# bipul-mohanto/fovPathTracing_optixCodeLatest

Measured on AMD Instinct MI355X. Metric: Mray/s, higher is better.
Workload: dtype f32; 1 GPU; C3: Sponza-class procedural atrium, 265640 tris, 1920x1080, foveated spp fovea/mid/periphery 8/2/1, radii 148/482, gaze centre, Disney BSDF + probe NEE, depth 4, ambient probe 2.5 @ frame res; triangles=265640, width=1920, height=1080, subframe=reset to 0 every frame (as the shipped app), parallelism=single GPU, frames_in_flight=2, gather=none

## Files before the change

fovpathtracing_optixcodelatest_amd/csrc/bvh_build.hip:

```cpp
#include <cstdio>
#include <cstring>
#include <vector>

#include <rocprim/rocprim.hpp>

#include "fovpt_device.h"

namespace {

__device__ inline uint32_t f2ord(float f)
{
    uint32_t u = __float_as_uint(f);
    return (u & 0x80000000u) ? ~u : (u | 0x80000000u);
}
__host__ __device__ inline float ord2f(uint32_t u)
{
    u = (u & 0x80000000u) ? (u & 0x7fffffffu) : ~u;
    float f;
    __builtin_memcpy(&f, &u, 4);
    return f;
}

struct Box { float lo[3], hi[3]; };

// ... 575 lines not shown
        C.code = code;
    }
    nodes[me.out] = nd;
    atomicMax(&stats[0], me.depth + 1u);
    atomicAdd(&stats[1], 1u);
}

#ifndef FOVPT_COST_LEAF_STEP
#define FOVPT_COST_LEAF_STEP 1.4f
#endif
__global__ void k_order_children(uint32_t first, uint32_t count, BvhNode4* __restrict__ nodes, const TriRec* __restrict__ tris, float2* __restrict__ pc)
{
    const uint32_t t = blockIdx.x * blockDim.x + threadIdx.x;
    if (t >= count) return;
    const uint32_t i = first + t;
    const BvhNode4 nd = nodes[i];
    float lo[3] = {INFINITY, INFINITY, INFINITY}, hi[3] = {-INFINITY, -INFINITY, -INFINITY};
    float P[4], C[4], sa[4], key[4];
    for (int k = 0; k < 4; k++) {
        const BvhChild& c = nd.c[k];
        P[k] = 0.f; C[k] = 1.f; sa[k] = 0.f; key[k] = -1.f;
        if (!(c.lox < INFINITY)) continue;
        lo[0] = fminf(lo[0], c.lox); lo[1] = fminf(lo[1], c.loy); lo[2] = fminf(lo[2], c.loz);
        hi[0] = fmaxf(hi[0], c.hix); hi[1] = fmaxf(hi[1], c.hiy); hi[2] = fmaxf(hi[2], c.hiz);
        const float dx = c.hix - c.lox, dy = c.hiy - c.loy, dz = c.hiz - c.loz;
        sa[k] = 2.0f * (dx * dy + dy * dz + dz * dx);
        if (c.code < 0) {
            const uint32_t lcode = (uint32_t)~c.code, n = (lcode & 7u) + 1u, t0 = (lcode >> 3) / 3u;
            float area = 0.f;
            for (uint32_t j = 0; j < n; j++) {
                const TriRec& T = tris[t0 + j];
                const float cx = T.e1y * T.e2z - T.e1z * T.e2y, cy = T.e1z * T.e2x - T.e1x * T.e2z, cz = T.e1x * T.e2y - T.e1y * T.e2x;
                area += 0.5f * sqrtf(cx * cx + cy * cy + cz * cz);
            }
            P[k] = sa[k] > 0.f ? fminf(1.0f, area / sa[k]) : 1.0f;
            C[k] = FOVPT_COST_LEAF_STEP;
        } else {
            const float2 v = pc[c.code];
            P[k] = v.x; C[k] = v.y;
        }
        key[k] = P[k] / C[k];
    }
    const float dx = hi[0] - lo[0], dy = hi[1] - lo[1], dz = hi[2] - lo[2];
    const float sa_node = 2.0f * (dx * dy + dy * dz + dz * dx);
    int ord[4] = {0, 1, 2, 3};
    for (int a = 1; a < 4; a++)
        for (int b = a; b > 0 && key[ord[b]] > key[ord[b - 1]]; b--) { const int tmp = ord[b]; ord[b] = ord[b - 1]; ord[b - 1] = tmp; }
    float pass = 1.0f, cost = 1.0f;
    BvhNode4 out;
    for (int k = 0; k < 4; k++) {
        const int j = ord[k];
        out.c[k] = nd.c[j];
        out.c[k].pad = (uint32_t)j;
        if (key[j] < 0.f) continue;
        const float h = sa_node > 0.f ? fminf(1.0f, sa[j] / sa_node) : 1.0f;
        cost += pass * h * C[j];
        pass *= 1.0f - h * P[j];
    }
    nodes[i] = out;
    pc[i] = make_float2(1.0f - pass, cost);
}

__global__ void k_emit_tiny(int n, const Box* __restrict__ boxes, BvhNode4* __restrict__ nodes, uint32_t* __restrict__ stats, uint32_t* __restrict__ leaf_pos)
{
    Box u = boxes[0];
    for (int i = 1; i < n; i++)
        for (int k = 0; k < 3; k++) { u.lo[k] = fminf(u.lo[k], boxes[i].lo[k]); u.hi[k] = fmaxf(u.hi[k], boxes[i].hi[k]); }
    BvhNode4 nd;
    for (int k = 0; k < 4; k++) {
        BvhChild& C = nd.c[k];
        C.lox = C.loy = C.loz = C.hix = C.hiy = C.hiz = INFINITY;
        C.code = leaf_code(0, 1);
        C.pad = (uint32_t)k;
    }
    nd.c[0].lox = u.lo[0]; nd.c[0].loy = u.lo[1]; nd.c[0].loz = u.lo[2];
    nd.c[0].hix = u.hi[0]; nd.c[0].hiy = u.hi[1]; nd.c[0].hiz = u.hi[2];
    nd.c[0].code = leaf_code(0, n);
    nodes[0] = nd;
    stats[0] = 1; stats[1] = 1;
    for (int i = 0; i < n; i++) leaf_pos[i] = (uint32_t)i;
}

__global__ void k_emit_tris_generic(const float* __restrict__ flat, const uint32_t* __restrict__ mesh_of_prim, const uint32_t* __restrict__ vals,
                                    const uint32_t* __restrict__ ref_prim, const uint32_t* __restrict__ leaf_pos, uint32_t n, TriRec* __restrict__ tris)
{
    uint32_t i = blockIdx.x * blockDim.x + threadIdx.x;
    if (i >= n) return;
    const uint32_t prim = ref_prim ? ref_prim[vals[i]] : vals[i];
    const float* p = flat + (size_t)prim * 9;
    TriRec t;
    t.v0x = p[0]; t.v0y = p[1]; t.v0z = p[2];
    t.e1x = p[3] - p[0]; t.e1y = p[4] - p[1]; t.e1z = p[5] - p[2];
    t.e2x = p[6] - p[0]; t.e2y = p[7] - p[1]; t.e2z = p[8] - p[2];
    t.prim = prim; t.mesh = mesh_of_prim[prim]; t.pad = 0;
    tris[leaf_pos[i]] = t;
}

#define FOVPT_SPLIT_MAX 8
__device__ inline uint32_t split_count(const float* __restrict__ p, float s)
{
    float ext = 0.f;
    for (int a = 0; a < 3; a++) ext = fmaxf(ext, fmaxf(p[a], fmaxf(p[3 + a], p[6 + a])) - fminf(p[a], fminf(p[3 + a], p[6 + a])));
    const float k = floorf(ext / s);
    return k >= (float)FOVPT_SPLIT_MAX ? (uint32_t)FOVPT_SPLIT_MAX : k >= 1.f ? (uint32_t)k : 1u;
}
__global__ void k_split_count(const float* __restrict__ flat, uint32_t n, float s, uint32_t* __restrict__ count, unsigned long long* __restrict__ total)
{
    const uint32_t i = blockIdx.x * blockDim.x + threadIdx.x;
    uint32_t k = i < n ? split_count(flat + (size_t)i * 9, s) : 0u;
    if (count && i < n) count[i] = k;
    for (int off = 32; off > 0; off >>= 1) k += __shfl_xor(k, off);
    if ((threadIdx.x & 63) == 0 && k) atomicAdd(total, (unsigned long long)k);
}
__global__ void k_scene_extent(const float* __restrict__ flat, uint32_t n, uint32_t* __restrict__ bounds)
{
    const uint32_t i = blockIdx.x * blockDim.x + threadIdx.x;
    for (int a = 0; a < 3; a++) {
        float mn = INFINITY, mx = -INFINITY;
        if (i < n) { const float* p = flat + (size_t)i * 9; mn = fminf(p[a], fminf(p[3 + a], p[6 + a])); mx = fmaxf(p[a], fmaxf(p[3 + a], p[6 + a])); }
        for (int off = 32; off > 0; off >>= 1) { mn = fminf(mn, __shfl_xor(mn, off)); mx = fmaxf(mx, __shfl_xor(mx, off)); }
        if ((threadIdx.x & 63) == 0) { atomicMin(&bounds[a], f2ord(mn)); atomicMax(&bounds[3 + a], f2ord(mx)); }
    }
}
__global__ void k_split_emit(const float* __restrict__ flat, uint32_t n, const uint32_t* __restrict__ count, const uint32_t* __restrict__ first,
                             Box* __restrict__ boxes, uint32_t* __restrict__ ref_prim, uint32_t* __restrict__ bounds)
{
    const uint32_t i = blockIdx.x * blockDim.x + threadIdx.x;
    float cmn[3] = {INFINITY, INFINITY, INFINITY}, cmx[3] = {-INFINITY, -INFINITY, -INFINITY};
    if (i < n) {
        const float* p = flat + (size_t)i * 9;
        float lo[3], hi[3], ext = 0.f, mag = 0.f;
        int ax = 0;
        for (int a = 0; a < 3; a++) {
            lo[a] = fminf(p[a], fminf(p[3 + a], p[6 + a])); hi[a] = fmaxf(p[a], fmaxf(p[3 + a], p[6 + a]));
            if (hi[a] - lo[a] > ext) { ext = hi[a] - lo[a]; ax = a; }
            mag = fmaxf(mag, fmaxf(fabsf(lo[a]), fabsf(hi[a])));
        }
        const float pad = fovpt_tri_pad(ext, mag);
        const uint32_t k = count[i], f = first[i];
        for (uint32_t j = 0; j < k; j++) {
            Box b;
            if (k == 1u) { for (int a = 0; a < 3; a++) { b.lo[a] = lo[a]; b.hi[a] = hi[a]; } }
            else {
                const float c0 = j == 0u ? lo[ax] : lo[ax] + (hi[ax] - lo[ax]) * ((float)j / (float)k);
                const float c1 = j + 1u == k ? hi[ax] : lo[ax] + (hi[ax] - lo[ax]) * ((float)(j + 1u) / (float)k);
                for (int a = 0; a < 3; a++) { b.lo[a] = INFINITY; b.hi[a] = -INFINITY; }
                for (int e = 0; e < 3; e++) {
                    const float* u = p + 3 * e;
                    const float* v = p + 3 * ((e + 1) % 3);
                    if (u[ax] >= c0 && u[ax] <= c1) for (int a = 0; a < 3; a++) { b.lo[a] = fminf(b.lo[a], u[a]); b.hi[a] = fmaxf(b.hi[a], u[a]); }
                    for (int side = 0; side < 2; side++) {
                        const float c = side ? c1 : c0;
                        if ((u[ax] < c && v[ax] > c) || (u[ax] > c && v[ax] < c)) {
                            const float t = (c - u[ax]) / (v[ax] - u[ax]);
                            for (int a = 0; a < 3; a++) {
                                const float x = a == ax ? c : u[a] + (v[a] - u[a]) * t;
                                b.lo[a] = fminf(b.lo[a], x); b.hi[a] = fmaxf(b.hi[a], x);
                            }
                        }
                    }
                }
                if (!(b.lo[0] <= b.hi[0])) { for (int a = 0; a < 3; a++) { b.lo[a] = lo[a]; b.hi[a] = hi[a]; } }
                for (int a = 0; a < 3; a++) { b.lo[a] = fmaxf(b.lo[a], lo[a]); b.hi[a] = fminf(b.hi[a], hi[a]); }
            }
            for (int a = 0; a < 3; a++) {
                b.lo[a] -= pad; b.hi[a] += pad;
                const float c = 0.5f * (b.lo[a] + b.hi[a]);
                cmn[a] = fminf(cmn[a], c); cmx[a] = fmaxf(cmx[a], c);
            }
            boxes[f + j] = b;
            ref_prim[f + j] = i;
        }
    }
    for (int a = 0; a < 3; a++) {
        float mn = cmn[a], mx = cmx[a];
        for (int off = 32; off > 0; off >>= 1) { mn = fminf(mn, __shfl_xor(mn, off)); mx = fmaxf(mx, __shfl_xor(mx, off)); }
        if ((threadIdx.x & 63) == 0 && mn <= mx) { atomicMin(&bounds[a], f2ord(mn)); atomicMax(&bounds[3 + a], f2ord(mx)); }
    }
}

#define HC(x) do { hipError_t e_ = (x); if (e_ != hipSuccess) { snprintf(err, errlen, "%s failed: %s", #x, hipGetErrorString(e_)); goto fail; } } while (0)

}

hipError_t fovpt_build_lbvh(hipStream_t st, const float* flat, const uint32_t* mesh_of_prim, uint32_t n_prims, int use_ploc, float split_budget,
                            int reinsert, BvhBuildResult* out, char* err, size_t errlen)
{
    uint32_t n = n_prims;
    uint32_t *ref_prim = nullptr, *split_cnt = nullptr, *split_first = nullptr;
    unsigned long long* split_total = nullptr;
    void* split_temp = nullptr;
    Box *boxes = nullptr, *ibox = nullptr;
    uint32_t *bounds = nullptr, *vals = nullptr, *vals_s = nullptr, *arrive = nullptr, *stats = nullptr;
    uint64_t *keys = nullptr, *keys_s = nullptr;
    int *left = nullptr, *right = nullptr, *parent_int = nullptr, *parent_leaf = nullptr, *rfirst = nullptr, *rlast = nullptr;
    void* temp = nullptr;
    size_t temp_bytes = 0;
    int *c_node = nullptr, *t_node = nullptr, *nn = nullptr;
    Box *c_box = nullptr, *t_box = nullptr;
    uint32_t *valid = nullptr, *pos = nullptr, *node_counter = nullptr, *size_int = nullptr, *leaf_pos = nullptr, *node_first = nullptr, *node_depth = nullptr;
    unsigned char *side_int = nullptr, *side_leaf = nullptr;
    void* scan_temp = nullptr;
    size_t scan_bytes = 0;
    Work4 *work_a = nullptr, *work_b = nullptr;
    DpCost* dp = nullptr;
    std::vector<uint32_t> round_end;
    std::vector<uint32_t> level_first;
    const char* order_env = getenv("FOVPT_BVH_ORDER");
    const bool order_children = !order_env || atoi(order_env) != 0;
    float2* order_pc = nullptr;
    const char* re_env = getenv("FOVPT_REINSERT");
    const int reinsert_rounds = reinsert >= 0 ? reinsert : re_env ? atoi(re_env) : FOVPT_REINSERT_DEFAULT;
    const bool verbose = getenv("FOVPT_BVH_VERBOSE") != nullptr;
    bool tree_changed = false;
    Move* re_moves = nullptr;
    unsigned long long* re_lock = nullptr;
    uint32_t *re_arrive = nullptr, *re_scalars = nullptr;
    unsigned char* re_flags = nullptr;
    uint32_t* dp_arrive = nullptr;
    uint32_t* counters = nullptr;
    BvhNode4* nodes = nullptr;
    TriRec* tris = nullptr;
    const int B = 256;
    uint32_t ni = 1, gn = 1, gi = 1;
    bool have_boxes = false;
    uint32_t h_bounds[6];
    uint32_t h_stats[2] = {0, 0};
    uint32_t h_counters[2] = {1, 0};
    hipError_t rc = hipSuccess;
    err[0] = 0;
    auto sweep_up = [&](int mode, const TreeView& T, float* cost) -> bool {
        const uint32_t nint = (uint32_t)T.n - 1u, g = (nint + 255u) / 256u;
        if (!re_arrive && hipMalloc(&re_arrive, 2ull * nint) != hipSuccess) { snprintf(err, errlen, "hipMalloc failed (sweep flags)"); return false; }
        if (hipMemsetAsync(re_arrive, 0, 2ull * nint, st) != hipSuccess) { snprintf(err, errlen, "hipMemsetAsync failed (sweep flags)"); return false; }
        unsigned short* done = (unsigned short*)re_arrive;
        for (uint32_t sweep = 0; sweep < 65000u;) {
            for (int k = 0; k < 16; k++, sweep++) {
                if (mode == 0) hipLaunchKernelGGL(k_sweep_up<0>, dim3(g), dim3(256), 0, st, T, sweep, done, size_int, side_int, side_leaf, cost, (DpCost*)nullptr);
                else hipLaunchKernelGGL(k_sweep_up<1>, dim3(g), dim3(256), 0, st, T, sweep, done, size_int, side_int, side_leaf, (float*)nullptr, dp);
            }
            unsigned short root_done = 0;
            if (hipMemcpyAsync(&root_done, done + (nint - 1u), 2, hipMemcpyDeviceToHost, st) != hipSuccess || hipStreamSynchronize(st) != hipSuccess) {
                snprintf(err, errlen, "bottom-up sweep failed: %s", hipGetErrorString(hipGetLastError()));
                return false;
            }
            if (root_done) return true;
        }
        snprintf(err, errlen, "bottom-up sweeps did not reach the root");
        return false;
    };
    for (int a = 0; a < 3; a++) { h_bounds[a] = 0xffffffffu; h_bounds[3 + a] = 0u; }
    HC(hipMalloc(&bounds, 6 * 4));
    if (split_budget > 0.f && n_prims > FOVPT_LEAF_MAX) {
        const uint32_t gp = (n_prims + B - 1) / B;
        unsigned long long h_total = 0, want = (unsigned long long)((double)n_prims * (1.0 + (double)split_budget));
        HC(hipMalloc(&split_total, 8));
        HC(hipMemcpyAsync(bounds, h_bounds, sizeof(h_bounds), hipMemcpyHostToDevice, st));
        hipLaunchKernelGGL(k_scene_extent, dim3(gp), dim3(B), 0, st, flat, n_prims, bounds);
        uint32_t hb[6];
        HC(hipMemcpyAsync(hb, bounds, sizeof(hb), hipMemcpyDeviceToHost, st));
        HC(hipStreamSynchronize(st));
        float hi_s = 0.f;
        for (int a = 0; a < 3; a++) hi_s = fmaxf(hi_s, ord2f(hb[3 + a]) - ord2f(hb[a]));
        float lo_s = hi_s * 1e-7f, s_cut = hi_s;
        for (int it = 0; it < 24 && hi_s > 0.f; it++) {
            const float mid = sqrtf(lo_s * hi_s);
            HC(hipMemsetAsync(split_total, 0, 8, st));
            hipLaunchKernelGGL(k_split_count, dim3(gp), dim3(B), 0, st, flat, n_prims, mid, (uint32_t*)nullptr, split_total);
            HC(hipMemcpyAsync(&h_total, split_total, 8, hipMemcpyDeviceToHost, st));
            HC(hipStreamSynchronize(st));
            if (h_total > want) lo_s = mid; else { hi_s = mid; s_cut = mid; }
        }
        HC(hipMalloc(&split_cnt, 4ull * n_prims)); HC(hipMalloc(&split_first, 4ull * n_prims));
        HC(hipMemsetAsync(split_total, 0, 8, st));
        hipLaunchKernelGGL(k_split_count, dim3(gp), dim3(B), 0, st, flat, n_prims, s_cut, split_cnt, split_total);
        HC(hipMemcpyAsync(&h_total, split_total, 8, hipMemcpyDeviceToHost, st));
        HC(hipStreamSynchronize(st));
        if (h_total > n_prims && h_total < (1ull << 27)) {
            size_t tb = 0;
            HC(rocprim::exclusive_scan(nullptr, tb, split_cnt, split_first, 0u, (size_t)n_prims, rocprim::plus<uint32_t>(), st));
            HC(hipMalloc(&split_temp, tb));
            HC(rocprim::exclusive_scan(split_temp, tb, split_cnt, split_first, 0u, (size_t)n_prims, rocprim::plus<uint32_t>(), st));
            n = (uint32_t)h_total;
            HC(hipMalloc(&boxes, sizeof(Box) * n));
            HC(hipMalloc(&ref_prim, 4ull * n));
            HC(hipMemcpyAsync(bounds, h_bounds, sizeof(h_bounds), hipMemcpyHostToDevice, st));
            hipLaunchKernelGGL(k_split_emit, dim3(gp), dim3(B), 0, st, flat, n_prims, split_cnt, split_first, boxes, ref_prim, bounds);
            HC(hipGetLastError());
            have_boxes = true;
        }
    }
    ni = n > 1 ? n - 1 : 1;
    gn = (n + B - 1) / B; gi = (ni + B - 1) / B;

    if (!have_boxes) HC(hipMalloc(&boxes, sizeof(Box) * n));
    HC(hipMalloc(&ibox, sizeof(Box) * ni));
    HC(hipMalloc(&stats, 2 * 4));
    HC(hipMalloc(&counters, 2 * 4));
    HC(hipMalloc(&keys, 8ull * n)); HC(hipMalloc(&keys_s, 8ull * n));
    HC(hipMalloc(&vals, 4ull * n)); HC(hipMalloc(&vals_s, 4ull * n));
    HC(hipMalloc(&left, 4ull * ni)); HC(hipMalloc(&right, 4ull * ni));
    HC(hipMalloc(&parent_int, 4ull * ni)); HC(hipMalloc(&parent_leaf, 4ull * n));
    HC(hipMalloc(&size_int, 4ull * ni)); HC(hipMalloc(&leaf_pos, 4ull * n)); HC(hipMalloc(&node_first, 4ull * ni));
    HC(hipMalloc(&nodes, sizeof(BvhNode4) * ni));
    HC(hipMalloc(&tris, sizeof(TriRec) * n));
    HC(hipMemsetAsync(stats, 0, 8, st));
    if (!have_boxes) {
        HC(hipMemcpyAsync(bounds, h_bounds, sizeof(h_bounds), hipMemcpyHostToDevice, st));
        hipLaunchKernelGGL(k_tri_bounds, dim3(gn), dim3(B), 0, st, flat, n, boxes, bounds);
    }
    if (n <= FOVPT_LEAF_MAX) {
        hipLaunchKernelGGL(k_iota, dim3(1), dim3(64), 0, st, vals_s, n);
        hipLaunchKernelGGL(k_emit_tiny, dim3(1), dim3(1), 0, st, (int)n, boxes, nodes, stats, leaf_pos);
    } else {
        int root = 0;
        hipLaunchKernelGGL(k_morton, dim3(gn), dim3(B), 0, st, boxes, n, bounds, keys, vals);
        HC(rocprim::radix_sort_pairs(nullptr, temp_bytes, keys, keys_s, vals, vals_s, (size_t)n, 0, 63, st));
        HC(hipMalloc(&temp, temp_bytes));
        HC(rocprim::radix_sort_pairs(temp, temp_bytes, keys, keys_s, vals, vals_s, (size_t)n, 0, 63, st));
        if (!use_ploc) {
            HC(hipMalloc(&arrive, 4ull * ni));
            HC(hipMalloc(&rfirst, 4ull * ni)); HC(hipMalloc(&rlast, 4ull * ni));
            HC(hipMemsetAsync(arrive, 0, 4ull * ni, st));
            hipLaunchKernelGGL(k_hierarchy, dim3(gi), dim3(B), 0, st, keys_s, (int)n, left, right, parent_int, parent_leaf, rfirst, rlast);
            hipLaunchKernelGGL(k_refit, dim3(gn), dim3(B), 0, st, boxes, vals_s, (int)n, left, right, parent_int, parent_leaf, ibox, arrive);
            hipLaunchKernelGGL(k_lbvh_generic, dim3(gn), dim3(B), 0, st, (int)n, rfirst, rlast, size_int, node_first, leaf_pos);
            root = 0;
        } else {
            HC(hipMalloc(&c_node, 4ull * n)); HC(hipMalloc(&t_node, 4ull * n)); HC(hipMalloc(&nn, 4ull * n));
            HC(hipMalloc(&c_box, sizeof(Box) * n)); HC(hipMalloc(&t_box, sizeof(Box) * n));
            HC(hipMalloc(&valid, 4ull * n)); HC(hipMalloc(&pos, 4ull * n));
            HC(hipMalloc(&node_counter, 4)); HC(hipMalloc(&node_depth, 4ull * ni));
            HC(hipMalloc(&side_int, ni)); HC(hipMalloc(&side_leaf, n));
            HC(hipMemsetAsync(node_counter, 0, 4, st));
            HC(hipMemsetAsync(side_int, 0, ni, st));
            HC(rocprim::exclusive_scan(nullptr, scan_bytes, valid, pos, 0u, (size_t)n, rocprim::plus<uint32_t>(), st));
            HC(hipMalloc(&scan_temp, scan_bytes));
            hipLaunchKernelGGL(k_ploc_init, dim3(gn), dim3(B), 0, st, (int)n, boxes, vals_s, c_node, c_box);
            uint32_t m = n;
            int force = 0, rounds = 0;
            round_end.clear();
            while (m > 1) {
                const uint32_t gm = (m + B - 1) / B;
                hipLaunchKernelGGL(k_ploc_nn, dim3(gm), dim3(B), 0, st, (int)m, force, c_box, nn);
                hipLaunchKernelGGL(k_ploc_merge, dim3(gm), dim3(B), 0, st, (int)m, c_node, c_box, nn, node_counter, left, right, parent_int,
                                   parent_leaf, side_int, side_leaf, ibox, size_int, valid, t_node, t_box);
                HC(rocprim::exclusive_scan(scan_temp, scan_bytes, valid, pos, 0u, (size_t)m, rocprim::plus<uint32_t>(), st));
                hipLaunchKernelGGL(k_ploc_compact, dim3(gm), dim3(B), 0, st, (int)m, valid, pos, t_node, t_box, c_node, c_box);
                uint32_t last_pos = 0, last_valid = 0, made = 0;
                HC(hipMemcpyAsync(&made, node_counter, 4, hipMemcpyDeviceToHost, st));
                HC(hipMemcpyAsync(&last_pos, pos + (m - 1), 4, hipMemcpyDeviceToHost, st));
                HC(hipMemcpyAsync(&last_valid, valid + (m - 1), 4, hipMemcpyDeviceToHost, st));
                HC(hipStreamSynchronize(st));
                round_end.push_back(made);
                const uint32_t m2 = last_pos + last_valid;
                force = ((uint64_t)(m - m2) * 64u < m) ? 1 : 0;
                m = m2;
                if (++rounds > 4096) { snprintf(err, errlen, "PLOC did not converge"); goto fail; }
            }
            if (reinsert_rounds > 0 && n > 16) {
                TreeView T;
                T.n = (int)n; T.left = left; T.right = right; T.parent_int = parent_int; T.parent_leaf = parent_leaf;
                T.ibox = ibox; T.boxes = boxes; T.vals = vals_s;
                const uint32_t nall = 2 * n - 1, gall2 = (nall + B - 1) / B;
                HC(hipMalloc(&re_moves, sizeof(Move) * (size_t)nall));
                HC(hipMalloc(&re_lock, 8ull * nall));
                HC(hipMalloc(&re_arrive, 2ull * ni));
                HC(hipMalloc(&re_scalars, 16));
                HC(hipMalloc(&re_flags, 2ull * nall));
                float cost_prev = 0.f;
                HC(hipMemsetAsync(re_scalars, 0, 16, st));
                if (!sweep_up(0, T, (float*)(re_scalars + 1))) goto fail;
                HC(hipMemcpyAsync(&cost_prev, re_scalars + 1, 4, hipMemcpyDeviceToHost, st));
                HC(hipStreamSynchronize(st));
                if (verbose) fprintf(stderr, "[fovpt bvh] PLOC tree: sum of internal areas %.6g\n", (double)cost_prev);
                for (int round = 0; round < reinsert_rounds; round++) {
                    uint32_t applied = 0;
                    float cost = 0.f;
                    hipLaunchKernelGGL(k_reinsert_find, dim3(gall2), dim3(B), 0, st, T, (int)n - 2, re_moves, 0u, 1u);
                    HC(hipMemsetAsync(re_lock, 0, 8ull * nall, st));
                    HC(hipMemsetAsync(re_flags, 0, 2ull * nall, st));
                    HC(hipMemsetAsync(re_scalars, 0, 16, st));
                    hipLaunchKernelGGL(k_reinsert_lock, dim3(gall2), dim3(B), 0, st, T, re_moves, re_lock, re_scalars);
                    hipLaunchKernelGGL(k_reinsert_check, dim3(gall2), dim3(B), 0, st, T, re_moves, re_lock, re_flags);
                    hipLaunchKernelGGL(k_reinsert_check2, dim3(gall2), dim3(B), 0, st, T, re_moves, re_lock, re_flags, re_flags + nall, re_scalars);
                    hipLaunchKernelGGL(k_reinsert_apply, dim3(gall2), dim3(B), 0, st, T, re_moves, re_flags + nall);
                    if (!sweep_up(0, T, (float*)(re_scalars + 1))) goto fail;
                    uint32_t candidates = 0;
                    HC(hipMemcpyAsync(&applied, re_scalars, 4, hipMemcpyDeviceToHost, st));
                    HC(hipMemcpyAsync(&cost, re_scalars + 1, 4, hipMemcpyDeviceToHost, st));
                    HC(hipMemcpyAsync(&candidates, re_scalars + 2, 4, hipMemcpyDeviceToHost, st));
                    HC(hipStreamSynchronize(st));
                    HC(hipGetLastError());
                    tree_changed = tree_changed || applied > 0;
                    if (verbose) fprintf(stderr, "[fovpt bvh] reinsertion round %d: %u of %u candidate moves, sum of internal areas %.6g\n", round, applied, candidates, (double)cost);
                    if (applied == 0 || !(cost_prev - cost > FOVPT_REINSERT_STOP * cost_prev)) break;
                    cost_prev = cost;
                }
            }
            const uint32_t gall = (2 * n - 1 + B - 1) / B;
            hipLaunchKernelGGL(k_dfs_offsets, dim3(gall), dim3(B), 0, st, (int)n, left, parent_int, parent_leaf, side_int, side_leaf, size_int,
                               leaf_pos, node_first, node_depth);
            root = (int)n - 2;
        }
        HC(hipMalloc(&dp, sizeof(DpCost) * ni));
        if (use_ploc && !tree_changed) {
            uint32_t first = 0;
            for (uint32_t end : round_end) {
                if (end > first)
                    hipLaunchKernelGGL(k_dp_range, dim3((end - first + B - 1) / B), dim3(B), 0, st, (int)first, (int)(end - first), boxes, vals_s,
                                       left, right, size_int, ibox, dp);
                first = end;
            }
        } else if (use_ploc) {
            TreeView T;
            T.n = (int)n; T.left = left; T.right = right; T.parent_int = parent_int; T.parent_leaf = parent_leaf;
            T.ibox = ibox; T.boxes = boxes; T.vals = vals_s;
            if (!sweep_up(1, T, nullptr)) goto fail;
        } else {
            HC(hipMalloc(&dp_arrive, 4ull * ni));
            HC(hipMemsetAsync(dp_arrive, 0, 4ull * ni, st));
            hipLaunchKernelGGL(k_dp_collapse, dim3(gn), dim3(B), 0, st, (int)n, boxes, vals_s, left, right, parent_int, parent_leaf, size_int, ibox,
                               dp, dp_arrive);
        }
        HC(hipMalloc(&work_a, sizeof(Work4) * ni)); HC(hipMalloc(&work_b, sizeof(Work4) * ni));
        Work4 w0; w0.node = root; w0.out = 0; w0.depth = 0;
        HC(hipMemcpyAsync(work_a, &w0, sizeof(w0), hipMemcpyHostToDevice, st));
        HC(hipMemcpyAsync(counters, h_counters, 8, hipMemcpyHostToDevice, st));
        uint32_t nwork = 1;
        int levels = 0;
        level_first.push_back(0u);
        level_first.push_back(1u);
        while (nwork > 0) {
            hipLaunchKernelGGL(k_collapse4, dim3((nwork + B - 1) / B), dim3(B), 0, st, (int)nwork, work_a, work_b, counters, left, right,
                               size_int, node_first, leaf_pos, boxes, vals_s, ibox, dp, nodes, stats);
            HC(hipMemcpyAsync(h_counters, counters, 8, hipMemcpyDeviceToHost, st));
            HC(hipStreamSynchronize(st));
            nwork = h_counters[1];
            if (nwork > 0) level_first.push_back(h_counters[0]);
            h_counters[1] = 0;
            HC(hipMemcpyAsync(counters + 1, &h_counters[1], 4, hipMemcpyHostToDevice, st));
            Work4* t = work_a; work_a = work_b; work_b = t;
            if (++levels > 4096) { snprintf(err, errlen, "BVH collapse did not terminate"); goto fail; }
        }
    }
    hipLaunchKernelGGL(k_emit_tris_generic, dim3(gn), dim3(B), 0, st, flat, mesh_of_prim, vals_s, ref_prim, leaf_pos, n, tris);
    HC(hipGetLastError());
    if (order_children && level_first.size() >= 2) {
        const uint32_t total = level_first.back();
        HC(hipMalloc(&order_pc, sizeof(float2) * (size_t)total));
        for (size_t L = level_first.size() - 1; L-- > 0;) {
            const uint32_t first = level_first[L], count = level_first[L + 1] - first;
            if (count) hipLaunchKernelGGL(k_order_children, dim3((count + B - 1) / B), dim3(B), 0, st, first, count, nodes, tris, order_pc);
        }
        HC(hipGetLastError());
    }
    HC(hipMemcpyAsync(h_stats, stats, 8, hipMemcpyDeviceToHost, st));
    HC(hipStreamSynchronize(st));

    {
        const size_t node_bytes = sizeof(BvhNode4) * (size_t)h_stats[1], tri_bytes = sizeof(TriRec) * (size_t)n;
        const size_t tri_off = (node_bytes + 255) & ~(size_t)255;
        char* scene = nullptr;
        HC(hipMalloc(&scene, tri_off + tri_bytes + 64));
        if (hipMemcpyAsync(scene, nodes, node_bytes, hipMemcpyDeviceToDevice, st) != hipSuccess
            || hipMemcpyAsync(scene + tri_off, tris, tri_bytes, hipMemcpyDeviceToDevice, st) != hipSuccess
            || hipMemsetAsync(scene + tri_off + tri_bytes, 0, 64, st) != hipSuccess
            || hipStreamSynchronize(st) != hipSuccess) {
            (void)hipFree(scene);
            snprintf(err, errlen, "copying the hierarchy failed");
            goto fail;
        }
        out->nodes = (BvhNode4*)scene; out->tris = (TriRec*)(scene + tri_off);
        out->num_nodes = h_stats[1];
        out->num_refs = n;
        out->max_depth = h_stats[0];
        out->reinserted = tree_changed ? 1u : 0u;
        out->node_bytes = node_bytes;
        out->tri_bytes = tri_bytes;
        if (level_first.size() < 2) level_first.assign({0u, 1u});
        out->num_levels = level_first.size() - 1 <= FOVPT_BVH_MAX_LEVELS ? (uint32_t)(level_first.size() - 1) : 0u;
        for (uint32_t L = 0; out->num_levels && L <= out->num_levels; L++) out->level_first[L] = level_first[L];
    }
fail:
    if (err[0]) rc = hipErrorUnknown;
    (void)hipFree(ref_prim); (void)hipFree(split_cnt); (void)hipFree(split_first); (void)hipFree(split_total); (void)hipFree(split_temp);
    (void)hipFree(boxes); (void)hipFree(ibox); (void)hipFree(bounds); (void)hipFree(stats); (void)hipFree(keys); (void)hipFree(keys_s);
    (void)hipFree(vals); (void)hipFree(vals_s); (void)hipFree(arrive); (void)hipFree(left); (void)hipFree(right); (void)hipFree(parent_int);
    (void)hipFree(parent_leaf); (void)hipFree(rfirst); (void)hipFree(rlast); (void)hipFree(temp); (void)hipFree(nodes); (void)hipFree(tris);
    (void)hipFree(c_node); (void)hipFree(t_node); (void)hipFree(nn); (void)hipFree(c_box); (void)hipFree(t_box); (void)hipFree(valid); (void)hipFree(pos);
    (void)hipFree(node_counter); (void)hipFree(size_int); (void)hipFree(leaf_pos); (void)hipFree(node_first); (void)hipFree(node_depth);
    (void)hipFree(dp); (void)hipFree(dp_arrive); (void)hipFree(order_pc);
    (void)hipFree(re_moves); (void)hipFree(re_lock); (void)hipFree(re_arrive); (void)hipFree(re_scalars); (void)hipFree(re_flags);
    (void)hipFree(side_int); (void)hipFree(side_leaf); (void)hipFree(scan_temp); (void)hipFree(work_a); (void)hipFree(work_b); (void)hipFree(counters);
    return rc;
}
```

fovpathtracing_optixcodelatest_amd/csrc/fovpt_api.hip:

```cpp
#include <cmath>
#include <cstdarg>
#include <cstdio>
#include <cstdlib>
#include <cstring>
#include <string>
#include <vector>

#include "fovpt_device.h"
#ifndef FOVPT_ASYNC_LAST_SHADE_DEFAULT
#define FOVPT_ASYNC_LAST_SHADE_DEFAULT 0
#endif
#ifndef FOVPT_SPLIT_BUDGET_DEFAULT
#define FOVPT_SPLIT_BUDGET_DEFAULT 0.0f
#endif
#include <dlfcn.h>
#include <rccl/rccl.h>

namespace {

std::string g_create_error;

struct DevBuf {
    void* p = nullptr;
    size_t bytes = 0;
    hipError_t reserve(size_t n)
    {
        if (n <= bytes) return hipSuccess;
        if (p) (void)hipFree(p);
        p = nullptr; bytes = 0;
        hipError_t e = hipMalloc(&p, n);
        if (e == hipSuccess) bytes = n;
        return e;
    }
    void release() { if (p) (void)hipFree(p); p = nullptr; bytes = 0; }
};

struct EventPair { hipEvent_t a, b; int kind; };

}

void fovpt_internal_set_error(const char* text) { g_create_error = text ? text : ""; }

#define FOVPT_NSQ 4

struct StateSet {
    DevBuf s_thr, s_rng, s_hit, s_rad, s_alpha, s_backplate, s_guide_n, s_guide_a, s_trace;
    DevBuf q_o[2], q_d[2], counters;
    DevBuf sq_o[FOVPT_NSQ], sq_d[FOVPT_NSQ], sq_vis[FOVPT_NSQ], sq_occ[FOVPT_NSQ];
    hipEvent_t ev_shade[FOVPT_MAX_ITERS + 1] = {};
    hipEvent_t ev_shadow[FOVPT_MAX_ITERS + 1] = {};
    hipEvent_t ev_shade2[FOVPT_MAX_ITERS + 1] = {};
    hipEvent_t ev_shadow2[FOVPT_MAX_ITERS + 1] = {};
    hipEvent_t ev_last_closest2 = nullptr;
    hipEvent_t ev_done = nullptr;
    hipEvent_t ev_last_closest = nullptr;
    bool used = false;
    std::vector<DevBuf*> all()
    {
        std::vector<DevBuf*> v = {&q_o[0], &q_d[0], &q_o[1], &q_d[1], &s_thr, &s_rng, &s_hit, &s_rad, &s_alpha, &s_backplate, &s_guide_n, &s_guide_a, &s_trace, &counters};
        for (int k = 0; k < FOVPT_NSQ; k++) { v.push_back(&sq_o[k]); v.push_back(&sq_d[k]); v.push_back(&sq_vis[k]); v.push_back(&sq_occ[k]); }
        return v;
    }
};

#ifndef FOVPT_LANES_DEFAULT
#define FOVPT_LANES_DEFAULT 2
#endif
#define FOVPT_MAX_LANES 4
#ifndef FOVPT_SETS_SLOT_LIMIT
#define FOVPT_SETS_SLOT_LIMIT (16ull << 20)
#endif

struct fovpt_ctx {
    int device = 0;
    int num_cus = 256;
    hipStream_t stream = nullptr;
    hipStream_t shadow_stream = nullptr;
    hipStream_t lane_main[FOVPT_MAX_LANES] = {}, lane_shadow[FOVPT_MAX_LANES] = {};
    int lanes = FOVPT_LANES_DEFAULT;
    int chains_default = 1;
    int partition = 1;
    std::string err;
    fovpt_config cfg;
    bool has_scene = false;
    uint64_t scene_id = 0;
    BvhNode4* nodes = nullptr;
    TriRec* tris = nullptr;
    DevBuf tri_tc, meshes, textures;
    std::vector<void*> tex_pixels;
    uint32_t num_tris = 0, any_catcher = 0;
    uint32_t bvh_levels[FOVPT_BVH_MAX_LEVELS + 1] = {};
    uint32_t bvh_num_levels = 0;
    std::vector<uint32_t> mesh_prim0, mesh_vbase, mesh_nv, h_tri_vidx;
    std::vector<float> h_vtx;
    DevBuf up_vtx, up_vidx;
    struct Staging { void* p = nullptr; size_t bytes = 0; hipEvent_t ev = nullptr; bool pending = false; } up_stage[2];
    int up_next = 0;
    hipEvent_t ev_scene = nullptr;
    bool refit_pending = false;
    DevBuf pr_data, pr_pdfx, pr_cdfx, pr_pdfy, pr_cdfy, pr_guidex, pr_guidey, pr_rec;
    bool guide_ok = false;
    int guide_w = 0, guide_h = 0;
    bool rows_identical = false;
    DevBuf fb_frame, fb_accum, fb_color, fb_normal, fb_albedo;
    DevBuf accum_before;
    DevBuf plan_owner, plan_blocks, plan_total, plan_base, plan_idx;
    std::vector<uint32_t> plan_off;
    std::string plan_key;
    bool use_accum_before = false;
    int dn_w = 0, dn_h = 0;
    FrameDev dn_frame{};
    int32_t dn_uniform = 0, dn_guides = 0, dn_world = 1;
    DevBuf dn_level, dn_i0, dn_i1, dn_color, dn_rgba;
    DevBuf gb_o, gb_d, gb_hit, gb_cnt, gb_prim, gb_pos, gb_nrm, gb_alb, rc_color, rc_rgba;
    DevBuf tp_prim[2], tp_pos[2], tp_nrm[2], tp_alb[2], tp_hist[2], tp_color, tp_rgba;
    int tp_last = 0;
    bool tp_valid = false;
    int tp_w = 0, tp_h = 0;
    float tp_eye[3] = {}, tp_U[3] = {}, tp_V[3] = {}, tp_W[3] = {};
    ncclComm_t comm = nullptr;
    int comm_rank = 0, comm_world = 0;
    DevBuf comm_packed, comm_gathered;
    StateSet set[2 * FOVPT_MAX_LANES];
    unsigned nsets = 4;
    unsigned last_set = 0;
    unsigned jobs = 0;
    int grid = 2048, grid_trace = 2048, grid_shadow = 1024, grid_shade = 1024;
    int spread_occlusion = 1;
    int async_last_shade = FOVPT_ASYNC_LAST_SHADE_DEFAULT;
    uint64_t slot_budget = 64ull << 20;
    fovpt_stats stats;
    std::vector<EventPair> pending;
    std::vector<hipEvent_t> free_events;
};

namespace {

int fail(fovpt_ctx* c, int code, const char* fmt, ...);
int sync_all(fovpt_ctx* c);

int fail(fovpt_ctx* c, int code, const char* fmt, ...)
{
    char buf[512];
    va_list ap;
    va_start(ap, fmt);
    vsnprintf(buf, sizeof(buf), fmt, ap);
    va_end(ap);
    if (c) c->err = buf; else g_create_error = buf;
    return code;
}

#define HIPCHK(c, x) do { hipError_t e_ = (x); if (e_ != hipSuccess) return fail((c), FOVPT_E_DEVICE, "%s: %s", #x, hipGetErrorString(e_)); } while (0)

int sync_all(fovpt_ctx* c)
{
    for (int l = 0; l < FOVPT_MAX_LANES; l++) {
        if (c->lane_main[l]) HIPCHK(c, hipStreamSynchronize(c->lane_main[l]));
        if (c->lane_shadow[l]) HIPCHK(c, hipStreamSynchronize(c->lane_shadow[l]));
    }
    if (c->shadow_stream) HIPCHK(c, hipStreamSynchronize(c->shadow_stream));
    return FOVPT_OK;
}

fovpt_config default_config()
{
    fovpt_config c;
    memset(&c, 0, sizeof(c));
    c.uniform = 0;
    c.r_inner = 74; c.r_outer = 241;
    c.spp_periphery = 8; c.spp_middle = 16; c.spp_fovea = 32;
    c.spp_uniform = 4;
    c.max_depth = 4;
    c.accumulate = 0;
    c.rank = 0; c.world = 1; c.tile_w = 8; c.tile_h = 4;
    return c;
}

hipEvent_t get_event(fovpt_ctx* c)
{
    if (!c->free_events.empty()) { hipEvent_t e = c->free_events.back(); c->free_events.pop_back(); return e; }
    hipEvent_t e = nullptr;
    if (hipEventCreate(&e) != hipSuccess) return nullptr;
    return e;
}

struct Timed {
    fovpt_ctx* c; int kind; hipStream_t st; hipEvent_t a = nullptr, b = nullptr;
    Timed(fovpt_ctx* c_, int k, hipStream_t s = nullptr) : c(c_), kind(k), st(s ? s : c_->stream)
    {
        if (c->cfg.profile == 2) (void)sync_all(c);
        if (c->cfg.profile) {
            a = get_event(c); b = get_event(c);
            if (a && b) (void)hipEventRecord(a, st);
            else { if (a) c->free_events.push_back(a); if (b) c->free_events.push_back(b); a = b = nullptr; }
        }
    }
    ~Timed()
    {
        if (a && b) { (void)hipEventRecord(b, st); EventPair p = {a, b, kind}; c->pending.push_back(p); }
        if (c->cfg.profile == 2) (void)hipStreamSynchronize(st);
    }
};

void drain_events(fovpt_ctx* c)
{
    for (auto& p : c->pending) {
        float ms = 0.f;
        if (hipEventElapsedTime(&ms, p.a, p.b) == hipSuccess) {
            switch (p.kind) {
            case 0: c->stats.ms_generate += ms; break;
            case 1: c->stats.ms_trace += ms; c->stats.n_trace_launches++; break;
            case 2: c->stats.ms_shade += ms; break;
            case 3: c->stats.ms_shadow += ms; c->stats.n_shadow_launches++; break;
            case 4: c->stats.ms_resolve += ms; break;
            }
        }
        c->free_events.push_back(p.a); c->free_events.push_back(p.b);
    }
    c->pending.clear();
}

void free_scene(fovpt_ctx* c)
{
    if (c->nodes) (void)hipFree(c->nodes);
    c->nodes = nullptr; c->tris = nullptr;
    for (void* p : c->tex_pixels) (void)hipFree(p);
    c->tex_pixels.clear();
    c->has_scene = false;
}

uint32_t shard_capacity(size_t slots) { return (uint32_t)(slots / FOVPT_SHARDS + 512); }

int ensure_state(fovpt_ctx* c, StateSet& S, size_t slots, size_t launches, hipStream_t st)
{
    const size_t v = 16;
    HIPCHK(c, S.s_thr.reserve(slots * v)); HIPCHK(c, S.s_rng.reserve(slots * v));
    HIPCHK(c, S.s_hit.reserve((size_t)shard_capacity(slots) * FOVPT_SHARDS * v));
#if FOVPT_V_STEPSTAT
    HIPCHK(c, S.s_trace.reserve((size_t)shard_capacity(slots) * FOVPT_SHARDS * v));
#endif
    HIPCHK(c, S.s_alpha.reserve(slots * v));
    HIPCHK(c, S.s_rad.reserve(slots * v * (size_t)c->cfg.max_depth));
    HIPCHK(c, S.s_backplate.reserve(launches * v));
    if (c->cfg.write_guides) { HIPCHK(c, S.s_guide_n.reserve(slots * v)); HIPCHK(c, S.s_guide_a.reserve(slots * v)); }
    const size_t qn = (size_t)shard_capacity(slots) * FOVPT_SHARDS;
    for (int k = 0; k < 2; k++) { HIPCHK(c, S.q_o[k].reserve(qn * v)); HIPCHK(c, S.q_d[k].reserve(qn * v)); }
    const int iters_max = c->cfg.max_depth + (c->any_catcher ? 25 : 0);
    for (int k = 0; k < FOVPT_NSQ && k < iters_max; k++) {
        HIPCHK(c, S.sq_o[k].reserve(qn * v)); HIPCHK(c, S.sq_d[k].reserve(qn * v));
        HIPCHK(c, S.sq_vis[k].reserve(qn * v)); HIPCHK(c, S.sq_occ[k].reserve(qn * v));
    }
    if (!S.counters.p) {
        HIPCHK(c, S.counters.reserve(sizeof(Counters)));
        HIPCHK(c, hipMemsetAsync(S.counters.p, 0, sizeof(Counters), st));
        HIPCHK(c, hipStreamSynchronize(st));
    }
    return FOVPT_OK;
}

SceneView scene_view(const fovpt_ctx* c)
{
    SceneView sc;
    sc.nodes = c->nodes; sc.tris = c->tris; sc.tri_tc = (const float2*)c->tri_tc.p;
    sc.meshes = (const MeshDev*)c->meshes.p; sc.textures = (const TexDev*)c->textures.p;
    sc.num_tris = c->num_tris; sc.any_catcher = c->any_catcher;
    sc.tri_off = (uint32_t)((const char*)c->tris - (const char*)c->nodes);
    sc.num_nodes = c->stats.num_bvh_nodes;
    return sc;
}


int run_job(fovpt_ctx* c, const fovpt_launch_params* lp, const PassDev* passes_in, int npass, int chunked, int whole_frame);

int run_passes(fovpt_ctx* c, const fovpt_launch_params* lp, const PassDev* passes_in, int npass, int whole_frame)
{
    if (!c->has_scene || lp->traversable != c->scene_id) return fail(c, FOVPT_E_NO_SCENE, "launch without a scene (traversable %llu, current %llu)",
                                                                     (unsigned long long)lp->traversable, (unsigned long long)c->scene_id);
    if (!lp->probe.data || !lp->probe.cdfValuesX || !lp->probe.cdfValuesY || !lp->probe.pdfValuesX || !lp->probe.pdfValuesY
        || lp->probe.width <= 0 || lp->probe.height <= 0)
        return fail(c, FOVPT_E_NO_PROBE, "launch with an incomplete probe");
    if (!lp->frame.accum_buffer || !lp->frame.frame_buffer) return fail(c, FOVPT_E_NO_FRAME, "launch with null frame buffers");
    if (lp->frame.size.x <= 0 || lp->frame.size.y <= 0) return fail(c, FOVPT_E_INVALID, "bad frame size");
    if (c->cfg.max_depth < 1 || c->cfg.max_depth > 32) return fail(c, FOVPT_E_INVALID, "max_depth out of range");

    uint64_t all_slots = 0;
    for (int p = 0; p < npass; p++) {
        if (passes_in[p].spp == 0) return fail(c, FOVPT_E_INVALID, "samples_per_launch must be >= 1 (do{}while(--i), deviceProgram.cu:448,539)");
        all_slots += (uint64_t)passes_in[p].gw * passes_in[p].gh * passes_in[p].spp;
    }
    const uint64_t budget = c->slot_budget;
    if (all_slots > budget) {
        c->stats.frames++;
        const size_t npix = (size_t)lp->frame.size.x * lp->frame.size.y;
        auto blends = [&](const PassDev& P) { return c->cfg.accumulate && P.subframe > 0 && !P.redraw; };
        auto snapshot = [&]() -> int {
            HIPCHK(c, c->accum_before.reserve(npix * 16));
            HIPCHK(c, hipMemcpyAsync(c->accum_before.p, lp->frame.accum_buffer, npix * 16, hipMemcpyDeviceToDevice, c->shadow_stream));
            return FOVPT_OK;
        };
        if (npass > 0 && blends(passes_in[0])) { int rc = snapshot(); if (rc) return rc; }
        if (whole_frame && c->cfg.world > 1 && c->cfg.rank != 0) {
            HIPCHK(c, hipMemsetAsync(lp->frame.frame_buffer, 0, npix * 4, c->shadow_stream));
            HIPCHK(c, hipMemsetAsync(lp->frame.accum_buffer, 0, npix * 16, c->shadow_stream));
        }
        for (int p = 0; p < npass; p++) {
            const PassDev& P = passes_in[p];
            c->use_accum_before = blends(P);
            if (p > 0 && c->use_accum_before) { int rc = snapshot(); if (rc) return rc; }
            const uint64_t per_row = (uint64_t)P.gw * P.spp;
            if (per_row == 0 || P.gh == 0) continue;
            if (per_row > budget) return fail(c, FOVPT_E_INVALID, "one launch row needs %llu sample slots (budget %llu)", (unsigned long long)per_row, (unsigned long long)budget);
            const uint32_t rows_per = (uint32_t)(budget / per_row);
            for (uint32_t y0 = 0; y0 < P.gh; y0 += rows_per) {
                PassDev Q = P;
                Q.frame_pass = (uint32_t)p;
                Q.row0 = y0; Q.row1 = y0 + rows_per < P.gh ? y0 + rows_per : P.gh;
                int rc = run_job(c, lp, &Q, 1, 1, 0);
                if (rc) return rc;
            }
        }
        return FOVPT_OK;
    }
    PassDev full[FOVPT_MAX_PASSES];
    for (int p = 0; p < npass; p++) { full[p] = passes_in[p]; full[p].row0 = 0; full[p].row1 = passes_in[p].gh; full[p].frame_pass = (uint32_t)p; }
    c->stats.frames++;
    return run_job(c, lp, full, npass, 0, whole_frame);
}

int run_job(fovpt_ctx* c, const fovpt_launch_params* lp, const PassDev* passes_in, int npass, int chunked, int whole_frame)
{
    FrameDev fd;
    memset(&fd, 0, sizeof(fd));
    fd.chunked = chunked;
    fd.zero_holes = (whole_frame && !chunked && c->cfg.world > 1 && c->cfg.rank != 0) ? 1 : 0;
    uint64_t slots = 0, launches = 0;
    for (int p = 0; p < npass; p++) {
        PassDev P = passes_in[p];
        const uint64_t rows = P.row1 - P.row0;
        P.slot_base = (uint32_t)slots; P.launch_base = (uint32_t)launches;
        slots += (uint64_t)P.gw * rows * P.spp;
        launches += (uint64_t)P.gw * rows;
        fd.pass[p] = P;
    }
    if (slots >= (1ull << 31)) return fail(c, FOVPT_E_INVALID, "launch too large: %llu sample slots", (unsigned long long)slots);
    fd.npass = npass;
    fd.w = lp->frame.size.x; fd.h = lp->frame.size.y;
    fd.cx = lp->frame.c.x; fd.cy = lp->frame.c.y;
    const fovpt_float3* cam[4] = {&lp->camera.eye, &lp->camera.U, &lp->camera.V, &lp->camera.W};
    float* dst[4] = {fd.eye, fd.U, fd.V, fd.W};
    for (int k = 0; k < 4; k++) { dst[k][0] = cam[k]->x; dst[k][1] = cam[k]->y; dst[k][2] = cam[k]->z; }
    fd.probe = lp->probe;
    const bool own_probe = c->guide_ok && lp->probe.cdfValuesX == (float*)c->pr_cdfx.p && lp->probe.cdfValuesY == (float*)c->pr_cdfy.p
                           && lp->probe.width == c->guide_w && lp->probe.height == c->guide_h;
    fd.guide_x = own_probe ? (const uint32_t*)c->pr_guidex.p : nullptr;
    fd.guide_y = own_probe ? (const uint32_t*)c->pr_guidey.p : nullptr;
    fd.probe_rec = (own_probe && !c->rows_identical && lp->probe.data == (fovpt_float4*)c->pr_data.p && lp->probe.pdfValuesX == (float*)c->pr_pdfx.p)
                   ? (const float4*)c->pr_rec.p : nullptr;
    fd.probe_row_mul = (c->rows_identical && lp->probe.data == (fovpt_float4*)c->pr_data.p && lp->probe.pdfValuesX == (float*)c->pr_pdfx.p
                        && lp->probe.cdfValuesX == (float*)c->pr_cdfx.p && lp->probe.width == c->guide_w && lp->probe.height == c->guide_h) ? 0 : 1;
    fd.accum = lp->frame.accum_buffer;
    fd.accum_prev = (chunked && c->use_accum_before) ? (const fovpt_float4*)c->accum_before.p : lp->frame.accum_buffer;
    fd.frame = lp->frame.frame_buffer;
    if (c->cfg.write_guides) {
        if (c->any_catcher) return fail(c, FOVPT_E_INVALID, "write_guides is not available with shadow-catcher materials");
        fd.g_normal = lp->frame.normal_buffer; fd.g_color = lp->frame.color_buffer; fd.g_albedo = lp->frame.albedo_buffer;
    }
    fd.total_slots = (uint32_t)slots;
    fd.max_depth = c->cfg.max_depth;
    fd.accumulate = c->cfg.accumulate;
    fd.options = c->cfg.options;
    fd.partition = (c->partition == 2 || (c->partition == 1 && !c->cfg.uniform)) ? 1 : 0;
    fd.rank = c->cfg.rank; fd.world = c->cfg.world < 1 ? 1 : c->cfg.world;
    fd.tile_w = c->cfg.tile_w > 0 ? c->cfg.tile_w : 8; fd.tile_h = c->cfg.tile_h > 0 ? c->cfg.tile_h : 4;

    if (slots == 0) return FOVPT_OK;
    if (c->refit_pending) {
        for (int l = 0; l < FOVPT_MAX_LANES; l++) {
            if (c->lane_main[l]) HIPCHK(c, hipStreamWaitEvent(c->lane_main[l], c->ev_scene, 0));
            if (c->lane_shadow[l] && c->lane_shadow[l] != c->shadow_stream) HIPCHK(c, hipStreamWaitEvent(c->lane_shadow[l], c->ev_scene, 0));
        }
        c->refit_pending = false;
    }
    const unsigned few = c->lanes < 2 ? 2u : (unsigned)c->lanes;
    const unsigned nrot = (chunked || (unsigned long long)slots > FOVPT_SETS_SLOT_LIMIT || c->nsets < few) ? few : c->nsets;
    const unsigned set_index = c->jobs == 0 ? 0u : (c->last_set + 1u) % nrot;
    StateSet& S = c->set[set_index];
    const int fif = c->cfg.frames_in_flight > 0 ? c->cfg.frames_in_flight : c->lanes;
    const unsigned lanes = (unsigned)(fif < c->lanes ? fif : c->lanes);
    const int chains = c->cfg.chains_per_frame > 0 ? c->cfg.chains_per_frame : c->chains_default;
    const bool two_chains = chains == 2 && c->lanes >= 2 && !chunked && slots >= 16384;
    const unsigned lane = two_chains ? 0u : (lanes > 1u && !chunked) ? c->jobs % lanes : 0u;
    hipStream_t st = c->lane_main[lane], ss = c->lane_shadow[lane];
    if (S.used) HIPCHK(c, hipStreamWaitEvent(st, S.ev_done, 0));
    if (S.used && two_chains) HIPCHK(c, hipStreamWaitEvent(c->lane_main[1], S.ev_done, 0));
    int rc = ensure_state(c, S, (size_t)slots, (size_t)launches, st);
    if (rc) return rc;
    for (unsigned k = 0; k < nrot && !chunked; k++)
        if (k != set_index && (c->set[k].s_thr.bytes < (size_t)slots * 16 || c->set[k].s_rad.bytes < (size_t)slots * 16 * (size_t)c->cfg.max_depth)) {
            rc = ensure_state(c, c->set[k], (size_t)slots, (size_t)launches, st);
            if (rc) return rc;
        }
    c->jobs++;
    c->last_set = set_index;
    S.used = true;

    PathState ps;
    ps.thr = (float4*)S.s_thr.p;
    ps.rng = (uint4*)S.s_rng.p; ps.hit = (float4*)S.s_hit.p; ps.rad = (float4*)S.s_rad.p; ps.stride = (size_t)c->cfg.max_depth;
    ps.alpha = (float4*)S.s_alpha.p; ps.backplate = (float4*)S.s_backplate.p;
    ps.guide_n = c->cfg.write_guides ? (float4*)S.s_guide_n.p : nullptr;
    ps.guide_a = c->cfg.write_guides ? (float4*)S.s_guide_a.p : nullptr;
#if FOVPT_V_STEPSTAT
    ps.trace = (uint4*)S.s_trace.p;
#endif
    ShadowQueue sq[FOVPT_NSQ];
    for (int k = 0; k < FOVPT_NSQ; k++) {
        sq[k].o = (float4*)S.sq_o[k].p; sq[k].d = (float4*)S.sq_d[k].p;
        sq[k].val_vis = (float4*)S.sq_vis[k].p; sq[k].val_occ = (float4*)S.sq_occ[k].p;
    }
    const SceneView sc = scene_view(c);
    Counters* cnt = (Counters*)S.counters.p;
#if FOVPT_V_STEPSTAT
    HIPCHK(c, hipMemsetAsync(cnt, 0, offsetof(Counters, stat_radiance), st));
#endif
    const uint32_t cap = shard_capacity((size_t)slots);
    int iters = c->cfg.max_depth + (c->any_catcher ? 1 + 24 : 0);
    if (iters > FOVPT_MAX_ITERS) iters = FOVPT_MAX_ITERS;
    const int nsq = iters < FOVPT_NSQ ? iters : FOVPT_NSQ;
    const bool tail_async = c->async_last_shade != 0;
    int spread_it = (c->spread_occlusion && fd.world > 1 && lanes > 1u && lane == 0u && !two_chains && !chunked && !tail_async
                           && c->cfg.max_depth >= 2) ? (c->spread_occlusion == 2 ? 1 : -2) : -1;
    if (spread_it == -2) spread_it = iters <= nsq ? iters - 1 : 1;
    auto issue_chain = [&](hipStream_t st, hipStream_t ss, uint32_t sel, uint32_t slot_begin, uint32_t slot_end, int div,
                           hipEvent_t* ev_shade, hipEvent_t* ev_shadow, hipEvent_t ev_last_closest) -> int {
        RayQueue qa, qb;
        qa.o = (float4*)S.q_o[0].p; qa.d = (float4*)S.q_d[0].p;
        qb.o = (float4*)S.q_o[1].p; qb.d = (float4*)S.q_d[1].p;
        const int g_gen = c->grid / div, g_trace = c->grid_trace / div, g_shadow = c->grid_shadow / div, g_shade = c->grid_shade / div;
        { Timed t(c, 0, st); fovpt_launch_generate(st, fd, ps, qa, cap, cnt, slot_begin, slot_end, g_gen, sel); }
        { Timed t(c, 1, st); fovpt_launch_traverse(st, sc, ps, qa, sq[0], cap, cnt, 0, -1, g_trace, (tail_async && iters == 1) ? ev_last_closest : nullptr, sel); }
// ... 154 lines not shown
    double r[3][3];
    cross(v, w, r[0]); cross(w, u, r[1]); cross(u, v, r[2]);
    const double det = (u[0] * r[0][0] + u[1] * r[0][1]) + u[2] * r[0][2];
    if (det == 0.0 || !std::isfinite(det)) return false;
    for (int i = 0; i < 3; i++)
        for (int j = 0; j < 3; j++) inv[3 * i + j] = (float)(r[i][j] / det);
    return true;
}

int enqueue_gbuffer(fovpt_ctx* c, const fovpt_launch_params* lp, const FrameDev& view, GBufferDev& g, const char* who,
                    const GBufferDev* target = nullptr)
{
    if (!c->has_scene || lp->traversable != c->scene_id) return fail(c, FOVPT_E_NO_SCENE, "%s without a scene (traversable %llu, current %llu)", who,
                                                                     (unsigned long long)lp->traversable, (unsigned long long)c->scene_id);
#if FOVPT_V_STEPSTAT
    return fail(c, FOVPT_E_INVALID, "%s: not available in a diagnostic (FOVPT_V_STEPSTAT) build", who);
#endif
    const int w = lp->frame.size.x, h = lp->frame.size.y;
    if (w <= 0 || h <= 0) return fail(c, FOVPT_E_INVALID, "%s: frame size %d x %d", who, w, h);
    const size_t n = (size_t)w * (size_t)h;
    if (n >= (1ull << 31)) return fail(c, FOVPT_E_INVALID, "%s: frame too large (%d x %d)", who, w, h);
    HIPCHK(c, hipSetDevice(c->device));
    { const int rc_ = reserve_gbuffer(c, n); if (rc_) return rc_; }
    FrameDev fd;
    memset(&fd, 0, sizeof(fd));
    fd.w = w; fd.h = h;
    memcpy(fd.eye, view.eye, sizeof(fd.eye)); memcpy(fd.U, view.U, sizeof(fd.U));
    memcpy(fd.V, view.V, sizeof(fd.V)); memcpy(fd.W, view.W, sizeof(fd.W));
    RayQueue q; q.o = (float4*)c->gb_o.p; q.d = (float4*)c->gb_d.p;
    PathState ps;
    memset(&ps, 0, sizeof(ps));
    ps.hit = (float4*)c->gb_hit.p;
    ShadowQueue sq;
    memset(&sq, 0, sizeof(sq));
    Counters* cnt = (Counters*)c->gb_cnt.p;
    if (target) g = *target;
    else { g.prim = (uint32_t*)c->gb_prim.p; g.pos = (float4*)c->gb_pos.p; g.nrm = (float4*)c->gb_nrm.p; g.alb = (float4*)c->gb_alb.p; }
    hipStream_t st = c->shadow_stream;
    fovpt_launch_gbuffer_rays(st, fd, q, cnt);
    fovpt_launch_traverse(st, scene_view(c), ps, q, sq, (uint32_t)n, cnt, 0, -1, c->grid_trace);
    fovpt_launch_gbuffer_fill(st, fd, scene_view(c), q, ps.hit, g);
    HIPCHK(c, hipGetLastError());
    return FOVPT_OK;
}

int build_hierarchy(fovpt_ctx* c, hipStream_t st, const float* d_flat, const uint32_t* d_mesh_of, uint32_t ntri, BvhBuildResult& br, float& ms)
{
    struct Ev { hipEvent_t e = nullptr; ~Ev() { if (e) (void)hipEventDestroy(e); } } ev0, ev1;
    HIPCHK(c, hipEventCreate(&ev0.e)); HIPCHK(c, hipEventCreate(&ev1.e));
    const hipEvent_t e0 = ev0.e, e1 = ev1.e;
    HIPCHK(c, hipEventRecord(e0, st));
    memset(&br, 0, sizeof(br));
    char errbuf[256];
    const char* bvh_env = getenv("FOVPT_BVH");
    const int use_ploc = !(bvh_env && strcmp(bvh_env, "lbvh") == 0);
    float split_budget = FOVPT_SPLIT_BUDGET_DEFAULT;
    if (const char* sb = getenv("FOVPT_SPLIT")) split_budget = (float)atof(sb);
    if (!(split_budget >= 0.f) || split_budget > 2.f) split_budget = 0.f;
    hipError_t be = fovpt_build_lbvh(st, d_flat, d_mesh_of, ntri, use_ploc, split_budget, -1, &br, errbuf, sizeof(errbuf));
    if (be == hipSuccess && br.reinserted && 3 * br.max_depth + 1 > FOVPT_STACK) {
        (void)hipFree(br.nodes);
        memset(&br, 0, sizeof(br));
        be = fovpt_build_lbvh(st, d_flat, d_mesh_of, ntri, use_ploc, split_budget, 0, &br, errbuf, sizeof(errbuf));
    }
    (void)hipEventRecord(e1, st);
    (void)hipEventSynchronize(e1);
    ms = 0.f;
    (void)hipEventElapsedTime(&ms, e0, e1);
    if (be != hipSuccess) return fail(c, FOVPT_E_DEVICE, "LBVH build: %s", errbuf);
    if (3 * br.max_depth + 1 > FOVPT_STACK) {
        (void)hipFree(br.nodes);
        return fail(c, FOVPT_E_BVH_DEPTH, "hierarchy depth %u needs more than the %d traversal stack entries", br.max_depth, FOVPT_STACK);
    }
    if ((size_t)((const char*)br.tris - (const char*)br.nodes) + br.tri_bytes + 64 >= (1ull << 32)) {
        (void)hipFree(br.nodes);
        return fail(c, FOVPT_E_INVALID, "hierarchy of %llu bytes exceeds the 32-bit offsets of the traversal",
                    (unsigned long long)(br.node_bytes + br.tri_bytes));
    }
    return FOVPT_OK;
}

void adopt_hierarchy(fovpt_ctx* c, const BvhBuildResult& br, float ms)
{
    c->nodes = br.nodes; c->tris = br.tris;
    c->num_tris = br.num_refs;
    c->bvh_num_levels = br.num_levels;
    memcpy(c->bvh_levels, br.level_first, sizeof(c->bvh_levels));
    c->stats.num_bvh_nodes = br.num_nodes; c->stats.bvh_max_depth = br.max_depth;
    c->stats.bvh_bytes = br.node_bytes; c->stats.tri_bytes = br.tri_bytes; c->stats.ms_bvh_build = ms;
}

}

extern "C" {

int fovpt_create(fovpt_ctx** out, int device)
{
    if (!out) return fail(nullptr, FOVPT_E_INVALID, "null out pointer");
    *out = nullptr;
    int n = 0;
    hipError_t e = hipGetDeviceCount(&n);
    if (e != hipSuccess || n == 0) return fail(nullptr, FOVPT_E_DEVICE, "no HIP device found (%s)", hipGetErrorString(e));
    if (device < 0 || device >= n) return fail(nullptr, FOVPT_E_INVALID, "device %d out of range (%d devices)", device, n);
    e = hipSetDevice(device);
    if (e != hipSuccess) return fail(nullptr, FOVPT_E_DEVICE, "hipSetDevice: %s", hipGetErrorString(e));
    fovpt_ctx* c = new fovpt_ctx;
    c->device = device;
    c->cfg = default_config();
    memset(&c->stats, 0, sizeof(c->stats));
    hipDeviceProp_t prop;
    if (hipGetDeviceProperties(&prop, device) == hipSuccess && prop.multiProcessorCount > 0) c->num_cus = prop.multiProcessorCount;
    c->grid = c->num_cus * 8;
    c->grid_trace = c->num_cus * FOVPT_GRID_PER_CU;
    c->grid_shadow = c->num_cus * FOVPT_GRID_SHADOW_PER_CU;
    if (const char* g = getenv("FOVPT_GRID_GEN")) { const int v = atoi(g); if (v > 0 && v <= 64) c->grid = c->num_cus * v; }
    if (const char* g = getenv("FOVPT_GRID")) { const int v = atoi(g); if (v > 0 && v <= 64) c->grid_trace = c->num_cus * v; }
    if (const char* g = getenv("FOVPT_GRID_SHADOW")) { const int v = atoi(g); if (v > 0 && v <= 16) c->grid_shadow = c->num_cus * v; }
    c->grid = (c->grid + FOVPT_SHARDS - 1) / FOVPT_SHARDS * FOVPT_SHARDS;
    c->grid_trace = (c->grid_trace + FOVPT_SHARDS - 1) / FOVPT_SHARDS * FOVPT_SHARDS;
    c->grid_shadow = (c->grid_shadow + FOVPT_SHARDS - 1) / FOVPT_SHARDS * FOVPT_SHARDS;
    c->grid_shade = c->num_cus * 8;
    if (const char* g = getenv("FOVPT_GRID_SHADE")) { const int v = atoi(g); if (v > 0 && v <= 16) c->grid_shade = c->num_cus * v; }
    c->grid_shade = (c->grid_shade + FOVPT_SHARDS - 1) / FOVPT_SHARDS * FOVPT_SHARDS;
    if (const char* a = getenv("FOVPT_ASYNC_LAST_SHADE")) c->async_last_shade = atoi(a) != 0;
    if (const char* sb = getenv("FOVPT_SLOT_BUDGET")) { const long long v = atoll(sb); if (v > 0) c->slot_budget = (uint64_t)v; }
    int prio_lo = 0, prio_hi = 0;
    (void)hipDeviceGetStreamPriorityRange(&prio_lo, &prio_hi);
    e = hipStreamCreateWithPriority(&c->stream, hipStreamDefault, prio_hi);
    if (e == hipSuccess) e = hipStreamCreateWithPriority(&c->shadow_stream, hipStreamDefault, prio_lo);
    if (const char* l = getenv("FOVPT_LANES")) { const int v = atoi(l); if (v >= 1 && v <= FOVPT_MAX_LANES) c->lanes = v; }
    if (const char* l = getenv("FOVPT_PARTITION")) { const int v = atoi(l); if (v >= 0 && v <= 2) c->partition = v; }
    if (const char* l = getenv("FOVPT_SPREAD_OCCLUSION")) c->spread_occlusion = atoi(l);
    if (const char* l = getenv("FOVPT_CHAINS")) { const int v = atoi(l); if (v == 1 || v == 2) c->chains_default = v; }
    c->nsets = 2u * (unsigned)c->lanes;
    if (const char* l = getenv("FOVPT_SETS")) { const int v = atoi(l); if (v >= 2 && v <= 2 * FOVPT_MAX_LANES) c->nsets = (unsigned)v; }
    c->lane_main[0] = c->stream; c->lane_shadow[0] = c->shadow_stream;
    for (int l = 1; l < c->lanes; l++) {
        if (e == hipSuccess) e = hipStreamCreateWithPriority(&c->lane_main[l], hipStreamDefault, prio_hi);
        if (e == hipSuccess) e = hipStreamCreateWithPriority(&c->lane_shadow[l], hipStreamDefault, prio_lo);
    }
    for (StateSet& S : c->set) {
        for (int k = 0; k <= FOVPT_MAX_ITERS && e == hipSuccess; k++) {
            e = hipEventCreateWithFlags(&S.ev_shade[k], hipEventDefault);
            if (e == hipSuccess) e = hipEventCreateWithFlags(&S.ev_shadow[k], hipEventDefault);
            if (e == hipSuccess) e = hipEventCreateWithFlags(&S.ev_shade2[k], hipEventDefault);
            if (e == hipSuccess) e = hipEventCreateWithFlags(&S.ev_shadow2[k], hipEventDefault);
        }
        if (e == hipSuccess) e = hipEventCreateWithFlags(&S.ev_done, hipEventDefault);
        if (e == hipSuccess) e = hipEventCreateWithFlags(&S.ev_last_closest, hipEventDefault);
        if (e == hipSuccess) e = hipEventCreateWithFlags(&S.ev_last_closest2, hipEventDefault);
    }
    if (e != hipSuccess) { fovpt_destroy(c); return fail(nullptr, FOVPT_E_DEVICE, "stream/event creation: %s", hipGetErrorString(e)); }
    *out = c;
    return FOVPT_OK;
}

void fovpt_destroy(fovpt_ctx* c)
{
    if (!c) return;
    (void)hipSetDevice(c->device);
    (void)sync_all(c);
    drain_events(c);
    for (hipEvent_t e : c->free_events) (void)hipEventDestroy(e);
    for (StateSet& S : c->set) {
        for (int k = 0; k <= FOVPT_MAX_ITERS; k++) {
            if (S.ev_shade[k]) (void)hipEventDestroy(S.ev_shade[k]);
            if (S.ev_shadow[k]) (void)hipEventDestroy(S.ev_shadow[k]);
            if (S.ev_shade2[k]) (void)hipEventDestroy(S.ev_shade2[k]);
            if (S.ev_shadow2[k]) (void)hipEventDestroy(S.ev_shadow2[k]);
        }
        if (S.ev_done) (void)hipEventDestroy(S.ev_done);
        if (S.ev_last_closest) (void)hipEventDestroy(S.ev_last_closest);
        if (S.ev_last_closest2) (void)hipEventDestroy(S.ev_last_closest2);
        for (DevBuf* b : S.all()) b->release();
    }
    (void)fovpt_comm_destroy(c);
    free_scene(c);
    DevBuf* bufs[] = {&c->tri_tc, &c->meshes, &c->textures, &c->pr_data, &c->pr_pdfx, &c->pr_cdfx, &c->pr_pdfy, &c->pr_cdfy, &c->pr_guidex, &c->pr_guidey, &c->pr_rec,
                      &c->fb_frame, &c->fb_accum, &c->fb_color, &c->fb_normal, &c->fb_albedo, &c->accum_before,
                      &c->plan_owner, &c->plan_blocks, &c->plan_total, &c->plan_base, &c->plan_idx,
                      &c->comm_packed, &c->comm_gathered, &c->dn_level, &c->dn_i0, &c->dn_i1, &c->dn_color, &c->dn_rgba,
                      &c->gb_o, &c->gb_d, &c->gb_hit, &c->gb_cnt, &c->gb_prim, &c->gb_pos, &c->gb_nrm, &c->gb_alb, &c->rc_color, &c->rc_rgba,
                      &c->tp_color, &c->tp_rgba, &c->up_vtx, &c->up_vidx};
    for (DevBuf* b : bufs) b->release();
    for (int k = 0; k < 2; k++) { c->tp_prim[k].release(); c->tp_pos[k].release(); c->tp_nrm[k].release(); c->tp_alb[k].release(); c->tp_hist[k].release(); }
    for (auto& S : c->up_stage) {
        if (S.p) (void)hipHostFree(S.p);
        if (S.ev) (void)hipEventDestroy(S.ev);
    }
    if (c->ev_scene) (void)hipEventDestroy(c->ev_scene);
    for (int l = 0; l < FOVPT_MAX_LANES; l++) {
        if (c->lane_main[l] && c->lane_main[l] != c->stream) (void)hipStreamDestroy(c->lane_main[l]);
        if (c->lane_shadow[l] && c->lane_shadow[l] != c->shadow_stream) (void)hipStreamDestroy(c->lane_shadow[l]);
    }
    if (c->stream) (void)hipStreamDestroy(c->stream);
    if (c->shadow_stream) (void)hipStreamDestroy(c->shadow_stream);
    delete c;
}

const char* fovpt_last_error(const fovpt_ctx* c) { return c ? c->err.c_str() : g_create_error.c_str(); }

int fovpt_set_scene(fovpt_ctx* c, const fovpt_mesh_desc* meshes, int num_meshes,
                    const fovpt_texture_desc* textures, int num_textures, uint64_t* traversable_out)
{
    if (!c) return FOVPT_E_INVALID;
    if (!meshes || num_meshes <= 0) return fail(c, FOVPT_E_INVALID, "scene needs at least one mesh");
    HIPCHK(c, hipSetDevice(c->device));
    { const int rc_ = sync_all(c); if (rc_) return rc_; }
    free_scene(c);
    c->tp_valid = false;
    c->up_vtx.release(); c->up_vidx.release();
    c->refit_pending = false;
    uint64_t ntri = 0;
    bool any_tc = false;
    for (int m = 0; m < num_meshes; m++) {
        const fovpt_mesh_desc& D = meshes[m];
        if (!D.vertex || !D.index) return fail(c, FOVPT_E_INVALID, "mesh %d has null vertex/index", m);
        ntri += D.num_triangles;
        if (D.texcoord && D.texture_id >= 0) any_tc = true;
        if (D.texture_id >= num_textures) return fail(c, FOVPT_E_INVALID, "mesh %d references texture %d of %d (SimplePathtracer.cpp:581-583 would index out of range)", m, D.texture_id, num_textures);
    }
    if (ntri == 0) return fail(c, FOVPT_E_INVALID, "scene has no triangles");
    if (ntri > (1ull << 26)) return fail(c, FOVPT_E_INVALID, "too many triangles (%llu > 2^26)", (unsigned long long)ntri);
    std::vector<float> flat((size_t)ntri * 9);
    std::vector<uint32_t> mesh_of((size_t)ntri);
    std::vector<float> tc(any_tc ? (size_t)ntri * 6 : 0, 0.0f);
    std::vector<MeshDev> md((size_t)num_meshes);
    c->any_catcher = 0;
    c->mesh_prim0.assign((size_t)num_meshes, 0u); c->mesh_vbase.assign((size_t)num_meshes, 0u); c->mesh_nv.assign((size_t)num_meshes, 0u);
    c->h_tri_vidx.assign((size_t)ntri * 3, 0u);
    c->h_vtx.clear();
    size_t t = 0;
    for (int m = 0; m < num_meshes; m++) {
        const fovpt_mesh_desc& D = meshes[m];
        c->mesh_prim0[m] = (uint32_t)t; c->mesh_vbase[m] = (uint32_t)(c->h_vtx.size() / 3); c->mesh_nv[m] = D.num_vertices;
        c->h_vtx.insert(c->h_vtx.end(), D.vertex, D.vertex + 3 * (size_t)D.num_vertices);
        md[m].material = D.material;
        md[m].texture_id = D.texture_id >= 0 ? D.texture_id : -1;
        md[m].has_texcoord = D.texcoord ? 1 : 0;
        if (D.material.flags & FOVPT_MATERIAL_FLAG_SHADOW_CATCHER) c->any_catcher = 1;
        for (uint32_t k = 0; k < D.num_triangles; k++, t++) {
            for (int v = 0; v < 3; v++) {
                const uint32_t idx = D.index[3 * (size_t)k + v];
                if (idx >= D.num_vertices) return fail(c, FOVPT_E_INVALID, "mesh %d triangle %u indexes vertex %u of %u", m, k, idx, D.num_vertices);
                c->h_tri_vidx[t * 3 + v] = c->mesh_vbase[m] + idx;
                flat[t * 9 + v * 3 + 0] = D.vertex[3 * (size_t)idx + 0];
                flat[t * 9 + v * 3 + 1] = D.vertex[3 * (size_t)idx + 1];
                flat[t * 9 + v * 3 + 2] = D.vertex[3 * (size_t)idx + 2];
                if (any_tc && D.texcoord) { tc[t * 6 + v * 2] = D.texcoord[2 * (size_t)idx]; tc[t * 6 + v * 2 + 1] = D.texcoord[2 * (size_t)idx + 1]; }
            }
            mesh_of[t] = (uint32_t)m;
        }
    }
    struct Tmp { void* p = nullptr; ~Tmp() { if (p) (void)hipFree(p); } } t_flat, t_mesh_of;
    HIPCHK(c, hipMalloc(&t_flat.p, flat.size() * 4));
    HIPCHK(c, hipMalloc(&t_mesh_of.p, mesh_of.size() * 4));
    float* d_flat = (float*)t_flat.p; uint32_t* d_mesh_of = (uint32_t*)t_mesh_of.p;
    HIPCHK(c, hipMemcpy(d_flat, flat.data(), flat.size() * 4, hipMemcpyHostToDevice));
    HIPCHK(c, hipMemcpy(d_mesh_of, mesh_of.data(), mesh_of.size() * 4, hipMemcpyHostToDevice));
    if (any_tc) {
        HIPCHK(c, c->tri_tc.reserve(tc.size() * 4));
        HIPCHK(c, hipMemcpy(c->tri_tc.p, tc.data(), tc.size() * 4, hipMemcpyHostToDevice));
    }
    std::vector<TexDev> td((size_t)(num_textures > 0 ? num_textures : 1));
    for (int k = 0; k < num_textures; k++) {
        const fovpt_texture_desc& X = textures[k];
        if (!X.pixel || X.width <= 0 || X.height <= 0) return fail(c, FOVPT_E_INVALID, "texture %d is empty", k);
        void* px = nullptr;
        const size_t nb = (size_t)X.width * X.height * 4;
        HIPCHK(c, hipMalloc(&px, nb));
        c->tex_pixels.push_back(px);
        HIPCHK(c, hipMemcpy(px, X.pixel, nb, hipMemcpyHostToDevice));
        td[k].px = (const uint32_t*)px; td[k].w = X.width; td[k].h = X.height;
    }
    HIPCHK(c, c->textures.reserve(td.size() * sizeof(TexDev)));
    HIPCHK(c, hipMemcpy(c->textures.p, td.data(), td.size() * sizeof(TexDev), hipMemcpyHostToDevice));
    for (int m = 0; m < num_meshes; m++) {
        md[m].tex.px = nullptr; md[m].tex.w = md[m].tex.h = 0;
        if (md[m].texture_id >= 0) md[m].tex = td[md[m].texture_id];
    }
    HIPCHK(c, c->meshes.reserve(md.size() * sizeof(MeshDev)));
    HIPCHK(c, hipMemcpy(c->meshes.p, md.data(), md.size() * sizeof(MeshDev), hipMemcpyHostToDevice));

    BvhBuildResult br;
    float ms = 0.f;
    { const int rc_ = build_hierarchy(c, c->stream, d_flat, d_mesh_of, (uint32_t)ntri, br, ms); if (rc_) return rc_; }
    adopt_hierarchy(c, br, ms);
    c->stats.num_triangles = ntri;
    c->has_scene = true;
    c->scene_id = (c->scene_id & 0xffffffffull) + 1;
    c->scene_id |= 0x464f565000000000ull;
    if (traversable_out) *traversable_out = c->scene_id;
    return FOVPT_OK;
}

int fovpt_update_vertices(fovpt_ctx* c, const fovpt_vertex_update* up, int num_updates, int flags)
{
    if (!c) return FOVPT_E_INVALID;
    if (!c->has_scene) return fail(c, FOVPT_E_NO_SCENE, "fovpt_update_vertices without a scene");
    if (num_updates < 0 || (num_updates > 0 && !up)) return fail(c, FOVPT_E_INVALID, "fovpt_update_vertices: %d updates at %p", num_updates, (const void*)up);
    if (flags & ~(FOVPT_UPDATE_DEVICE | FOVPT_UPDATE_REBUILD)) return fail(c, FOVPT_E_INVALID, "fovpt_update_vertices: unknown flag bits %d", flags);
    const bool device = (flags & FOVPT_UPDATE_DEVICE) != 0, rebuild = (flags & FOVPT_UPDATE_REBUILD) != 0;
    const int nmesh = (int)c->mesh_nv.size();
    std::vector<char> seen((size_t)nmesh, 0);
    size_t floats = 0;
    for (int k = 0; k < num_updates; k++) {
        const fovpt_vertex_update& U = up[k];
        if (U.mesh < 0 || U.mesh >= nmesh) return fail(c, FOVPT_E_INVALID, "fovpt_update_vertices: mesh %d of %d", U.mesh, nmesh);
        if (seen[U.mesh]) return fail(c, FOVPT_E_INVALID, "fovpt_update_vertices: mesh %d is listed twice", U.mesh);
        seen[U.mesh] = 1;
        if (U.num_vertices != c->mesh_nv[U.mesh])
            return fail(c, FOVPT_E_INVALID, "fovpt_update_vertices: mesh %d has %u vertices, the update %u", U.mesh, c->mesh_nv[U.mesh], U.num_vertices);
        if (!U.vertex) return fail(c, FOVPT_E_INVALID, "fovpt_update_vertices: mesh %d has a null vertex pointer", U.mesh);
        if (!device)
            for (size_t i = 0; i < 3 * (size_t)U.num_vertices; i++)
                if (!std::isfinite(U.vertex[i])) return fail(c, FOVPT_E_INVALID, "fovpt_update_vertices: mesh %d vertex %zu is not finite", U.mesh, i / 3);
        floats += 3 * (size_t)U.num_vertices;
    }
    if (c->h_vtx.size() / 3 >= (1ull << 32)) return fail(c, FOVPT_E_INVALID, "fovpt_update_vertices: more than 2^32 - 1 vertices");
    if (c->bvh_num_levels == 0) return fail(c, FOVPT_E_INVALID, "fovpt_update_vertices: the hierarchy has more than %d levels", FOVPT_BVH_MAX_LEVELS);
    if (num_updates == 0 && !rebuild) return FOVPT_OK;
    HIPCHK(c, hipSetDevice(c->device));
    if (rebuild) { const int rc_ = sync_all(c); if (rc_) return rc_; }
    const hipStream_t st = c->shadow_stream;
    if (!c->up_vtx.p) {
        if (!c->ev_scene) HIPCHK(c, hipEventCreateWithFlags(&c->ev_scene, hipEventDisableTiming));
        for (auto& S : c->up_stage)
            if (!S.ev) HIPCHK(c, hipEventCreateWithFlags(&S.ev, hipEventDisableTiming));
        HIPCHK(c, c->up_vidx.reserve(c->h_tri_vidx.size() * 4));
        HIPCHK(c, c->up_vtx.reserve(c->h_vtx.size() * 4));
        HIPCHK(c, hipMemcpyAsync(c->up_vidx.p, c->h_tri_vidx.data(), c->h_tri_vidx.size() * 4, hipMemcpyHostToDevice, st));
        HIPCHK(c, hipMemcpyAsync(c->up_vtx.p, c->h_vtx.data(), c->h_vtx.size() * 4, hipMemcpyHostToDevice, st));
    }
    float* vtx = (float*)c->up_vtx.p;
    if (device) {
        VertexGather g;
        memset(&g, 0, sizeof(g));
        for (int k = 0; k < num_updates; k++) {
            g.src[g.count] = up[k].vertex; g.dst[g.count] = c->mesh_vbase[up[k].mesh]; g.n[g.count] = up[k].num_vertices;
            g.max_n = up[k].num_vertices > g.max_n ? up[k].num_vertices : g.max_n;
            if (++g.count == FOVPT_GATHER_BATCH || k + 1 == num_updates) { fovpt_launch_gather_vertices(st, g, vtx); memset(&g, 0, sizeof(g)); }
        }
        HIPCHK(c, hipGetLastError());
    } else if (floats) {
        auto& S = c->up_stage[c->up_next];
        c->up_next ^= 1;
        if (S.pending) { HIPCHK(c, hipEventSynchronize(S.ev)); S.pending = false; }
        if (S.bytes < floats * 4) {
            if (S.p) (void)hipHostFree(S.p);
            S.p = nullptr; S.bytes = 0;
            HIPCHK(c, hipHostMalloc(&S.p, floats * 4, hipHostMallocDefault));
            S.bytes = floats * 4;
        }
        float* h = (float*)S.p;
        for (int k = 0; k < num_updates; k++) {
            const size_t n = 3 * (size_t)up[k].num_vertices;
            memcpy(h, up[k].vertex, n * 4);
            HIPCHK(c, hipMemcpyAsync(vtx + 3 * (size_t)c->mesh_vbase[up[k].mesh], h, n * 4, hipMemcpyHostToDevice, st));
            h += n;
        }
        HIPCHK(c, hipEventRecord(S.ev, st));
        S.pending = true;
    }
    if (!rebuild) {
        fovpt_launch_refit(st, c->nodes, c->tris, c->bvh_levels, c->bvh_num_levels, (const uint3*)c->up_vidx.p, vtx);
        HIPCHK(c, hipGetLastError());
        HIPCHK(c, hipEventRecord(c->ev_scene, st));
        c->refit_pending = true;
        return FOVPT_OK;
    }
    const uint32_t ntri = (uint32_t)c->stats.num_triangles;
    struct Tmp { void* p = nullptr; ~Tmp() { if (p) (void)hipFree(p); } } t_flat, t_mesh_of;
    HIPCHK(c, hipMalloc(&t_flat.p, (size_t)ntri * 36));
    HIPCHK(c, hipMalloc(&t_mesh_of.p, (size_t)ntri * 4));
    std::vector<uint32_t> mesh_of((size_t)ntri);
    for (int m = 0; m < nmesh; m++) {
        const uint32_t end = m + 1 < nmesh ? c->mesh_prim0[m + 1] : ntri;
        for (uint32_t t = c->mesh_prim0[m]; t < end; t++) mesh_of[t] = (uint32_t)m;
    }
    HIPCHK(c, hipMemcpyAsync(t_mesh_of.p, mesh_of.data(), mesh_of.size() * 4, hipMemcpyHostToDevice, st));
    fovpt_launch_flatten(st, ntri, (const uint3*)c->up_vidx.p, vtx, (float*)t_flat.p);
    HIPCHK(c, hipGetLastError());
    HIPCHK(c, hipStreamSynchronize(st));
    BvhBuildResult br;
    float ms = 0.f;
    { const int rc_ = build_hierarchy(c, st, (const float*)t_flat.p, (const uint32_t*)t_mesh_of.p, ntri, br, ms); if (rc_) return rc_; }
    (void)hipFree(c->nodes);
    adopt_hierarchy(c, br, ms);
    return FOVPT_OK;
}

int fovpt_set_probe(fovpt_ctx* c, int width, int height, const fovpt_float4* data,
                    const float* pdfX, const float* cdfX, const float* pdfY, const float* cdfY,
                    const fovpt_float3* offset, fovpt_probe* out)
{
    if (!c) return FOVPT_E_INVALID;
    if (!data || !pdfX || !cdfX || !pdfY || !cdfY || width <= 0 || height <= 0 || !out)
        return fail(c, FOVPT_E_INVALID, "Probe Data is not valid");
    HIPCHK(c, hipSetDevice(c->device));
    { const int rc_ = sync_all(c); if (rc_) return rc_; }
    const size_t n = (size_t)width * height;
    HIPCHK(c, c->pr_pdfx.reserve(n * 4)); HIPCHK(c, c->pr_cdfx.reserve(n * 4));
    HIPCHK(c, c->pr_pdfy.reserve((size_t)height * 4)); HIPCHK(c, c->pr_cdfy.reserve((size_t)height * 4));
    HIPCHK(c, c->pr_data.reserve(n * 16));
    HIPCHK(c, hipMemcpy(c->pr_pdfx.p, pdfX, n * 4, hipMemcpyHostToDevice));
    HIPCHK(c, hipMemcpy(c->pr_cdfx.p, cdfX, n * 4, hipMemcpyHostToDevice));
    HIPCHK(c, hipMemcpy(c->pr_pdfy.p, pdfY, (size_t)height * 4, hipMemcpyHostToDevice));
    HIPCHK(c, hipMemcpy(c->pr_cdfy.p, cdfY, (size_t)height * 4, hipMemcpyHostToDevice));
    HIPCHK(c, hipMemcpy(c->pr_data.p, data, n * 16, hipMemcpyHostToDevice));
    bool sorted = true;
    for (int row = 0; row < height && sorted; row++) {
        const float* cr = cdfX + (size_t)row * width;
        for (int k = 1; k < width; k++) if (!(cr[k] >= cr[k - 1])) { sorted = false; break; }
    }
    for (int k = 1; k < height && sorted; k++) if (!(cdfY[k] >= cdfY[k - 1])) sorted = false;
    c->guide_ok = false;
    if (sorted) {
        HIPCHK(c, c->pr_guidex.reserve((size_t)height * (width + 2) * 4));
        HIPCHK(c, c->pr_guidey.reserve((size_t)(height + 2) * 4));
        fovpt_launch_build_guide(c->stream, (const float*)c->pr_cdfx.p, width, height, (uint32_t*)c->pr_guidex.p);
        fovpt_launch_build_guide(c->stream, (const float*)c->pr_cdfy.p, height, 1, (uint32_t*)c->pr_guidey.p);
        HIPCHK(c, c->pr_rec.reserve(n * 32));
        fovpt_launch_probe_records(c->stream, n, (const float*)c->pr_cdfx.p, (const float*)c->pr_pdfx.p, (const float4*)c->pr_data.p, (float4*)c->pr_rec.p);
        HIPCHK(c, hipStreamSynchronize(c->stream));
        c->guide_ok = true;
    }
    c->guide_w = width; c->guide_h = height;
    c->rows_identical = true;
    for (int row = 1; row < height && c->rows_identical; row++)
        if (memcmp(data + (size_t)row * width, data, (size_t)width * 16) || memcmp(pdfX + (size_t)row * width, pdfX, (size_t)width * 4)
            || memcmp(cdfX + (size_t)row * width, cdfX, (size_t)width * 4)) c->rows_identical = false;
    memset(out, 0, sizeof(*out));
    out->width = width; out->height = height;
    out->data = (fovpt_float4*)c->pr_data.p;
    out->pdfValuesX = (float*)c->pr_pdfx.p; out->cdfValuesX = (float*)c->pr_cdfx.p;
    out->pdfValuesY = (float*)c->pr_pdfy.p; out->cdfValuesY = (float*)c->pr_cdfy.p;
    if (offset) out->offset = *offset;
    return FOVPT_OK;
}

int fovpt_set_probe_data(fovpt_ctx* c, int width, int height, const fovpt_float4* data, const fovpt_float3* offset, fovpt_probe* out)
{
    if (!c) return FOVPT_E_INVALID;
    if (!data || width <= 0 || height <= 0 || !out) return fail(c, FOVPT_E_INVALID, "Probe Data is not valid");
    HIPCHK(c, hipSetDevice(c->device));
    { const int rc_ = sync_all(c); if (rc_) return rc_; }
    const size_t n = (size_t)width * height;
    HIPCHK(c, c->pr_pdfx.reserve(n * 4)); HIPCHK(c, c->pr_cdfx.reserve(n * 4));
// ... 592 lines not shown
    if (!c || !out) return FOVPT_E_INVALID;
    HIPCHK(c, hipSetDevice(c->device));
    { const int rc_ = sync_all(c); if (rc_) return rc_; }
    drain_events(c);
    c->stats.radiance_rays = c->stats.shadow_rays = c->stats.paths = 0;
    for (StateSet& S : c->set) {
        if (!S.counters.p) continue;
        unsigned long long h[3];
        HIPCHK(c, hipMemcpy(h, (const char*)S.counters.p + offsetof(Counters, stat_radiance), sizeof(h), hipMemcpyDeviceToHost));
        c->stats.radiance_rays += h[0]; c->stats.shadow_rays += h[1]; c->stats.paths += h[2];
    }
    *out = c->stats;
    return FOVPT_OK;
}

int fovpt_reset_stats(fovpt_ctx* c)
{
    if (!c) return FOVPT_E_INVALID;
    HIPCHK(c, hipSetDevice(c->device));
    { const int rc_ = sync_all(c); if (rc_) return rc_; }
    drain_events(c);
    for (StateSet& S : c->set)
        if (S.counters.p) HIPCHK(c, hipMemset((char*)S.counters.p + offsetof(Counters, stat_radiance), 0, sizeof(Counters) - offsetof(Counters, stat_radiance)));
    c->stats.radiance_rays = c->stats.shadow_rays = c->stats.paths = c->stats.frames = 0;
    c->stats.ms_generate = c->stats.ms_trace = c->stats.ms_shade = c->stats.ms_shadow = c->stats.ms_resolve = 0.0;
    c->stats.n_trace_launches = c->stats.n_shadow_launches = 0;
    return FOVPT_OK;
}

void* fovpt_stream(fovpt_ctx* c) { return c ? (void*)c->shadow_stream : nullptr; }

int fovpt_probe_build_cdf(int width, int height, const fovpt_float4* data,
                          float* pdfValuesX, float* cdfValuesX, float* pdfValuesY, float* cdfValuesY)
{
    if (width <= 0 || height <= 0 || !data || !pdfValuesX || !cdfValuesX || !pdfValuesY || !cdfValuesY) return FOVPT_E_INVALID;
    volatile float col_total = 0.0f;
    for (int row = 0; row < height; ++row) {
        volatile float row_total = 0.0f;
        float* pdf_row = pdfValuesX + (size_t)row * width;
        float* cdf_row = cdfValuesX + (size_t)row * width;
        const fovpt_float4* px = data + (size_t)row * width;
        for (int k = 0; k < width; ++k) {
            const float lum = px[k].x * 0.3f + px[k].y * 0.6f + px[k].z * 0.1f;
            row_total = row_total + lum;
            pdf_row[k] = lum;
            cdf_row[k] = row_total;
        }
        const float inv = 1.0f / row_total;
        for (int k = 0; k < width; ++k) { pdf_row[k] *= inv; cdf_row[k] *= inv; }
        col_total = col_total + row_total;
        pdfValuesY[row] = row_total;
        cdfValuesY[row] = col_total;
    }
    const float total = col_total;
    for (int row = 0; row < height; ++row) { cdfValuesY[row] /= total; pdfValuesY[row] /= total; }
    return FOVPT_OK;
}

int fovpt_camera_uvw(const fovpt_float3* eye, const fovpt_float3* lookat, const fovpt_float3* up,
                     float fovY, float aspect, fovpt_float3* U, fovpt_float3* V, fovpt_float3* W)
{
    if (!eye || !lookat || !up || !U || !V || !W) return FOVPT_E_INVALID;
    const float wx = lookat->x - eye->x, wy = lookat->y - eye->y, wz = lookat->z - eye->z;
    const float wlen = sqrtf(wx * wx + wy * wy + wz * wz);
    float ux = wy * up->z - wz * up->y, uy = wz * up->x - wx * up->z, uz = wx * up->y - wy * up->x;
    float inv = 1.0f / sqrtf(ux * ux + uy * uy + uz * uz);
    ux *= inv; uy *= inv; uz *= inv;
    float vx = uy * wz - uz * wy, vy = uz * wx - ux * wz, vz = ux * wy - uy * wx;
    inv = 1.0f / sqrtf(vx * vx + vy * vy + vz * vz);
    vx *= inv; vy *= inv; vz *= inv;
    const float vlen = wlen * tanf(0.5f * fovY * 3.14159265358979323846f / 180.0f);
    vx *= vlen; vy *= vlen; vz *= vlen;
    const float ulen = vlen * aspect;
    ux *= ulen; uy *= ulen; uz *= ulen;
    U->x = ux; U->y = uy; U->z = uz; V->x = vx; V->y = vy; V->z = vz; W->x = wx; W->y = wy; W->z = wz;
    return FOVPT_OK;
}

int fovpt_debug_buffer(fovpt_ctx* c, const char* name, void** ptr, size_t* bytes)
{
    if (!c || !name || !ptr || !bytes) return FOVPT_E_INVALID;
    if (strcmp(name, "bvh_nodes") == 0 && c->has_scene) { *ptr = c->nodes; *bytes = (size_t)c->stats.bvh_bytes; return FOVPT_OK; }
    if (strcmp(name, "bvh_tris") == 0 && c->has_scene) { *ptr = c->tris; *bytes = (size_t)c->stats.tri_bytes; return FOVPT_OK; }
    if (strcmp(name, "scene_vertices") == 0 && c->up_vtx.p) { *ptr = c->up_vtx.p; *bytes = c->h_vtx.size() * 4; return FOVPT_OK; }
    StateSet& S = c->set[c->last_set];
    struct { const char* n; DevBuf* b; } tab[] = {
        {"sq_o", &S.sq_o[0]}, {"sq_d", &S.sq_d[0]}, {"sq_vis", &S.sq_vis[0]}, {"sq_occ", &S.sq_occ[0]}, {"counters", &S.counters},
        {"hit", &S.s_hit}, {"trace", &S.s_trace}, {"queue_a_o", &S.q_o[0]}, {"queue_a_d", &S.q_d[0]}, {"queue_b_o", &S.q_o[1]}, {"queue_b_d", &S.q_d[1]},
    };
    for (auto& t : tab)
        if (strcmp(t.n, name) == 0) { *ptr = t.b->p; *bytes = t.b->bytes; return FOVPT_OK; }
    return fail(c, FOVPT_E_INVALID, "unknown debug buffer %s", name);
}

int fovpt_debug_trace(fovpt_ctx* c, int n, const float* origins3, const float* dirs3, uint32_t* prim_out, float* tuv_out3, uint8_t* occluded_out)
{
    if (!c || n < 0 || (n && (!origins3 || !dirs3))) return FOVPT_E_INVALID;
    if (!c->has_scene) return fail(c, FOVPT_E_NO_SCENE, "fovpt_debug_trace without a scene");
    if (n == 0) return FOVPT_OK;
    HIPCHK(c, hipSetDevice(c->device));
    { const int rc_ = sync_all(c); if (rc_) return rc_; }
    StateSet& S = c->set[(c->last_set + 1u) % 2u];
    const size_t slots = (size_t)n * FOVPT_SHARDS;
    int rc = ensure_state(c, S, slots, 1, c->stream);
    if (rc) return rc;
    const uint32_t cap = shard_capacity(slots);
    hipStream_t st = c->stream;
    std::vector<float> o4((size_t)n * 4), d4((size_t)n * 4), d4s((size_t)n * 4), vis((size_t)n * 4, 0.f), occ((size_t)n * 4, 0.f);
    for (int i = 0; i < n; i++) {
        const uint32_t slot = (uint32_t)i, cell = 0u;
        for (int k = 0; k < 3; k++) { o4[4 * (size_t)i + k] = origins3[3 * (size_t)i + k]; d4[4 * (size_t)i + k] = d4s[4 * (size_t)i + k] = dirs3[3 * (size_t)i + k]; }
        memcpy(&o4[4 * (size_t)i + 3], &slot, 4);
        d4[4 * (size_t)i + 3] = 0.f;
        memcpy(&d4s[4 * (size_t)i + 3], &cell, 4);
        vis[4 * (size_t)i] = 1.f; occ[4 * (size_t)i] = 2.f;
    }
    const size_t bytes = (size_t)n * 16;
    HIPCHK(c, hipMemcpyAsync(S.q_o[0].p, o4.data(), bytes, hipMemcpyHostToDevice, st));
    HIPCHK(c, hipMemcpyAsync(S.q_d[0].p, d4.data(), bytes, hipMemcpyHostToDevice, st));
    HIPCHK(c, hipMemcpyAsync(S.sq_o[0].p, o4.data(), bytes, hipMemcpyHostToDevice, st));
    HIPCHK(c, hipMemcpyAsync(S.sq_d[0].p, d4s.data(), bytes, hipMemcpyHostToDevice, st));
    HIPCHK(c, hipMemcpyAsync(S.sq_vis[0].p, vis.data(), bytes, hipMemcpyHostToDevice, st));
    HIPCHK(c, hipMemcpyAsync(S.sq_occ[0].p, occ.data(), bytes, hipMemcpyHostToDevice, st));
    HIPCHK(c, hipMemsetAsync(S.counters.p, 0, offsetof(Counters, stat_radiance), st));
    const uint32_t un = (uint32_t)n;
    Counters* cnt = (Counters*)S.counters.p;
    HIPCHK(c, hipMemcpyAsync(&cnt->shard[0][FOVPT_CNT_Q(0)], &un, 4, hipMemcpyHostToDevice, st));
    HIPCHK(c, hipMemcpyAsync(&cnt->shard[0][FOVPT_CNT_SQ(0)], &un, 4, hipMemcpyHostToDevice, st));
    PathState ps;
    memset(&ps, 0, sizeof(ps));
    ps.thr = (float4*)S.s_thr.p; ps.rng = (uint4*)S.s_rng.p; ps.hit = (float4*)S.s_hit.p; ps.rad = (float4*)S.s_rad.p;
    ps.stride = (size_t)c->cfg.max_depth; ps.alpha = (float4*)S.s_alpha.p; ps.backplate = (float4*)S.s_backplate.p;
#if FOVPT_V_STEPSTAT
    ps.trace = (uint4*)S.s_trace.p;
#endif
    RayQueue q; q.o = (float4*)S.q_o[0].p; q.d = (float4*)S.q_d[0].p;
    ShadowQueue sq; sq.o = (float4*)S.sq_o[0].p; sq.d = (float4*)S.sq_d[0].p; sq.val_vis = (float4*)S.sq_vis[0].p; sq.val_occ = (float4*)S.sq_occ[0].p;
    const SceneView sc = scene_view(c);
    fovpt_launch_traverse(st, sc, ps, q, sq, cap, cnt, 0, -1, c->grid_trace);
    fovpt_launch_traverse(st, sc, ps, q, sq, cap, cnt, -1, 0, c->grid_shadow);
    HIPCHK(c, hipGetLastError());
    std::vector<float> hit((size_t)n * 4), cell((size_t)n * 4 * (size_t)c->cfg.max_depth);
    HIPCHK(c, hipMemcpyAsync(hit.data(), S.s_hit.p, bytes, hipMemcpyDeviceToHost, st));
    HIPCHK(c, hipMemcpyAsync(cell.data(), S.s_rad.p, bytes * (size_t)c->cfg.max_depth, hipMemcpyDeviceToHost, st));
    HIPCHK(c, hipStreamSynchronize(st));
    std::vector<TriRec> tris(c->num_tris);
    HIPCHK(c, hipMemcpy(tris.data(), c->tris, sizeof(TriRec) * (size_t)c->num_tris, hipMemcpyDeviceToHost));
    HIPCHK(c, hipMemset(S.counters.p, 0, offsetof(Counters, stat_radiance)));
    for (int i = 0; i < n; i++) {
        uint32_t pos;
        memcpy(&pos, &hit[4 * (size_t)i + 3], 4);
        const bool miss = pos == 0xffffffffu;
        const size_t tri = miss ? 0 : (size_t)pos / 3;
        if (!miss && (pos % 3u != 0u || tri >= tris.size())) return fail(c, FOVPT_E_DEVICE, "hit record %d points at 16-byte unit %u", i, pos);
        if (prim_out) prim_out[i] = miss ? 0xffffffffu : tris[tri].prim;
        if (tuv_out3) for (int k = 0; k < 3; k++) tuv_out3[3 * (size_t)i + k] = hit[4 * (size_t)i + k];
        if (occluded_out) {
            const float v = cell[4 * (size_t)i * (size_t)c->cfg.max_depth];
            if (v != 1.f && v != 2.f) return fail(c, FOVPT_E_DEVICE, "shadow ray %d left %g in its cell", i, (double)v);
            occluded_out[i] = v == 2.f ? 1 : 0;
        }
    }
    return FOVPT_OK;
}

int fovpt_debug_math(fovpt_ctx* c, int op, const float* a, const float* b, float* out, size_t n)
// ... 19 lines not shown
```

fovpathtracing_optixcodelatest_amd/csrc/fovpt_device.h:

```cpp
#pragma once

#include <hip/hip_runtime.h>
#include <stdint.h>

#include "../../include/fovpt.h"

#define FOVPT_WAVE 64
#define FOVPT_BLOCK 256
#ifndef FOVPT_V_STEPSTAT
#define FOVPT_V_STEPSTAT 0
#endif
#ifndef FOVPT_V_CYCLES
#define FOVPT_V_CYCLES 0
#endif
#ifndef FOVPT_V_VOTE_ANYHIT
#define FOVPT_V_VOTE_ANYHIT 1
#endif
#ifndef FOVPT_V_MIXED
#define FOVPT_V_MIXED 1
#endif
#ifndef FOVPT_V_MIXED_ANYHIT
#define FOVPT_V_MIXED_ANYHIT 1
#endif
#ifndef FOVPT_V_GEN_OWNED
#define FOVPT_V_GEN_OWNED 1
#endif
#ifndef FOVPT_V_ANYHIT_SORT
#define FOVPT_V_ANYHIT_SORT 0
#endif
#ifndef FOVPT_LEAF_MAX
#define FOVPT_LEAF_MAX 4
#endif
#define FOVPT_STACK 64
#define FOVPT_QUADS_PER_BLOCK (FOVPT_BLOCK / 4)
#ifndef FOVPT_TBLOCK
#define FOVPT_TBLOCK 64
#endif
#define FOVPT_TQUADS (FOVPT_TBLOCK / 4)
#ifndef FOVPT_GRID_PER_CU
#define FOVPT_GRID_PER_CU 24
#endif
#ifndef FOVPT_GRID_SHADOW_PER_CU
#define FOVPT_GRID_SHADOW_PER_CU 6
#endif
#define FOVPT_MAX_PASSES 3
#define FOVPT_MAX_ITERS 63
#define FOVPT_SHARDS 8

struct alignas(16) TriRec {
    float v0x, v0y, v0z, e1x;
    float e1y, e1z, e2x, e2y;
    float e2z;
    uint32_t prim;
    uint32_t mesh;
    uint32_t pad;
};
static_assert(sizeof(TriRec) == 48, "TriRec");

struct alignas(16) BvhChild {
    float lox, loy, loz, hix;
    float hiy, hiz;
    int32_t code;
    uint32_t pad;
};
struct alignas(16) BvhNode4 {
    BvhChild c[4];
};
static_assert(sizeof(BvhNode4) == 128, "BvhNode4");

struct TexDev {
    const uint32_t* px;
    int32_t w, h;
};

struct MeshDev {
    fovpt_material material;
    int32_t texture_id;
    int32_t has_texcoord;
    TexDev tex;
};

struct SceneView {
    const BvhNode4* nodes;
    const TriRec* tris;
    const float2* tri_tc;
    const MeshDev* meshes;
    const TexDev* textures;
    uint32_t num_tris;
    uint32_t any_catcher;
    uint32_t tri_off;
    uint32_t num_nodes;
};


struct PassDev {
    uint32_t gw, gh;
    uint32_t fx, fy, fz;
    int32_t fill;
    uint32_t offx, offy;
    float r_inner, r_outer;
    uint32_t spp;
    uint32_t subframe;
    uint32_t redraw;
    uint32_t slot_base;
    uint32_t launch_base;
    uint32_t row0, row1;
    uint32_t frame_pass;
};

struct FrameDev {
    PassDev pass[FOVPT_MAX_PASSES];
    int32_t npass;
    int32_t w, h;
    uint32_t cx, cy;
    float eye[3], U[3], V[3], W[3];
    fovpt_probe probe;
    const uint32_t* guide_x;
    const uint32_t* guide_y;
    const float4* probe_rec;
    int32_t probe_row_mul;
    fovpt_float4* accum;
    const fovpt_float4* accum_prev;
    uint32_t* frame;
    fovpt_float4 *g_normal, *g_color, *g_albedo;
    uint32_t total_slots;
    int32_t max_depth;
    int32_t accumulate;
    int32_t rank, world, tile_w, tile_h;
    int32_t chunked;
    int32_t zero_holes;
    int32_t options;
    int32_t partition;
};

struct RayQueue {
    float4* o;
    float4* d;
};

struct PathState {
    float4* thr;
    uint4* rng;
    float4* hit;
    float4* rad;
    size_t stride;
    float4* alpha;
    float4* guide_n;
    float4* guide_a;
    float4* backplate;
#if FOVPT_V_STEPSTAT
    uint4* trace;
#endif
};

struct ShadowQueue {
    float4* o;
    float4* d;
    float4* val_vis;
    float4* val_occ;
};

#ifndef FOVPT_SHARD_STRIDE
#define FOVPT_SHARD_STRIDE 128
#endif
struct Counters {
    uint32_t shard[FOVPT_SHARDS][FOVPT_SHARD_STRIDE];
    unsigned long long stat_radiance, stat_shadow, stat_paths;
    unsigned long long diag[2][4];
#if FOVPT_V_CYCLES
    unsigned long long cyc[2][8][16];
    uint32_t hist[2][8][3][64];
    unsigned long long wtime[8][32768][2];
#endif
};
static_assert(2 * (FOVPT_MAX_ITERS + 1) <= FOVPT_SHARD_STRIDE, "shard block holds both queues' sizes");
#define FOVPT_CNT_Q(it) (it)
#define FOVPT_CNT_SQ(it) (FOVPT_MAX_ITERS + 1 + (it))

__device__ inline float fovpt_tri_pad(float ext, float mag) { return 1e-4f * ext + 1e-5f * mag + 1e-20f; }

#define FOVPT_BVH_MAX_LEVELS 64
struct BvhBuildResult {
    BvhNode4* nodes;
    TriRec* tris;
    uint32_t num_nodes;
    uint32_t num_refs;
    uint32_t max_depth;
    uint32_t reinserted;
    size_t node_bytes, tri_bytes;
    uint32_t num_levels;
    uint32_t level_first[FOVPT_BVH_MAX_LEVELS + 1];
};

hipError_t fovpt_build_lbvh(hipStream_t st, const float* flat, const uint32_t* mesh_of_prim, uint32_t n, int use_ploc, float split_budget,
                            int reinsert, BvhBuildResult* out, char* err, size_t errlen);

void fovpt_launch_generate(hipStream_t st, const FrameDev& fd, PathState ps, RayQueue queue0, uint32_t cap, Counters* cnt, uint32_t slot_begin,
                           uint32_t slot_end, int grid, uint32_t sel = 0);
void fovpt_launch_traverse(hipStream_t st, SceneView sc, PathState ps, RayQueue queue, ShadowQueue sq, uint32_t cap,
                           Counters* cnt, int it_closest, int it_shadow, int grid, hipEvent_t done = nullptr, uint32_t sel = 0);
void fovpt_launch_shade(hipStream_t st, const FrameDev& fd, SceneView sc, PathState ps, RayQueue queue_in, RayQueue queue_out,
                        ShadowQueue sq, uint32_t cap, Counters* cnt, int depth, int grid, hipEvent_t done = nullptr, uint32_t sel = 0);
void fovpt_launch_resolve(hipStream_t st, const FrameDev& fd, PathState ps, Counters* cnt, hipEvent_t done = nullptr);
void fovpt_launch_plan_owner(hipStream_t st, const FrameDev& fd, uint8_t* owner, uint32_t* block_count, uint32_t nblocks);
void fovpt_launch_plan_scan_fill(hipStream_t st, uint32_t npix, uint32_t nblocks, int world, const uint8_t* owner, uint32_t* block_count,
                                 uint32_t* total, const uint32_t* rank_base, uint32_t* idx, int phase);
void fovpt_launch_gather_pack(hipStream_t st, uint32_t n, const uint32_t* idx, const uint32_t* frame, uint32_t* packed);
void fovpt_launch_gather_unpack(hipStream_t st, int world, uint32_t stride, uint32_t total, const uint32_t* base, const uint32_t* idx,
                                const uint32_t* gathered, uint32_t* frame);
struct DenoiseArgs {
    int32_t n_pass[FOVPT_MAX_PASSES];
    int32_t iterations;
    float inv_c, inv_n, inv_a;
};
void fovpt_launch_denoise(hipStream_t st, const FrameDev& fd, const DenoiseArgs& a, const fovpt_float4* color, const fovpt_float4* normal,
                          const fovpt_float4* albedo, float4* I0, float4* I1, uint8_t* level, fovpt_float4* out_color, uint32_t* out_rgba);
struct GBufferDev {
    uint32_t* prim;
    float4* pos;
    float4* nrm;
    float4* alb;
};
void fovpt_launch_gbuffer_rays(hipStream_t st, const FrameDev& fd, RayQueue q, Counters* cnt);
void fovpt_launch_gbuffer_fill(hipStream_t st, const FrameDev& fd, SceneView sc, RayQueue q, const float4* hit, GBufferDev g);
struct ReconstructArgs {
    float inv_support[2];
    float inv_n, inv_z;
    int32_t levels;
    int32_t remodulate;
};
void fovpt_launch_reconstruct(hipStream_t st, const FrameDev& fd, const ReconstructArgs& a, const fovpt_float4* in, const fovpt_float4* albedo,
                              GBufferDev g, fovpt_float4* out_color, uint32_t* out_rgba);
struct TemporalArgs {
    float inv[9];
    float eye_prev[3];
    int32_t cap[4];
    float normal_tol, depth_tol;
    int32_t reproject;
    int32_t uniform;
};
void fovpt_launch_temporal(hipStream_t st, const FrameDev& fd, const TemporalArgs& a, const fovpt_float4* in, GBufferDev g, GBufferDev gp,
                           const float4* hist_prev, float4* hist_out, fovpt_float4* out_color, uint32_t* out_rgba);
#define FOVPT_GATHER_BATCH 32
struct VertexGather {
    const float* src[FOVPT_GATHER_BATCH];
    uint32_t dst[FOVPT_GATHER_BATCH];
    uint32_t n[FOVPT_GATHER_BATCH];
    int32_t count;
    uint32_t max_n;
};
void fovpt_launch_gather_vertices(hipStream_t st, const VertexGather& g, float* vtx);
void fovpt_launch_refit(hipStream_t st, BvhNode4* nodes, TriRec* tris, const uint32_t* levels, uint32_t num_levels, const uint3* tri_vidx,
                        const float* vtx);
void fovpt_launch_flatten(hipStream_t st, uint32_t n, const uint3* tri_vidx, const float* vtx, float* flat);
void fovpt_launch_build_guide(hipStream_t st, const float* cdf, int n, int segments, uint32_t* guide);
void fovpt_launch_probe_records(hipStream_t st, size_t n, const float* cdfX, const float* pdfX, const float4* data, float4* rec);
void fovpt_launch_build_cdf(hipStream_t st, int w, int h, const float4* data, float* pdfX, float* cdfX, float* pdfY, float* cdfY, float* row_total);
void fovpt_launch_math(hipStream_t st, int op, const float* a, const float* b, float* out, size_t n);
```

fovpathtracing_optixcodelatest_amd/csrc/refit.hip:

```cpp
#include "fovpt_device.h"

namespace {

__device__ inline void tri_box(const float* p, float* lo, float* hi)
{
    float ext = 0.f, mag = 0.f;
    for (int a = 0; a < 3; a++) {
        const float x0 = p[a], x1 = p[3 + a], x2 = p[6 + a];
        lo[a] = fminf(x0, fminf(x1, x2)); hi[a] = fmaxf(x0, fmaxf(x1, x2));
        ext = fmaxf(ext, hi[a] - lo[a]);
        mag = fmaxf(mag, fmaxf(fabsf(lo[a]), fabsf(hi[a])));
    }
    const float pad = fovpt_tri_pad(ext, mag);
    for (int a = 0; a < 3; a++) { lo[a] -= pad; hi[a] += pad; }
}

__global__ void k_gather_vertices(VertexGather g, float* __restrict__ vtx)
{
    for (int u = blockIdx.y; u < g.count; u += gridDim.y) {
        const float* __restrict__ src = g.src[u];
        float* __restrict__ dst = vtx + 3 * (size_t)g.dst[u];
        const size_t n = 3 * (size_t)g.n[u];
        for (size_t i = (size_t)blockIdx.x * blockDim.x + threadIdx.x; i < n; i += (size_t)gridDim.x * blockDim.x) dst[i] = src[i];
    }
}

__global__ void k_refit_level(uint32_t first, uint32_t count, BvhNode4* __restrict__ nodes, TriRec* __restrict__ tris,
                              const uint3* __restrict__ tri_vidx, const float* __restrict__ vtx)
{
    const uint32_t t = blockIdx.x * blockDim.x + threadIdx.x;
    if (t >= 4u * count) return;
    float4* rec = reinterpret_cast<float4*>(&nodes[first + (t >> 2)].c[t & 3u]);
    const float4 r0 = rec[0], r1 = rec[1];
    if (!(r0.x < INFINITY)) return;
    const int32_t code = __float_as_int(r1.z);
    float lo[3] = {INFINITY, INFINITY, INFINITY}, hi[3] = {-INFINITY, -INFINITY, -INFINITY};
    if (code < 0) {
        const uint32_t lcode = (uint32_t)~code, n = (lcode & 7u) + 1u, t0 = (lcode >> 3) / 3u;
        for (uint32_t j = 0; j < n; j++) {
            float4* tr = reinterpret_cast<float4*>(&tris[t0 + j]);
            const float4 w2 = tr[2];
            const uint3 iv = tri_vidx[__float_as_uint(w2.y)];
            const uint32_t vi[3] = {iv.x, iv.y, iv.z};
            float p[9];
            for (int v = 0; v < 3; v++)
                for (int a = 0; a < 3; a++) p[3 * v + a] = vtx[3 * (size_t)vi[v] + a];
            tr[0] = make_float4(p[0], p[1], p[2], p[3] - p[0]);
            tr[1] = make_float4(p[4] - p[1], p[5] - p[2], p[6] - p[0], p[7] - p[1]);
            tr[2] = make_float4(p[8] - p[2], w2.y, w2.z, w2.w);
            float blo[3], bhi[3];
            tri_box(p, blo, bhi);
            for (int a = 0; a < 3; a++) { lo[a] = fminf(lo[a], blo[a]); hi[a] = fmaxf(hi[a], bhi[a]); }
        }
    } else {
        const float4* ch = reinterpret_cast<const float4*>(&nodes[code]);
        for (int k = 0; k < 4; k++) {
            const float4 c0 = ch[2 * k], c1 = ch[2 * k + 1];
            if (!(c0.x < INFINITY)) continue;
            lo[0] = fminf(lo[0], c0.x); lo[1] = fminf(lo[1], c0.y); lo[2] = fminf(lo[2], c0.z);
            hi[0] = fmaxf(hi[0], c0.w); hi[1] = fmaxf(hi[1], c1.x); hi[2] = fmaxf(hi[2], c1.y);
        }
    }
    rec[0] = make_float4(lo[0], lo[1], lo[2], hi[0]);
    rec[1] = make_float4(hi[1], hi[2], r1.z, r1.w);
}

__global__ void k_flatten(uint32_t n, const uint3* __restrict__ tri_vidx, const float* __restrict__ vtx, float* __restrict__ flat)
{
    const uint32_t i = blockIdx.x * blockDim.x + threadIdx.x;
    if (i >= n) return;
    const uint3 iv = tri_vidx[i];
    const uint32_t vi[3] = {iv.x, iv.y, iv.z};
    for (int v = 0; v < 3; v++)
        for (int a = 0; a < 3; a++) flat[9 * (size_t)i + 3 * v + a] = vtx[3 * (size_t)vi[v] + a];
}

}

void fovpt_launch_gather_vertices(hipStream_t st, const VertexGather& g, float* vtx)
{
    if (g.count <= 0 || g.max_n == 0) return;
    const uint64_t floats = 3ull * g.max_n;
    const uint32_t gx = (uint32_t)(floats < 1024ull * FOVPT_BLOCK ? (floats + FOVPT_BLOCK - 1) / FOVPT_BLOCK : 1024ull);
    hipLaunchKernelGGL(k_gather_vertices, dim3(gx, (uint32_t)g.count), dim3(FOVPT_BLOCK), 0, st, g, vtx);
}

void fovpt_launch_refit(hipStream_t st, BvhNode4* nodes, TriRec* tris, const uint32_t* levels, uint32_t num_levels, const uint3* tri_vidx,
                        const float* vtx)
{
    for (uint32_t L = num_levels; L-- > 0;) {
        const uint32_t first = levels[L], count = levels[L + 1] - first;
        if (count) hipLaunchKernelGGL(k_refit_level, dim3((4u * count + FOVPT_BLOCK - 1) / FOVPT_BLOCK), dim3(FOVPT_BLOCK), 0, st, first, count,
                                      nodes, tris, tri_vidx, vtx);
    }
}

void fovpt_launch_flatten(hipStream_t st, uint32_t n, const uint3* tri_vidx, const float* vtx, float* flat)
{
    if (n) hipLaunchKernelGGL(k_flatten, dim3((n + FOVPT_BLOCK - 1) / FOVPT_BLOCK), dim3(FOVPT_BLOCK), 0, st, n, tri_vidx, vtx, flat);
}
```

fovpathtracing_optixcodelatest_amd/csrc/wavefront.hip:

```cpp
#include "fovpt_device.h"
#include <hip/hip_ext.h>
#include "../../include/fovpt_detmath.h"
#include "fovpt_pixel.h"
#include "fovpt_scene.h"

#ifndef FOVPT_V_WAVES
#define FOVPT_V_WAVES 8
#endif

namespace {

#define kPi (3.141592653589793f)
#define k2Pi (3.141592653589793f * 2.0f)
#define kInvPi (1.0f / kPi)
#define kInv2Pi (1.0f / k2Pi)

__device__ inline uint32_t tea4(uint32_t v0, uint32_t v1)
{
    uint32_t s0 = 0;
#pragma unroll
    for (int n = 0; n < 4; n++) {
        s0 += 0x9e3779b9u;
        v0 += ((v1 << 4) + 0xa341316cu) ^ (v1 + s0) ^ ((v1 >> 5) + 0xc8013ea4u);
        v1 += ((v0 << 4) + 0xad90777du) ^ (v0 + s0) ^ ((v0 >> 5) + 0x7e95761eu);
    }
    return v0;
}
__device__ inline float rnd(uint32_t& prev)
{
    prev = 1664525u * prev + 1013904223u;
    return (float)(prev & 0x00FFFFFFu) / (float)0x01000000;
}
struct Rng {
    uint32_t s1, s2;
    __device__ inline uint32_t next()
    {
        s1 = (s2 ^ ((s1 << 5) | (s1 >> 27))) ^ (s1 * s2);
        s2 = s1 ^ ((s2 << 12) | (s2 >> 20));
        return s1;
    }
    __device__ inline float randf()
    {
        return clampf((float)next() * (1.0f / 4294967296.0f), 0.f, 0.999999f);
    }
    __device__ inline float randf01()
    {
        float t = randf();
        return (1.0f - t) * 0.0f + t * 1.0f;
    }
};

__device__ inline void probe_dir_to_uv(const V3& dir, float& u, float& v)
{
    float theta = fovpt_dm_acosf(clampf(dir.y, -1.0f, 1.0f));
    float phi = (dir.x == 0.0f && dir.z == 0.0f) ? 0.0f : fovpt_dm_atan2f(dir.z, dir.x);
    u = (kPi + phi) * kInvPi * 0.5f;
    v = theta * kInvPi;
}
__device__ inline float4 probe_eval(const fovpt_probe& pr, int row_mul, float u, float v)
{
    int px = max(0, min((int)(u * pr.width), pr.width - 1));
    int py = max(0, min((int)(v * pr.height), pr.height - 1));
    return ((const float4*)pr.data)[py * row_mul * pr.width + px];
}
__device__ inline int lower_bound(const float* __restrict__ a, int lower, int upper, float value)
{
    while (lower < upper) {
        int mid = lower + (upper - lower) / 2;
        if (a[mid] < value) lower = mid + 1;
        else upper = mid;
    }
    return lower;
}
template <int STRIDE>
__device__ inline int lower_bound_guided(const float* __restrict__ a, const uint32_t* __restrict__ guide, int base, int n, float value)
{
    const float fn = (float)n, inv = 1.0f / fn;
    int k = (int)(value * fn);
    k = max(0, min(k, n - 1));
    if ((float)k * inv > value) k = max(k - 1, 0);
    else if ((float)(k + 1) * inv <= value) k = min(k + 1, n - 1);
    const bool bracket = (float)k * inv <= value && value < (float)(k + 1) * inv;
    int lower = base + (bracket ? (int)guide[k] : 0);
    int upper = base + (bracket ? (int)guide[k + 1] : n);
    const int m = upper - lower;
    if (m <= 4) {
        if (m <= 0) return lower;
        const int last = upper - 1;
        const float v0 = a[(size_t)lower * STRIDE], v1 = a[(size_t)min(lower + 1, last) * STRIDE], v2 = a[(size_t)min(lower + 2, last) * STRIDE],
                    v3 = a[(size_t)min(lower + 3, last) * STRIDE];
        return lower + (int)(v0 < value) + (int)(m > 1 && v1 < value) + (int)(m > 2 && v2 < value) + (int)(m > 3 && v3 < value);
    }
    while (lower < upper) {
        int mid = lower + (upper - lower) / 2;
        if (a[(size_t)mid * STRIDE] < value) lower = mid + 1;
        else upper = mid;
    }
    return lower;
}
__device__ inline void probe_sample(const fovpt_probe& pr, const uint32_t* __restrict__ guide_x, const uint32_t* __restrict__ guide_y, const float4* __restrict__ rec,
                                    int row_mul, V3& dir, V3& color, float& pdf, Rng& rng)
{
    float r1 = rng.randf01();
    float r2 = rng.randf01();
    int row, col;
    if (guide_x) {
        row = lower_bound_guided<1>(pr.cdfValuesY, guide_y, 0, pr.height, r1);
        const int rx = row * row_mul;
        if (rec) col = lower_bound_guided<8>((const float*)rec, guide_x + (size_t)rx * (pr.width + 2), rx * pr.width, pr.width, r2) - rx * pr.width;
        else col = lower_bound_guided<1>(pr.cdfValuesX, guide_x + (size_t)rx * (pr.width + 2), rx * pr.width, pr.width, r2) - rx * pr.width;
    } else {
        row = lower_bound(pr.cdfValuesY, 0, pr.height, r1);
        const int rx = row * row_mul;
        col = lower_bound(pr.cdfValuesX, rx * pr.width, (rx + 1) * pr.width, r2) - rx * pr.width;
    }
    const int rowx = row * row_mul;
    if (guide_x && rec) {
        const float4 ra = rec[2 * (size_t)(rowx * pr.width + col)], rb = rec[2 * (size_t)(rowx * pr.width + col) + 1];
        color = v3(ra.z, ra.w, rb.x);
        pdf = ra.y * pr.pdfValuesY[row];
    } else {
        color = v3(((const float4*)pr.data)[rowx * pr.width + col]);
        pdf = pr.pdfValuesX[rowx * pr.width + col] * pr.pdfValuesY[row];
    }
    float u = col / float(pr.width);
    float v = row / float(pr.height);
    float sinTheta, cosTheta;
    fovpt_dm_sincos(v * kPi, &sinTheta, &cosTheta);
    if (sinTheta == 0.0f) pdf = 0.0f;
    else pdf *= pr.width * pr.height / (2.0f * kPi * kPi * sinTheta);
    float sinPhi, cosPhi;
    fovpt_dm_sincos(u * 2.0f * kPi, &sinPhi, &cosPhi);
    dir = v3(-sinTheta * cosPhi, cosTheta, -sinTheta * sinPhi);
}

typedef fovpt_material Mat;

__device__ inline float rcp_of_sqrt_as_the_reference(float x) { return (float)(1.0 / (double)sqrtf(x)); }
__device__ inline void basis_from_vector(const V3& w, V3& u, V3& v)
{
    if (fabsf(w.x) > fabsf(w.y)) {
        float invLen = rcp_of_sqrt_as_the_reference(w.x * w.x + w.z * w.z);
        u = v3(-w.z * invLen, 0.0f, w.x * invLen);
    } else {
        float invLen = rcp_of_sqrt_as_the_reference(w.y * w.y + w.z * w.z);
        u = v3(0.0f, w.z * invLen, -w.y * invLen);
    }
    v = cross(w, u);
}
__device__ inline V3 safe_normalize(const V3& a)
{
    float m = dot(a, a);
    if ((double)m > 0.0) return a * rcp_of_sqrt_as_the_reference(m);
    return v3(0.0f);
}
__device__ inline float half_plus_as_the_reference(float y) { return (float)(0.5 + (double)y); }
__device__ inline float schlick(float u)
{
    float m = clampf(1 - u, 0.0f, 1.0f);
    float m2 = m * m;
    return m2 * m2 * m;
}
__device__ inline float gtr1_pre(float NDotH, float a2, float log_a2)
{
    if (a2 < 0.0f) return kInvPi;
    float t = 1 + (a2 - 1) * NDotH * NDotH;
    return (a2 - 1) / (kPi * log_a2 * t);
}
__device__ inline float gtr2(float NDotH, float a)
{
    float a2 = a * a;
    float t = 1.0f + (a2 - 1.0f) * NDotH * NDotH;
    return a2 / (kPi * t * t);
}
__device__ inline float smith_ggx(float NDotv, float alphaG)
{
    float a = alphaG * alphaG;
    float b = NDotv * NDotv;
    return 1 / (NDotv + sqrtf(a + b - a * b));
}
__device__ inline float fresnel(float VDotN, float etaI, float etaT)
{
    float SinThetaT2 = sqr(etaI / etaT) * (1.0f - VDotN * VDotN);
    if (SinThetaT2 > 1.0f) return 1.0f;
    float LDotN = sqrtf(1.0f - SinThetaT2);
    float eta = etaT / etaI;
    float r1 = (VDotN - eta * LDotN) / (VDotN + eta * LDotN);
    float r2 = (LDotN - eta * VDotN) / (LDotN + eta * VDotN);
    return 0.5f * (sqr(r1) + sqr(r2));
}
struct BsdfView {
    float etaI, etaO;
    float NDotV;
    float FrV;
    float a;
    float GV_a, GV_q;
    float FV;
    V3 Cspec0;
    float cc_a2, cc_log;
};
__device__ inline BsdfView bsdf_view(const Mat& mat, const V3& albedo, float etaI, float etaO, const V3& N, const V3& V)
{
    BsdfView w;
    w.etaI = etaI; w.etaO = etaO;
    w.NDotV = dot(N, V);
    w.FrV = fresnel(w.NDotV, etaI, etaO);
    w.a = fmaxf(0.001f, mat.roughness);
    w.GV_a = smith_ggx(w.NDotV, w.a);
    w.GV_q = smith_ggx(w.NDotV, .25f);
    w.FV = schlick(w.NDotV);
    const V3 Cdlin = albedo;
    const float Cdlum = (float)(.3 * (double)Cdlin.x + .6 * (double)Cdlin.y + .1 * (double)Cdlin.z);
    const V3 Ctint = Cdlum > 0.0f ? div_vs(Cdlin, Cdlum) : v3(1.0f);
    w.Cspec0 = lerp3((float)((double)mat.specular * .08) * lerp3(v3(1.0f), Ctint, mat.specularTint), Cdlin, mat.metallic);
    const float cc_a = lerpf(.1f, .001f, mat.clearcoatGloss);
    w.cc_a2 = cc_a >= 1 ? -1.0f : cc_a * cc_a;
    w.cc_log = cc_a >= 1 ? 0.0f : fovpt_dm_logf(w.cc_a2);
    return w;
}
__device__ float bsdf_pdf(const Mat& mat, const BsdfView& w, const V3& n, const V3& V, const V3& L)
{
    if (dot(L, n) <= 0.0f) {
        float bsdfPdf = 0.0f;
        float brdfPdf = kInv2Pi * mat.subsurface * 0.5f;
        return lerpf(brdfPdf, bsdfPdf, mat.transmission);
    }
    const float F = w.FrV;
    const float a = w.a;
    const V3 half = safe_normalize(L + V);
    const float cosThetaHalf = fabsf(dot(half, n));
    const float pdfHalf = gtr2(cosThetaHalf, a) * cosThetaHalf;
    float pdfSpec = 0.25f * pdfHalf / fmaxf(1.e-6f, dot(L, half));
    float pdfDiff = fabsf(dot(L, n)) * kInvPi * (1.0f - mat.subsurface);
    float bsdfPdf = pdfSpec * F;
    float brdfPdf = lerpf(pdfDiff, pdfSpec, 0.5f);
    return lerpf(brdfPdf, bsdfPdf, mat.transmission);
}
__device__ float bsdf_sample(const Mat& mat, const BsdfView& w, const V3& U, const V3& V, const V3& N,
                             const V3& view, V3& light, Rng& rng)
{
    enum { SPECULAR, UNIFORM, COSINE };
    int kind;
    float r1, r2, z = 0.0f, angle;
    if (rng.randf() < mat.transmission) {
        const float F = w.FrV;
        if (rng.randf() < F) {
            r1 = rng.randf01();
            r2 = rng.randf01();
            kind = SPECULAR;
        } else {
            float eta = w.etaI / w.etaO;
            float cosThetaI = w.NDotV;
            float sin2ThetaI = fmaxf(0.0f, 1.0f - cosThetaI * cosThetaI);
            float sin2ThetaT = eta * eta * sin2ThetaI;
            if (sin2ThetaT >= 1) return 0.0f;
            float cosThetaT = sqrtf(1.0f - sin2ThetaT);
            light = eta * neg(view) + (eta * cosThetaI - cosThetaT) * N;
            return (1.0f - F) * mat.transmission;
        }
    } else {
        r1 = rng.randf01();
        r2 = rng.randf01();
        if (rng.randf() < 0.5f) {
            if (rng.randf() < mat.subsurface) { kind = UNIFORM; z = rng.randf01(); }
            else kind = COSINE;
        } else {
            kind = SPECULAR;
        }
    }
    if (kind == SPECULAR) angle = r1 * k2Pi;
    else if (kind == COSINE) angle = k2Pi * r2;
    else angle = k2Pi * rng.randf01();
    float sn, cs;
    fovpt_dm_sincos(angle, &sn, &cs);
    if (kind == SPECULAR) {
        const float a = w.a;
        const float cosThetaHalf = sqrtf((1.0f - r2) / (1.0f + (sqr(a) - 1.0f) * r2));
        const float sinThetaHalf = sqrtf(fmaxf(0.0f, 1.0f - sqr(cosThetaHalf)));
        V3 half = U * (sinThetaHalf * cs) + V * (sinThetaHalf * sn) + N * cosThetaHalf;
        if (dot(half, view) <= 0.0f) half = half * -1.0f;
        light = 2.0f * dot(view, half) * half - view;
    } else if (kind == UNIFORM) {
        const float ww = sqrtf(1.0f - z * z);
        const float x = cs * ww, y = sn * ww;
        light = U * x + V * y - N * z;
    } else {
        const float r = sqrtf(r1);
        const float sx = r * cs, sy = r * sn;
        const float zz = sqrtf(fmaxf(0.0f, 1.0f - sx * sx - sy * sy));
        light = U * sx + V * sy + N * zz;
    }
    return bsdf_pdf(mat, w, N, view, light);
}
__device__ V3 bsdf_eval(const Mat& mat, const V3& albedo, const BsdfView& w, const V3& N, const V3& V, const V3& L)
{
    float NDotL = dot(N, L);
    const float NDotV = w.NDotV;
    V3 H = normalize(L + V);
    float NDotH = dot(N, H);
    float LDotH = dot(L, H);
    const V3 Cdlin = albedo;
    const V3 Cspec0 = w.Cspec0;
    V3 bsdf = v3(0.0f);
    V3 brdf = v3(0.0f);
    float Ds = 0.0f, Gs = 0.0f;
    if (NDotL > 0) {
        Ds = gtr2(NDotH, w.a);
        Gs = w.GV_a * smith_ggx(NDotL, w.a);
    }
    if (mat.transmission > 0.0f) {
        if (NDotL <= 0) {
            const float F = w.FrV;
            bsdf = v3(mat.transmission * (1.0f - F) / fabsf(NDotL) * (1.0f - mat.metallic));
        } else {
            float FH = fresnel(LDotH, w.etaI, w.etaO);
            V3 Fs = lerp3(Cspec0, v3(1.0f), FH);
            bsdf = Gs * Fs * Ds;
        }
    }
    if (mat.transmission < 1.0f) {
        if (NDotL <= 0) {
            if (mat.subsurface > 0.0f) {
                V3 s = v3(sqrtf(mat.color.x), sqrtf(mat.color.y), sqrtf(mat.color.z));
                float FL = schlick(fabsf(NDotL)), FV = w.FV;
                float Fd = (1.0f - 0.5f * FL) * (1.0f - 0.5f * FV);
                brdf = kInvPi * s * mat.subsurface * Fd * (1.0f - mat.metallic);
            }
        } else {
            float FH = schlick(LDotH);
            V3 Fs = lerp3(Cspec0, v3(1.f), FH);
            float FL = schlick(NDotL), FV = w.FV;
            float Fd90 = half_plus_as_the_reference(2.0f * LDotH * LDotH * mat.roughness);
            float Fd = lerpf(1.0f, Fd90, FL) * lerpf(1.0f, Fd90, FV);
            float Dr = gtr1_pre(NDotH, w.cc_a2, w.cc_log);
            float Fc = lerpf(.04f, 1.0f, FH);
            float Gr = smith_ggx(NDotL, .25f) * w.GV_q;
            brdf = add_vs(kInvPi * Fd * Cdlin * (1.0f - mat.metallic) * (1.0f - mat.subsurface) + Gs * Fs * Ds,
                          mat.clearcoat * Gr * Fc * Dr);
        }
    }
    (void)NDotV;
    return lerp3(brdf, bsdf, mat.transmission);
}

__device__ inline uint32_t sel_first(uint32_t sel) { return sel == 2u ? 4u : 0u; }
__device__ inline uint32_t sel_mask(uint32_t sel) { return sel == 0u ? (uint32_t)FOVPT_SHARDS - 1u : 3u; }

__device__ inline uint32_t block_append(Counters* cnt, int word, uint32_t cap, bool pred, uint32_t* s_scratch , uint32_t sel = 0u)
{
    const unsigned long long mask = __ballot(pred);
    const uint32_t lane = __lane_id();
    const uint32_t wave = threadIdx.x >> 6;
    const uint32_t prefix = __popcll(mask & ((1ull << lane) - 1ull));
    if (lane == 0) s_scratch[wave] = (uint32_t)__popcll(mask);
    __syncthreads();
    const uint32_t c0 = s_scratch[0], c1 = s_scratch[1], c2 = s_scratch[2], c3 = s_scratch[3];
    const uint32_t shard = sel_first(sel) + (blockIdx.x & sel_mask(sel));
    if (threadIdx.x == 0) {
        const uint32_t total = c0 + c1 + c2 + c3;
        s_scratch[4] = total ? atomicAdd(&cnt->shard[shard][word], total) : 0u;
    }
    __syncthreads();
    const uint32_t before = (wave > 0 ? c0 : 0u) + (wave > 1 ? c1 : 0u) + (wave > 2 ? c2 : 0u);
    const uint32_t pos = shard * cap + s_scratch[4] + before + prefix;
    __syncthreads();
    return pos;
}

__device__ inline void block_append2(Counters* cnt, int word_a, bool pred_a, int word_b, bool pred_b, uint32_t cap,
                                     uint32_t* s_scratch , uint32_t& pos_a, uint32_t& pos_b, uint32_t sel = 0u)
{
    const unsigned long long ma = __ballot(pred_a), mb = __ballot(pred_b);
    const uint32_t lane = __lane_id();
    const uint32_t wave = threadIdx.x >> 6;
    const unsigned long long below = (1ull << lane) - 1ull;
    const uint32_t pa = __popcll(ma & below), pb = __popcll(mb & below);
    if (lane == 0) { s_scratch[wave] = (uint32_t)__popcll(ma); s_scratch[4 + wave] = (uint32_t)__popcll(mb); }
    __syncthreads();
    const uint32_t a0 = s_scratch[0], a1 = s_scratch[1], a2 = s_scratch[2], a3 = s_scratch[3];
    const uint32_t b0 = s_scratch[4], b1 = s_scratch[5], b2 = s_scratch[6], b3 = s_scratch[7];
    const uint32_t shard = sel_first(sel) + (blockIdx.x & sel_mask(sel));
    if (threadIdx.x == 0) {
        const uint32_t ta = a0 + a1 + a2 + a3;
        s_scratch[8] = ta ? atomicAdd(&cnt->shard[shard][word_a], ta) : 0u;
    }
    if (threadIdx.x == 64) {
        const uint32_t tb = b0 + b1 + b2 + b3;
        s_scratch[9] = tb ? atomicAdd(&cnt->shard[shard][word_b], tb) : 0u;
    }
    __syncthreads();
    pos_a = shard * cap + s_scratch[8] + (wave > 0 ? a0 : 0u) + (wave > 1 ? a1 : 0u) + (wave > 2 ? a2 : 0u) + pa;
    pos_b = shard * cap + s_scratch[9] + (wave > 0 ? b0 : 0u) + (wave > 1 ? b1 : 0u) + (wave > 2 ? b2 : 0u) + pb;
    __syncthreads();
}

__device__ inline void block_append2d(Counters* cnt, int word_a, bool pred_a, int word_b, bool pred_b, bool cls_b, uint32_t cap,
                                      uint32_t* s_scratch , uint32_t& pos_a, uint32_t& pos_b, uint32_t sel = 0u)
{
    const unsigned long long ma = __ballot(pred_a), mb0 = __ballot(pred_b & !cls_b), mb1 = __ballot(pred_b & cls_b);
    const uint32_t lane = __lane_id();
    const uint32_t wave = threadIdx.x >> 6;
    const unsigned long long below = (1ull << lane) - 1ull;
    const uint32_t pa = __popcll(ma & below), pb = __popcll((cls_b ? mb1 : mb0) & below);
    if (lane == 0) { s_scratch[wave] = (uint32_t)__popcll(ma); s_scratch[4 + wave] = (uint32_t)__popcll(mb0); s_scratch[8 + wave] = (uint32_t)__popcll(mb1); }
    __syncthreads();
    const uint32_t a0 = s_scratch[0], a1 = s_scratch[1], a2 = s_scratch[2], a3 = s_scratch[3];
    uint32_t before_b = 0u, tb0 = 0u, tb1 = 0u;
#pragma unroll
    for (uint32_t w = 0; w < 4u; w++) {
        const uint32_t b0 = s_scratch[4 + w], b1 = s_scratch[8 + w];
        if (w < wave) before_b += cls_b ? b1 : b0;
        tb0 += b0; tb1 += b1;
    }
    const uint32_t shard = sel_first(sel) + (blockIdx.x & sel_mask(sel));
    if (threadIdx.x == 0) {
        const uint32_t ta = a0 + a1 + a2 + a3;
        s_scratch[12] = ta ? atomicAdd(&cnt->shard[shard][word_a], ta) : 0u;
    }
    if (threadIdx.x == 64) s_scratch[13] = (tb0 + tb1) ? atomicAdd(&cnt->shard[shard][word_b], tb0 + tb1) : 0u;
    __syncthreads();
// ... 628 lines not shown
    if (MODE == 0) it_shadow = -1;
    if (MODE == 1) it_closest = -1;
    ShardMap ms, mq;
    if (MODE != 0) ms.load(cnt, FOVPT_CNT_SQ(it_shadow >= 0 ? it_shadow : 0), sel, cap);
    if (MODE != 1) mq.load(cnt, FOVPT_CNT_Q(it_closest >= 0 ? it_closest : 0), sel, cap);
    const uint32_t n_sh = (MODE != 0 && it_shadow >= 0) ? ms.total() : 0u;
    const uint32_t n_cl = (MODE != 1 && it_closest >= 0) ? mq.total() : 0u;
    if (blockIdx.x == 0 && threadIdx.x == 0) {
        if (n_cl) atomicAdd(&cnt->stat_radiance, (unsigned long long)n_cl);
        if (n_sh) atomicAdd(&cnt->stat_shadow, (unsigned long long)n_sh);
        if (it_closest == 0) atomicAdd(&cnt->stat_paths, (unsigned long long)n_cl);
    }
    QuadLane q;
    q.init();
    int* stack = s_stack + (threadIdx.x >> 2);
#if FOVPT_V_TOPLDS
    if (MODE != 1 && sc.num_nodes >= FOVPT_TOPN) {
        for (uint32_t k = threadIdx.x; k < FOVPT_TOPN * 8u; k += FOVPT_TBLOCK) s_top[k] = ((const float4*)sc.nodes)[k];
        __syncthreads();
    }
#endif
#if FOVPT_V_CYCLES
    if (threadIdx.x < 192) s_cyc_hist[threadIdx.x] = 0u;
    if (threadIdx.x == 0) s_cyc_last = 0u;
    __syncthreads();
    Cyc C;
    const uint32_t cyc_every = gridDim.x >= 512u ? gridDim.x / 256u : 1u;
    C.init(FOVPT_V_CYCLES != 3 && __builtin_amdgcn_readfirstlane((blockIdx.x % cyc_every == 0u && threadIdx.x < 64u) ? 1 : 0) != 0);
    const unsigned long long real0 = __builtin_amdgcn_s_memrealtime();
    const uint32_t life0 = cyc_stamp();
#endif
    if (n_sh) {
        const uint32_t nwaves = gridDim.x * (FOVPT_TBLOCK / 64), wave = blockIdx.x * (FOVPT_TBLOCK / 64) + (threadIdx.x >> 6);
        const uint32_t per = (n_sh + nwaves - 1u) / nwaves, first = min(n_sh, wave * per);
        traverse_shadow_pool(sc, ps, sq, ms, cap, first, min(n_sh, first + per), stack, q, cnt->diag[1] CYC_A);
    }
    const uint32_t quads = gridDim.x * FOVPT_TQUADS;
    for (uint32_t i = blockIdx.x * FOVPT_TQUADS + (threadIdx.x >> 2); i < n_cl; i += quads) {
        const uint32_t i0 = __builtin_amdgcn_readfirstlane(i - ((threadIdx.x & 63u) >> 2));
        RayT r;
        QuadTrav T;
        const uint32_t ph = mq.phys16(i, i0, cap);
        const float4 o = queue.o[ph], d = queue.d[ph];
        ray_setup(r, o, d);
        traverse_quad(sc, r, stack, q, T, cnt->diag[0] CYC_A);
        store_hit(ps, ph, T);
#if FOVPT_V_STEPSTAT
        if (q.j == 0) {
            ((uint32_t*)&queue.d[ph])[3] = T.steps;
            ps.trace[ph] = make_uint4((uint32_t)T.tr_lo, (uint32_t)(T.tr_lo >> 32), (uint32_t)T.tr_hi, (uint32_t)(T.tr_hi >> 32));
        }
#endif
    }
#if FOVPT_V_CYCLES
    {
        const uint32_t life1 = cyc_stamp();
        const unsigned long long real1 = __builtin_amdgcn_s_memrealtime();
        const int kind = it_shadow >= 0 ? 1 : 0, itn = (it_shadow >= 0 ? it_shadow : it_closest) & 3;
        const uint32_t wave = blockIdx.x * (FOVPT_TBLOCK / 64) + (threadIdx.x >> 6);
        if ((threadIdx.x & 63u) == 0u && wave < 32768u) { cnt->wtime[kind * 4 + itn][wave][0] = real0; cnt->wtime[kind * 4 + itn][wave][1] = real1; }
        if (C.on) {
            unsigned long long* g = cnt->cyc[kind][itn];
            const uint32_t v[9] = {C.n_node, C.gap, C.load, C.alu, C.lds, C.n_leaf, C.lgap, C.lload, C.lrest};
#pragma unroll
            for (int k = 0; k < 9; k++) if (v[k]) atomicAdd(g + k, (unsigned long long)v[k]);
            if ((threadIdx.x & 63u) == 0u) {
                const uint32_t x = cyc_stamp(), y = cyc_stamp();
                atomicAdd(g + 9, (unsigned long long)(y - x)); atomicAdd(g + 10, 1ull);
                atomicAdd(g + 11, (unsigned long long)(life1 - life0)); atomicAdd(g + 12, (unsigned long long)(real1 - real0)); atomicAdd(g + 13, 1ull);
            }
        }
        if (FOVPT_V_CYCLES >= 2 && C.on && threadIdx.x < 64u)
            for (uint32_t k = threadIdx.x; k < 192u; k += 64u) if (s_cyc_hist[k]) atomicAdd(&cnt->hist[kind][itn][k >> 6][k & 63u], s_cyc_hist[k]);
    }
#endif
}

#define FLAG_DONE 1u
#define FLAG_SECONDARY 2u

#define FLAG_ALPHA_ONE 4u
#define FLAG_ALPHA_SET 8u

#ifndef FOVPT_V_SHADEWAVES
#define FOVPT_V_SHADEWAVES 1
#endif
template <bool EXTRA>
__global__ __launch_bounds__(FOVPT_BLOCK, FOVPT_V_SHADEWAVES) void k_shade(const FrameDev fd, SceneView sc, PathState ps,
                                                       RayQueue queue_in, RayQueue queue_out,
                                                       ShadowQueue sq, uint32_t cap, Counters* __restrict__ cnt, int depth_iter, uint32_t sel)
{
    __shared__ uint32_t s_scratch[14];
    ShardMap mq;
    mq.load(cnt, FOVPT_CNT_Q(depth_iter), sel, cap);
    const uint32_t n = mq.total();
    const uint32_t nround = (n + FOVPT_BLOCK - 1) / FOVPT_BLOCK * FOVPT_BLOCK;
    for (uint32_t i = blockIdx.x * FOVPT_BLOCK + threadIdx.x; i < nround; i += gridDim.x * FOVPT_BLOCK) {
        bool want_shadow = false, want_next = false;
        uint32_t slot = 0;
        V3 next_o = v3(0.f), next_d = v3(0.f);
        float next_pdf = 0.f;
        float4 sh_o, sh_d, sh_vis, sh_occ;
        sh_o = sh_d = sh_vis = sh_occ = make_float4(0.f, 0.f, 0.f, 0.f);
        if (i < n) {
            const uint32_t ph = mq.phys(i, cap);
            const float4 o4 = queue_in.o[ph], d4 = queue_in.d[ph];
            slot = __float_as_uint(o4.w);
            const float4 hit = ps.hit[ph];
            const uint32_t tpos = __float_as_uint(hit.w);
            uint4 rs = ps.rng[slot];
            uint32_t flags = rs.z & 0xffu;
            int depth = (int)(rs.z >> 8);
            if (tpos == 0xffffffffu) {
                flags |= FLAG_DONE;
                if (EXTRA && (fd.options & FOVPT_OPT_SKY_MISS) && (flags & FLAG_SECONDARY) && depth < fd.max_depth) {
                    const V3 dir = v3(d4);
                    const float bsdfPdf = d4.w;
                    const V3 thr = v3(ps.thr[slot]);
                    float u, v;
                    probe_dir_to_uv(dir, u, v);
                    const fovpt_probe& pr = fd.probe;
                    const int col = max(0, min((int)(u * pr.width), pr.width - 1));
                    const int row = max(0, min((int)(v * pr.height), pr.height - 1));
                    float skyPdf = pr.pdfValuesX[row * fd.probe_row_mul * pr.width + col] * pr.pdfValuesY[row];
                    const float sinTheta = fovpt_dm_sinf(v * kPi);
                    if (fabsf(sinTheta) < 0.0001f) skyPdf = 0.0f;
                    else skyPdf *= float(pr.width) * float(pr.height) / (2.0f * kPi * kPi * sinTheta);
                    const float weight = 0.5f * bsdfPdf / (0.5f * bsdfPdf + 0.5f * skyPdf);
                    const V3 rad = v3(0.f) + (weight * v3(probe_eval(pr, fd.probe_row_mul, u, v))) * thr;
                    ps.rad[(size_t)slot * ps.stride + depth] = f4(rad, 0.f);
                    depth += 1;
                }
            } else {
                const V3 ray_o = v3(o4), ray_dir = v3(d4);
                Rng rng_probe; rng_probe.s1 = rs.x; rng_probe.s2 = rs.y;
                V3 wi, skyColor; float skyPdf;
                probe_sample(fd.probe, fd.guide_x, fd.guide_y, fd.probe_rec, fd.probe_row_mul, wi, skyColor, skyPdf, rng_probe);
                const float4 thr_in = ps.thr[slot];
                const TriRec T = load_tri_off(sc.tris, tpos << 4);
                const MeshDev M = sc.meshes[T.mesh];
                const Mat& mat = M.material;
                const V3 e1 = v3(T.e1x, T.e1y, T.e1z), e2 = v3(T.e2x, T.e2y, T.e2z);
                const V3 N_0 = normalize(cross(e1, e2));
                const V3 wo = neg(ray_dir);
                const V3 N = N_0 * copysignf(1.0f, dot(wo, N_0));
                const V3 P = ray_o + hit.x * ray_dir;
                const bool catcher = (mat.flags & FOVPT_MATERIAL_FLAG_SHADOW_CATCHER) != 0;
                if (catcher && (flags & FLAG_SECONDARY)) {
                    next_o = P; next_d = ray_dir; next_pdf = d4.w;
                    want_next = true;
                } else if (depth >= fd.max_depth) {
                    flags |= FLAG_ALPHA_ONE | FLAG_DONE;
                } else {
                    const float4 t4 = (flags & FLAG_SECONDARY) ? thr_in : make_float4(1.f, 1.f, 1.f, 1.0f);
                    V3 thr = v3(t4);
                    float rayEta = t4.w;
                    Rng rng = rng_probe;
                    V3 albedo = v3(mat.color);
                    if (M.texture_id >= 0 && M.has_texcoord) {
                        const float2* tc = sc.tri_tc + (size_t)T.prim * 3;
                        const float2 t0 = tc[0], t1 = tc[1], t2 = tc[2];
                        const float w0 = 1.f - hit.y - hit.z;
                        const float tcx = (w0 * t0.x + hit.y * t1.x) + hit.z * t2.x;
                        const float tcy = (w0 * t0.y + hit.y * t1.y) + hit.z * t2.y;
                        albedo = v3(tex2d(M.tex, tcx, tcy));
                    }
                    if (ps.guide_n && depth == 0 && (flags & FLAG_SECONDARY) == 0) {
                        ps.guide_n[slot] = f4(N, 0.f);
                        ps.guide_a[slot] = f4(albedo, 0.f);
                    }
                    float outEta;
                    if (rayEta == 1.0f)
                        outEta = (mat.eta == 0.0f) ? 2.0f / (1.0f - sqrtf(0.08f * mat.specular)) - 1.0f : mat.eta;
                    else
                        outEta = 1.0f;
                    const BsdfView view = bsdf_view(mat, albedo, rayEta, outEta, N, wo);
                    V3 sum_hit = v3(0.0f);
                    {
                        const float bsdfPdf = bsdf_pdf(mat, view, N, wo, wi);
                        const V3 f = bsdf_eval(mat, albedo, view, N, wo, wi);
                        if (bsdfPdf > 0.0f) {
                            const float weight = 0.5f * skyPdf / (0.5f * bsdfPdf + 0.5f * skyPdf);
                            if (weight > 0.0f) {
                                const V3 val = div_vs(weight * skyColor * f * fabsf(dot(wi, N)), skyPdf) * (1.0f / 1.f);
                                sum_hit = sum_hit + val;
                            }
                        }
                    }
                    const V3 sum_zero = v3(0.0f);
                    V3 rad_vis, rad_occ;
                    V3 alpha_vis = v3(0.f), alpha_occ = v3(0.f);
                    bool alpha_set_one = false;
                    if (!catcher) {
                        rad_vis = v3(0.f) + thr * sum_hit;
                        rad_occ = v3(0.f) + thr * sum_zero;
                        alpha_set_one = true;
                    } else {
                        rad_vis = v3(0.f); rad_occ = v3(0.f);
                        alpha_vis = thr * sum_zero;
                        alpha_occ = thr * sum_hit;
                    }
                    if ((flags & FLAG_SECONDARY) == 0) {
                        rad_vis = rad_vis + v3(mat.emission);
                        rad_occ = rad_occ + v3(mat.emission);
                    }
                    V3 bu, bv;
                    basis_from_vector(N, bu, bv);
                    V3 bsdfDir = v3(0.f);
                    const float bsdfPdf = bsdf_sample(mat, view, bu, bv, N, wo, bsdfDir, rng);
                    if (alpha_set_one) flags |= FLAG_ALPHA_ONE;
                    const bool same = rad_vis.x == rad_occ.x && rad_vis.y == rad_occ.y && rad_vis.z == rad_occ.z
                                   && alpha_vis.x == alpha_occ.x && alpha_vis.y == alpha_occ.y && alpha_vis.z == alpha_occ.z;
                    if (catcher) {
                        flags |= FLAG_ALPHA_SET;
                        if (same) ps.alpha[slot] = f4(v3(0.f) + alpha_occ, 0.f);
                        else {
                            want_shadow = true;
                            sh_o = f4(P, __uint_as_float(slot)); sh_d = f4(wi, __uint_as_float(0xffffffffu));
                            sh_vis = f4(v3(0.f) + alpha_vis, 0.f); sh_occ = f4(v3(0.f) + alpha_occ, 0.f);
                        }
                    }
                    if (bsdfPdf <= 0.0f) {
                        flags |= FLAG_DONE;
                    } else {
                        float4* cell = ps.rad + ((size_t)slot * ps.stride + depth);
                        if (!catcher && !same) {
                            want_shadow = true;
                            sh_o = f4(P, __uint_as_float(slot)); sh_d = f4(wi, __uint_as_float((uint32_t)depth));
                            sh_vis = f4(rad_vis, 0.f); sh_occ = f4(rad_occ, 0.f);
                        } else {
                            *cell = f4(rad_occ, 0.f);
                        }
                        flags |= FLAG_SECONDARY;
                        depth += 1;
                        if (depth < fd.max_depth || sc.any_catcher) {
                            const V3 f = bsdf_eval(mat, albedo, view, N, wo, bsdfDir);
                            if (dot(bsdfDir, N) <= 0.0f) rayEta = outEta;
                            thr = thr * div_vs(f * fabsf(dot(N, bsdfDir)), bsdfPdf);
                            bool rr_kill = false;
                            if (EXTRA && (fd.options & FOVPT_OPT_RUSSIAN_ROULETTE) && depth >= 2) {
                                const float q = fmaxf(0.05f, fminf(1.0f, fmaxf(thr.x, fmaxf(thr.y, thr.z))));
                                if (rng.randf() >= q) rr_kill = true;
                                else thr = thr * (1.0f / q);
                            }
                            if (!rr_kill) {
                                next_o = P; next_d = bsdfDir; next_pdf = bsdfPdf;
                                ps.thr[slot] = f4(thr, rayEta);
                                want_next = true;
                            }
                        }
                    }
                    rs.x = rng.s1; rs.y = rng.s2;
                }
            }
            rs.z = flags | ((uint32_t)depth << 8);
            ps.rng[slot] = rs;
        }
        uint32_t spos, qpos;
        if (fd.partition)
            block_append2d(cnt, FOVPT_CNT_SQ(depth_iter), want_shadow, FOVPT_CNT_Q(depth_iter + 1), want_next, next_d.y > 0.0f, cap, s_scratch, spos, qpos, sel);
        else
            block_append2(cnt, FOVPT_CNT_SQ(depth_iter), want_shadow, FOVPT_CNT_Q(depth_iter + 1), want_next, cap, s_scratch, spos, qpos, sel);
        if (want_shadow) { sq.o[spos] = sh_o; sq.d[spos] = sh_d; sq.val_vis[spos] = sh_vis; sq.val_occ[spos] = sh_occ; }
        if (want_next) { queue_out.o[qpos] = f4(next_o, __uint_as_float(slot)); queue_out.d[qpos] = f4(next_d, next_pdf); }
    }
}

__global__ __launch_bounds__(FOVPT_BLOCK) void k_resolve(const FrameDev fd, PathState ps, Counters* __restrict__ cnt)
{
    if (!FOVPT_V_STEPSTAT && blockIdx.x == 0 && blockIdx.y == 0) {
        uint32_t* w = &cnt->shard[0][0];
        for (uint32_t i = threadIdx.x; i < FOVPT_SHARDS * FOVPT_SHARD_STRIDE; i += FOVPT_BLOCK) w[i] = 0u;
    }
    __shared__ uint32_t s_key[FOVPT_BLOCK];
    __shared__ uint32_t s_idx[FOVPT_BLOCK];
    __shared__ uint32_t s_list_li[FOVPT_BLOCK];
    __shared__ uint32_t s_list_p[FOVPT_BLOCK];
    __shared__ float4 s_accum[FOVPT_BLOCK];
    __shared__ uint32_t s_rgba[FOVPT_BLOCK];
    __shared__ float4 s_gn[FOVPT_BLOCK], s_ga[FOVPT_BLOCK];
    __shared__ uint32_t s_wave[4];

    const uint32_t tx = threadIdx.x & 63, ty = threadIdx.x >> 6;
    const uint32_t x = blockIdx.x * 64 + tx;
    const uint32_t y = blockIdx.y * 4 + ty;
    const bool inside = x < (uint32_t)fd.w && y < (uint32_t)fd.h;
    const uint32_t image_index = y * (uint32_t)fd.w + x;

    int state = 0;
    int wp = 0;
    uint32_t wli = 0, key = 0xffffffffu;
    if (inside) {
        uint32_t wlx, wly;
        if (find_last_writer(fd, x, y, wp, wlx, wly)) {
            const PassDev& P = fd.pass[wp];
            state = launch_owned(fd, wp, wlx, wly) ? 1 : 2;
            wli = (wly - P.row0) * P.gw + wlx;
            key = P.launch_base + wli;
        }
    }
    if (state != 1) key = 0xffffffffu;
    s_key[threadIdx.x] = key;
    __syncthreads();

    const bool leader = state == 1 && (tx == 0 || s_key[threadIdx.x - 1] != key);
    const unsigned long long lm = __ballot(leader);
    if (tx == 0) s_wave[ty] = (uint32_t)__popcll(lm);
    __syncthreads();
    uint32_t base = 0;
    for (uint32_t w = 0; w < ty; w++) base += s_wave[w];
    const uint32_t nlist = s_wave[0] + s_wave[1] + s_wave[2] + s_wave[3];
    if (leader) {
        const uint32_t pos = base + (uint32_t)__popcll(lm & ((1ull << tx) - 1ull));
        s_idx[threadIdx.x] = pos;
        s_list_li[pos] = wli;
        s_list_p[pos] = (uint32_t)wp;
    }
    __syncthreads();

// ... 82 lines not shown
    if ((int)threadIdx.x < fd.world) block_count[(size_t)blockIdx.x * fd.world + threadIdx.x] = s_cnt[threadIdx.x];
}
__global__ __launch_bounds__(1024) void k_plan_scan(uint32_t nblocks, int world, uint32_t* __restrict__ block_count, uint32_t* __restrict__ total)
{
    __shared__ uint32_t s_part[1024];
    const int r = (int)blockIdx.x;
    if (r >= world) return;
    const uint32_t per = (nblocks + blockDim.x - 1u) / blockDim.x;
    const uint32_t b0 = min(nblocks, threadIdx.x * per), b1 = min(nblocks, b0 + per);
    uint32_t sum = 0u;
    for (uint32_t b = b0; b < b1; b++) sum += block_count[(size_t)b * world + r];
    s_part[threadIdx.x] = sum;
    __syncthreads();
    for (uint32_t off = 1u; off < blockDim.x; off <<= 1) {
        const uint32_t v = threadIdx.x >= off ? s_part[threadIdx.x - off] : 0u;
        __syncthreads();
        s_part[threadIdx.x] += v;
        __syncthreads();
    }
    uint32_t run = s_part[threadIdx.x] - sum;
    for (uint32_t b = b0; b < b1; b++) {
        const uint32_t c = block_count[(size_t)b * world + r];
        block_count[(size_t)b * world + r] = run;
        run += c;
    }
    if (threadIdx.x == blockDim.x - 1u) total[r] = s_part[threadIdx.x];
}
__global__ __launch_bounds__(FOVPT_BLOCK) void k_plan_fill(uint32_t npix, int world, const uint8_t* __restrict__ owner, const uint32_t* __restrict__ block_off,
                                                          const uint32_t* __restrict__ rank_base, uint32_t* __restrict__ idx)
{
    __shared__ uint32_t s_cnt[FOVPT_BLOCK / 64][64];
    const uint32_t i = blockIdx.x * FOVPT_BLOCK + threadIdx.x, wave = threadIdx.x >> 6, lane = threadIdx.x & 63u;
    const uint32_t o = i < npix ? owner[i] : FOVPT_PLAN_NOBODY;
    for (uint32_t k = threadIdx.x; k < (FOVPT_BLOCK / 64) * 64; k += FOVPT_BLOCK) (&s_cnt[0][0])[k] = 0u;
    __syncthreads();
    uint32_t in_wave = 0u;
    unsigned long long todo = __ballot(o != FOVPT_PLAN_NOBODY);
    while (todo) {
        const uint32_t leader = (uint32_t)__builtin_ctzll(todo);
        const uint32_t lo = (uint32_t)__builtin_amdgcn_readlane((int)o, (int)leader);
        const unsigned long long same = __ballot(o == lo);
        if (o == lo) in_wave = (uint32_t)__popcll(same & ((1ull << lane) - 1ull));
        if (lane == leader) s_cnt[wave][lo] = (uint32_t)__popcll(same);
        todo &= ~same;
    }
    __syncthreads();
    if (o == FOVPT_PLAN_NOBODY) return;
    uint32_t before = in_wave;
    for (uint32_t w = 0; w < wave; w++) before += s_cnt[w][o];
    idx[rank_base[o] + block_off[(size_t)blockIdx.x * world + o] + before] = i;
}
__global__ void k_gather_pack(uint32_t n, const uint32_t* __restrict__ idx, const uint32_t* __restrict__ frame, uint32_t* __restrict__ packed)
{
    for (uint32_t i = blockIdx.x * blockDim.x + threadIdx.x; i < n; i += gridDim.x * blockDim.x) packed[i] = frame[idx[i]];
}
__global__ void k_gather_unpack(int world, uint32_t stride, const uint32_t* __restrict__ base, const uint32_t* __restrict__ idx,
                                const uint32_t* __restrict__ gathered, uint32_t* __restrict__ frame)
{
    const uint32_t total = base[world];
    for (uint32_t i = blockIdx.x * blockDim.x + threadIdx.x; i < total; i += gridDim.x * blockDim.x) {
        int r = 0;
        while (r + 1 < world && i >= base[r + 1]) r++;
        frame[idx[i]] = gathered[(size_t)r * stride + (i - base[r])];
    }
}

__global__ void k_build_guide(const float* __restrict__ cdf, int n, int segments, uint32_t* __restrict__ guide)
{
    const size_t i = (size_t)blockIdx.x * blockDim.x + threadIdx.x;
    const size_t total = (size_t)segments * (n + 2);
    if (i >= total) return;
    const int seg = (int)(i / (n + 2)), m = (int)(i - (size_t)seg * (n + 2));
    const float value = (float)m * (1.0f / (float)n);
    guide[i] = (uint32_t)(lower_bound(cdf, seg * n, (seg + 1) * n, value) - seg * n);
}

__global__ void k_probe_records(size_t n, const float* __restrict__ cdfX, const float* __restrict__ pdfX, const float4* __restrict__ data, float4* __restrict__ rec)
{
    const size_t i = (size_t)blockIdx.x * blockDim.x + threadIdx.x;
    if (i >= n) return;
    const float4 c = data[i];
    rec[2 * i] = make_float4(cdfX[i], pdfX[i], c.x, c.y);
    rec[2 * i + 1] = make_float4(c.z, 0.f, 0.f, 0.f);
}

#define CDF_ROWS 8
#define CDF_COLS 256
#define CDF_LD (CDF_COLS + 4)
__global__ __launch_bounds__(CDF_COLS) void k_cdf_rows(int w, int h, const float4* __restrict__ data, float* __restrict__ pdfX, float* __restrict__ cdfX,
                                                      float* __restrict__ row_total)
{
    __shared__ __attribute__((aligned(16))) float s_w[CDF_ROWS][CDF_LD], s_c[CDF_ROWS][CDF_LD];
    const int j0 = blockIdx.x * CDF_ROWS, t = threadIdx.x;
    float run = 0.0f;
    float4 c[CDF_ROWS];
#pragma unroll
    for (int r = 0; r < CDF_ROWS; r++) c[r] = (j0 + r < h && t < w) ? data[(size_t)(j0 + r) * w + t] : make_float4(0.f, 0.f, 0.f, 0.f);
    for (int i0 = 0; i0 < w; i0 += CDF_COLS) {
#pragma unroll
        for (int r = 0; r < CDF_ROWS; r++) s_w[r][t] = c[r].x * 0.3f + c[r].y * 0.6f + c[r].z * 0.1f;
        __syncthreads();
        const int in = i0 + CDF_COLS + t;
#pragma unroll
        for (int r = 0; r < CDF_ROWS; r++) c[r] = (j0 + r < h && in < w) ? data[(size_t)(j0 + r) * w + in] : make_float4(0.f, 0.f, 0.f, 0.f);
        if (t < CDF_ROWS && j0 + t < h) {
            const int n = min(CDF_COLS, w - i0);
            int k = 0;
            for (; k + 4 <= n; k += 4) {
                const float4 v = *(const float4*)&s_w[t][k];
                float4 o;
                run += v.x; o.x = run; run += v.y; o.y = run; run += v.z; o.z = run; run += v.w; o.w = run;
                *(float4*)&s_c[t][k] = o;
            }
            for (; k < n; k++) { run += s_w[t][k]; s_c[t][k] = run; }
        }
        __syncthreads();
#pragma unroll
        for (int r = 0; r < CDF_ROWS; r++) {
            const int j = j0 + r, i = i0 + t;
            if (j < h && i < w) { pdfX[(size_t)j * w + i] = s_w[r][t]; cdfX[(size_t)j * w + i] = s_c[r][t]; }
        }
        __syncthreads();
    }
    if (t < CDF_ROWS && j0 + t < h) row_total[j0 + t] = run;
}
__global__ void k_cdf_rows_scale(int w, int h, float* __restrict__ pdfX, float* __restrict__ cdfX, const float* __restrict__ row_total)
{
    const size_t k = (size_t)blockIdx.x * blockDim.x + threadIdx.x;
    if (k >= (size_t)w * h) return;
    const float invTotalWeightX = 1.0f / row_total[k / (size_t)w];
    pdfX[k] *= invTotalWeightX;
    cdfX[k] *= invTotalWeightX;
}
__global__ __launch_bounds__(256) void k_cdf_cols(int h, const float* __restrict__ row_total, float* __restrict__ pdfY, float* __restrict__ cdfY)
{
    __shared__ __attribute__((aligned(16))) float s_v[2048], s_c[2048];
    __shared__ float s_total;
    if (blockIdx.x != 0) return;
    float totalWeightY = 0.0f;
    for (int j0 = 0; j0 < h; j0 += 2048) {
        const int n = min(2048, h - j0);
        for (int k = (int)threadIdx.x; k < n; k += (int)blockDim.x) s_v[k] = row_total[j0 + k];
        __syncthreads();
        if (threadIdx.x == 0) {
            int k = 0;
            for (; k + 4 <= n; k += 4) {
                const float4 v = *(const float4*)&s_v[k];
                float4 o;
                totalWeightY += v.x; o.x = totalWeightY; totalWeightY += v.y; o.y = totalWeightY;
                totalWeightY += v.z; o.z = totalWeightY; totalWeightY += v.w; o.w = totalWeightY;
                *(float4*)&s_c[k] = o;
            }
            for (; k < n; k++) { totalWeightY += s_v[k]; s_c[k] = totalWeightY; }
        }
        __syncthreads();
        for (int k = (int)threadIdx.x; k < n; k += (int)blockDim.x) { pdfY[j0 + k] = s_v[k]; cdfY[j0 + k] = s_c[k]; }
        __syncthreads();
    }
    if (threadIdx.x == 0) s_total = totalWeightY;
    __syncthreads();
    const float total = s_total;
    for (int j = (int)threadIdx.x; j < h; j += (int)blockDim.x) {
        cdfY[j] /= total;
        pdfY[j] /= total;
    }
}

__global__ void k_math(int op, const float* a, const float* b, float* out, size_t n)
{
    size_t i = (size_t)blockIdx.x * blockDim.x + threadIdx.x;
    if (i >= n) return;
    float r = 0.f;
    switch (op) {
    case FOVPT_OP_SIN: r = fovpt_dm_sinf(a[i]); break;
    case FOVPT_OP_COS: r = fovpt_dm_cosf(a[i]); break;
    case FOVPT_OP_ACOS: r = fovpt_dm_acosf(a[i]); break;
    case FOVPT_OP_ATAN2: r = fovpt_dm_atan2f(a[i], b[i]); break;
    case FOVPT_OP_LOG: r = fovpt_dm_logf(a[i]); break;
    case FOVPT_OP_POW: r = fovpt_dm_powf(a[i], b[i]); break;
    case FOVPT_OP_SQRT: r = sqrtf(a[i]); break;
    case FOVPT_OP_DIV: r = a[i] / b[i]; break;
    case FOVPT_OP_RSQRTD: r = rcp_of_sqrt_as_the_reference(a[i]); break;
    case FOVPT_OP_HALFPLUS: r = half_plus_as_the_reference(a[i]); break;
    case FOVPT_OP_UNORM8: r = unorm8((uint32_t)a[i] & 255u); break;
    }
    out[i] = r;
}

}

void fovpt_launch_generate(hipStream_t st, const FrameDev& fd, PathState ps, RayQueue queue0, uint32_t cap, Counters* cnt, uint32_t slot_begin,
                           uint32_t slot_end, int grid, uint32_t sel)
{
    unsigned long long space = 0;
    for (int p = 0; p < fd.npass && p < FOVPT_MAX_PASSES; p++) {
        OwnedSpace o;
        o.init(fd, fd.pass[p]);
        space += ((unsigned long long)o.tile_rows * o.per_row * o.tile_lis * fd.pass[p].spp + FOVPT_BLOCK - 1u) / FOVPT_BLOCK * FOVPT_BLOCK;
    }
    if (FOVPT_V_GEN_OWNED && fd.world > 1 && sel == 0u && slot_begin == 0u && slot_end == fd.total_slots && space <= (unsigned long long)fd.total_slots)
        hipLaunchKernelGGL(k_generate_owned, dim3(grid), dim3(FOVPT_BLOCK), 0, st, fd, ps, queue0, cap, cnt);
    else
        hipLaunchKernelGGL(k_generate, dim3(grid), dim3(FOVPT_BLOCK), 0, st, fd, ps, queue0, cap, cnt, slot_begin, slot_end, sel);
}
void fovpt_launch_traverse(hipStream_t st, SceneView sc, PathState ps, RayQueue queue, ShadowQueue sq, uint32_t cap,
                           Counters* cnt, int it_closest, int it_shadow, int grid, hipEvent_t done, uint32_t sel)
{
    int blocks = grid * FOVPT_BLOCK / FOVPT_TBLOCK > 0 ? grid * FOVPT_BLOCK / FOVPT_TBLOCK : 1;
    if (it_shadow < 0) {
        const unsigned long long rounds = ((sel ? 4ull : 8ull) * cap + FOVPT_TQUADS - 1) / FOVPT_TQUADS;
        if ((unsigned long long)blocks > rounds) blocks = (int)((rounds + FOVPT_SHARDS - 1) / FOVPT_SHARDS * FOVPT_SHARDS);
    }
    auto kernel = it_shadow < 0 ? k_traverse<0> : it_closest < 0 ? k_traverse<1> : k_traverse<2>;
    if (done) hipExtLaunchKernelGGL(kernel, dim3(blocks), dim3(FOVPT_TBLOCK), 0, st, nullptr, done, 0, sc, ps, queue, sq, cap, cnt, it_closest, it_shadow, sel);
    else hipLaunchKernelGGL(kernel, dim3(blocks), dim3(FOVPT_TBLOCK), 0, st, sc, ps, queue, sq, cap, cnt, it_closest, it_shadow, sel);
}
void fovpt_launch_shade(hipStream_t st, const FrameDev& fd, SceneView sc, PathState ps, RayQueue queue_in, RayQueue queue_out,
                        ShadowQueue sq, uint32_t cap, Counters* cnt, int depth, int grid, hipEvent_t done, uint32_t sel)
{
    if (fd.options) {
        if (done) hipExtLaunchKernelGGL(k_shade<true>, dim3(grid), dim3(FOVPT_BLOCK), 0, st, nullptr, done, 0, fd, sc, ps, queue_in, queue_out, sq, cap, cnt, depth, sel);
        else hipLaunchKernelGGL(k_shade<true>, dim3(grid), dim3(FOVPT_BLOCK), 0, st, fd, sc, ps, queue_in, queue_out, sq, cap, cnt, depth, sel);
    } else {
        if (done) hipExtLaunchKernelGGL(k_shade<false>, dim3(grid), dim3(FOVPT_BLOCK), 0, st, nullptr, done, 0, fd, sc, ps, queue_in, queue_out, sq, cap, cnt, depth, sel);
        else hipLaunchKernelGGL(k_shade<false>, dim3(grid), dim3(FOVPT_BLOCK), 0, st, fd, sc, ps, queue_in, queue_out, sq, cap, cnt, depth, sel);
    }
}
void fovpt_launch_resolve(hipStream_t st, const FrameDev& fd, PathState ps, Counters* cnt, hipEvent_t done)
{
    dim3 grid((fd.w + 63) / 64, (fd.h + 3) / 4);
    if (done) hipExtLaunchKernelGGL(k_resolve, grid, dim3(FOVPT_BLOCK), 0, st, nullptr, done, 0, fd, ps, cnt);
    else hipLaunchKernelGGL(k_resolve, grid, dim3(FOVPT_BLOCK), 0, st, fd, ps, cnt);
}
void fovpt_launch_plan_owner(hipStream_t st, const FrameDev& fd, uint8_t* owner, uint32_t* block_count, uint32_t nblocks)
{
    hipLaunchKernelGGL(k_plan_owner, dim3(nblocks), dim3(FOVPT_BLOCK), 0, st, fd, owner, block_count);
}
void fovpt_launch_plan_scan_fill(hipStream_t st, uint32_t npix, uint32_t nblocks, int world, const uint8_t* owner, uint32_t* block_count,
                                 uint32_t* total, const uint32_t* rank_base, uint32_t* idx, int phase)
{
    if (phase == 0) hipLaunchKernelGGL(k_plan_scan, dim3(world), dim3(1024), 0, st, nblocks, world, block_count, total);
    else hipLaunchKernelGGL(k_plan_fill, dim3(nblocks), dim3(FOVPT_BLOCK), 0, st, npix, world, owner, block_count, rank_base, idx);
}
void fovpt_launch_gather_pack(hipStream_t st, uint32_t n, const uint32_t* idx, const uint32_t* frame, uint32_t* packed)
{
    if (n) hipLaunchKernelGGL(k_gather_pack, dim3((n + 255u) / 256u < 2048u ? (n + 255u) / 256u : 2048u), dim3(256), 0, st, n, idx, frame, packed);
}
void fovpt_launch_gather_unpack(hipStream_t st, int world, uint32_t stride, uint32_t total, const uint32_t* base, const uint32_t* idx,
                                const uint32_t* gathered, uint32_t* frame)
{
    if (total) hipLaunchKernelGGL(k_gather_unpack, dim3((total + 255u) / 256u < 2048u ? (total + 255u) / 256u : 2048u), dim3(256), 0, st, world, stride, base, idx, gathered, frame);
}
void fovpt_launch_build_guide(hipStream_t st, const float* cdf, int n, int segments, uint32_t* guide)
{
    const size_t total = (size_t)segments * (n + 2);
    hipLaunchKernelGGL(k_build_guide, dim3((unsigned)((total + 255) / 256)), dim3(256), 0, st, cdf, n, segments, guide);
}
void fovpt_launch_probe_records(hipStream_t st, size_t n, const float* cdfX, const float* pdfX, const float4* data, float4* rec)
{
    hipLaunchKernelGGL(k_probe_records, dim3((unsigned)((n + 255) / 256)), dim3(256), 0, st, n, cdfX, pdfX, data, rec);
}
void fovpt_launch_build_cdf(hipStream_t st, int w, int h, const float4* data, float* pdfX, float* cdfX, float* pdfY, float* cdfY, float* row_total)
{
    hipLaunchKernelGGL(k_cdf_rows, dim3((h + CDF_ROWS - 1) / CDF_ROWS), dim3(CDF_COLS), 0, st, w, h, data, pdfX, cdfX, row_total);
    hipLaunchKernelGGL(k_cdf_rows_scale, dim3((unsigned)(((size_t)w * h + 255) / 256)), dim3(256), 0, st, w, h, pdfX, cdfX, row_total);
    hipLaunchKernelGGL(k_cdf_cols, dim3(1), dim3(256), 0, st, h, row_total, pdfY, cdfY);
}
void fovpt_launch_math(hipStream_t st, int op, const float* a, const float* b, float* out, size_t n)
{
    hipLaunchKernelGGL(k_math, dim3((unsigned)((n + 255) / 256)), dim3(256), 0, st, op, a, b, out, n);
}
```

Baseline: 4611 Mray/s.

## Precompute per-triangle normals and compact per-mesh shading records for the shade kernel

Adds a 32-byte per-triangle TriShade record holding the precomputed geometric normal plus prim and mesh ids, built during BVH emit and refit. It also adds a compact 64-byte ShadeMesh record with derived material constants (clamped roughness, output eta, clearcoat terms) and a separate rarely-read record for emission and sqrt(color). The shade kernel reads these instead of the 48-byte TriRec and the full MeshDev, which removes a cross product, a normalize and per-hit material derivations, and cuts the bytes loaded per hit. The probe sampling inverse sizes are precomputed and specialised by template. The cost is extra scene memory and extra writes during build and refit.

```diff
diff --git a/fovpathtracing_optixcodelatest_amd/csrc/bvh_build.hip b/fovpathtracing_optixcodelatest_amd/csrc/bvh_build.hip
--- a/fovpathtracing_optixcodelatest_amd/csrc/bvh_build.hip
+++ b/fovpathtracing_optixcodelatest_amd/csrc/bvh_build.hip
@@ -681,7 +681,8 @@
 }
 
 __global__ void k_emit_tris_generic(const float* __restrict__ flat, const uint32_t* __restrict__ mesh_of_prim, const uint32_t* __restrict__ vals,
-                                    const uint32_t* __restrict__ ref_prim, const uint32_t* __restrict__ leaf_pos, uint32_t n, TriRec* __restrict__ tris)
+                                    const uint32_t* __restrict__ ref_prim, const uint32_t* __restrict__ leaf_pos, uint32_t n, TriRec* __restrict__ tris,
+                                    TriShade* __restrict__ tri_shade)
 {
     uint32_t i = blockIdx.x * blockDim.x + threadIdx.x;
     if (i >= n) return;
@@ -693,6 +694,7 @@
     t.e2x = p[6] - p[0]; t.e2y = p[7] - p[1]; t.e2z = p[8] - p[2];
     t.prim = prim; t.mesh = mesh_of_prim[prim]; t.pad = 0;
     tris[leaf_pos[i]] = t;
+    tri_shade[leaf_pos[i]] = fovpt_tri_shade(t.e1x, t.e1y, t.e1z, t.e2x, t.e2y, t.e2z, t.prim, t.mesh);
 }
 
 #define FOVPT_SPLIT_MAX 8
@@ -820,6 +822,7 @@
     uint32_t* counters = nullptr;
     BvhNode4* nodes = nullptr;
     TriRec* tris = nullptr;
+    TriShade* tri_shade = nullptr;
     const int B = 256;
     uint32_t ni = 1, gn = 1, gi = 1;
     bool have_boxes = false;
@@ -903,6 +906,7 @@
     HC(hipMalloc(&size_int, 4ull * ni)); HC(hipMalloc(&leaf_pos, 4ull * n)); HC(hipMalloc(&node_first, 4ull * ni));
     HC(hipMalloc(&nodes, sizeof(BvhNode4) * ni));
     HC(hipMalloc(&tris, sizeof(TriRec) * n));
+    HC(hipMalloc(&tri_shade, sizeof(TriShade) * n));
     HC(hipMemsetAsync(stats, 0, 8, st));
     if (!have_boxes) {
         HC(hipMemcpyAsync(bounds, h_bounds, sizeof(h_bounds), hipMemcpyHostToDevice, st));
@@ -1043,7 +1047,7 @@
             if (++levels > 4096) { snprintf(err, errlen, "BVH collapse did not terminate"); goto fail; }
         }
     }
-    hipLaunchKernelGGL(k_emit_tris_generic, dim3(gn), dim3(B), 0, st, flat, mesh_of_prim, vals_s, ref_prim, leaf_pos, n, tris);
+    hipLaunchKernelGGL(k_emit_tris_generic, dim3(gn), dim3(B), 0, st, flat, mesh_of_prim, vals_s, ref_prim, leaf_pos, n, tris, tri_shade);
     HC(hipGetLastError());
     if (order_children && level_first.size() >= 2) {
         const uint32_t total = level_first.back();
@@ -1060,17 +1064,20 @@
     {
         const size_t node_bytes = sizeof(BvhNode4) * (size_t)h_stats[1], tri_bytes = sizeof(TriRec) * (size_t)n;
         const size_t tri_off = (node_bytes + 255) & ~(size_t)255;
+        const size_t shade_off = (tri_off + tri_bytes + 64 + 255) & ~(size_t)255, shade_bytes = sizeof(TriShade) * (size_t)n;
         char* scene = nullptr;
-        HC(hipMalloc(&scene, tri_off + tri_bytes + 64));
+        HC(hipMalloc(&scene, shade_off + shade_bytes));
         if (hipMemcpyAsync(scene, nodes, node_bytes, hipMemcpyDeviceToDevice, st) != hipSuccess
             || hipMemcpyAsync(scene + tri_off, tris, tri_bytes, hipMemcpyDeviceToDevice, st) != hipSuccess
-            || hipMemsetAsync(scene + tri_off + tri_bytes, 0, 64, st) != hipSuccess
+            || hipMemsetAsync(scene + tri_off + tri_bytes, 0, shade_off - (tri_off + tri_bytes), st) != hipSuccess
+            || hipMemcpyAsync(scene + shade_off, tri_shade, shade_bytes, hipMemcpyDeviceToDevice, st) != hipSuccess
             || hipStreamSynchronize(st) != hipSuccess) {
             (void)hipFree(scene);
             snprintf(err, errlen, "copying the hierarchy failed");
             goto fail;
         }
         out->nodes = (BvhNode4*)scene; out->tris = (TriRec*)(scene + tri_off);
+        out->tri_shade = (TriShade*)(scene + shade_off);
         out->num_nodes = h_stats[1];
         out->num_refs = n;
         out->max_depth = h_stats[0];
@@ -1086,7 +1093,7 @@
     (void)hipFree(ref_prim); (void)hipFree(split_cnt); (void)hipFree(split_first); (void)hipFree(split_total); (void)hipFree(split_temp);
     (void)hipFree(boxes); (void)hipFree(ibox); (void)hipFree(bounds); (void)hipFree(stats); (void)hipFree(keys); (void)hipFree(keys_s);
     (void)hipFree(vals); (void)hipFree(vals_s); (void)hipFree(arrive); (void)hipFree(left); (void)hipFree(right); (void)hipFree(parent_int);
-    (void)hipFree(parent_leaf); (void)hipFree(rfirst); (void)hipFree(rlast); (void)hipFree(temp); (void)hipFree(nodes); (void)hipFree(tris);
+    (void)hipFree(parent_leaf); (void)hipFree(rfirst); (void)hipFree(rlast); (void)hipFree(temp); (void)hipFree(nodes); (void)hipFree(tris); (void)hipFree(tri_shade);
     (void)hipFree(c_node); (void)hipFree(t_node); (void)hipFree(nn); (void)hipFree(c_box); (void)hipFree(t_box); (void)hipFree(valid); (void)hipFree(pos);
     (void)hipFree(node_counter); (void)hipFree(size_int); (void)hipFree(leaf_pos); (void)hipFree(node_first); (void)hipFree(node_depth);
     (void)hipFree(dp); (void)hipFree(dp_arrive); (void)hipFree(order_pc);
diff --git a/fovpathtracing_optixcodelatest_amd/csrc/fovpt_api.hip b/fovpathtracing_optixcodelatest_amd/csrc/fovpt_api.hip
--- a/fovpathtracing_optixcodelatest_amd/csrc/fovpt_api.hip
+++ b/fovpathtracing_optixcodelatest_amd/csrc/fovpt_api.hip
@@ -86,7 +86,9 @@
     uint64_t scene_id = 0;
     BvhNode4* nodes = nullptr;
     TriRec* tris = nullptr;
+    TriShade* tri_shade = nullptr;
     DevBuf tri_tc, meshes, textures;
+    DevBuf shade_meshes, shade_rare;
     std::vector<void*> tex_pixels;
     uint32_t num_tris = 0, any_catcher = 0;
     uint32_t bvh_levels[FOVPT_BVH_MAX_LEVELS + 1] = {};
@@ -223,7 +225,7 @@
 void free_scene(fovpt_ctx* c)
 {
     if (c->nodes) (void)hipFree(c->nodes);
-    c->nodes = nullptr; c->tris = nullptr;
+    c->nodes = nullptr; c->tris = nullptr; c->tri_shade = nullptr;
     for (void* p : c->tex_pixels) (void)hipFree(p);
     c->tex_pixels.clear();
     c->has_scene = false;
@@ -263,6 +265,7 @@
     SceneView sc;
     sc.nodes = c->nodes; sc.tris = c->tris; sc.tri_tc = (const float2*)c->tri_tc.p;
     sc.meshes = (const MeshDev*)c->meshes.p; sc.textures = (const TexDev*)c->textures.p;
+    sc.tri_shade = c->tri_shade; sc.shade_meshes = (const ShadeMesh*)c->shade_meshes.p; sc.shade_rare = (const ShadeMeshRare*)c->shade_rare.p;
     sc.num_tris = c->num_tris; sc.any_catcher = c->any_catcher;
     sc.tri_off = (uint32_t)((const char*)c->tris - (const char*)c->nodes);
     sc.num_nodes = c->stats.num_bvh_nodes;
@@ -356,6 +359,7 @@
     fd.guide_y = own_probe ? (const uint32_t*)c->pr_guidey.p : nullptr;
     fd.probe_rec = (own_probe && !c->rows_identical && lp->probe.data == (fovpt_float4*)c->pr_data.p && lp->probe.pdfValuesX == (float*)c->pr_pdfx.p)
                    ? (const float4*)c->pr_rec.p : nullptr;
+    fd.probe_inv_w = 1.0f / (float)lp->probe.width; fd.probe_inv_h = 1.0f / (float)lp->probe.height;
     fd.probe_row_mul = (c->rows_identical && lp->probe.data == (fovpt_float4*)c->pr_data.p && lp->probe.pdfValuesX == (float*)c->pr_pdfx.p
                         && lp->probe.cdfValuesX == (float*)c->pr_cdfx.p && lp->probe.width == c->guide_w && lp->probe.height == c->guide_h) ? 0 : 1;
     fd.accum = lp->frame.accum_buffer;
@@ -676,7 +680,7 @@
 
 void adopt_hierarchy(fovpt_ctx* c, const BvhBuildResult& br, float ms)
 {
-    c->nodes = br.nodes; c->tris = br.tris;
+    c->nodes = br.nodes; c->tris = br.tris; c->tri_shade = br.tri_shade;
     c->num_tris = br.num_refs;
     c->bvh_num_levels = br.num_levels;
     memcpy(c->bvh_levels, br.level_first, sizeof(c->bvh_levels));
@@ -771,6 +775,7 @@
     (void)fovpt_comm_destroy(c);
     free_scene(c);
     DevBuf* bufs[] = {&c->tri_tc, &c->meshes, &c->textures, &c->pr_data, &c->pr_pdfx, &c->pr_cdfx, &c->pr_pdfy, &c->pr_cdfy, &c->pr_guidex, &c->pr_guidey, &c->pr_rec,
+                      &c->shade_meshes, &c->shade_rare,
                       &c->fb_frame, &c->fb_accum, &c->fb_color, &c->fb_normal, &c->fb_albedo, &c->accum_before,
                       &c->plan_owner, &c->plan_blocks, &c->plan_total, &c->plan_base, &c->plan_idx,
                       &c->comm_packed, &c->comm_gathered, &c->dn_level, &c->dn_i0, &c->dn_i1, &c->dn_color, &c->dn_rgba,
@@ -875,6 +880,11 @@
     }
     HIPCHK(c, c->meshes.reserve(md.size() * sizeof(MeshDev)));
     HIPCHK(c, hipMemcpy(c->meshes.p, md.data(), md.size() * sizeof(MeshDev), hipMemcpyHostToDevice));
+    HIPCHK(c, c->shade_meshes.reserve(md.size() * sizeof(ShadeMesh)));
+    HIPCHK(c, c->shade_rare.reserve(md.size() * sizeof(ShadeMeshRare)));
+    fovpt_launch_shade_meshes(c->stream, num_meshes, (const MeshDev*)c->meshes.p, (ShadeMesh*)c->shade_meshes.p, (ShadeMeshRare*)c->shade_rare.p);
+    HIPCHK(c, hipGetLastError());
+    HIPCHK(c, hipStreamSynchronize(c->stream));
 
     BvhBuildResult br;
     float ms = 0.f;
@@ -957,7 +967,7 @@
         S.pending = true;
     }
     if (!rebuild) {
-        fovpt_launch_refit(st, c->nodes, c->tris, c->bvh_levels, c->bvh_num_levels, (const uint3*)c->up_vidx.p, vtx);
+        fovpt_launch_refit(st, c->nodes, c->tris, c->tri_shade, c->bvh_levels, c->bvh_num_levels, (const uint3*)c->up_vidx.p, vtx);
         HIPCHK(c, hipGetLastError());
         HIPCHK(c, hipEventRecord(c->ev_scene, st));
         c->refit_pending = true;
@@ -1716,6 +1726,9 @@
     if (!c || !name || !ptr || !bytes) return FOVPT_E_INVALID;
     if (strcmp(name, "bvh_nodes") == 0 && c->has_scene) { *ptr = c->nodes; *bytes = (size_t)c->stats.bvh_bytes; return FOVPT_OK; }
     if (strcmp(name, "bvh_tris") == 0 && c->has_scene) { *ptr = c->tris; *bytes = (size_t)c->stats.tri_bytes; return FOVPT_OK; }
+    if (strcmp(name, "tri_shade") == 0 && c->has_scene) { *ptr = c->tri_shade; *bytes = (size_t)c->num_tris * sizeof(TriShade); return FOVPT_OK; }
+    if (strcmp(name, "shade_meshes") == 0 && c->has_scene) { *ptr = c->shade_meshes.p; *bytes = c->mesh_nv.size() * sizeof(ShadeMesh); return FOVPT_OK; }
+    if (strcmp(name, "shade_rare") == 0 && c->has_scene) { *ptr = c->shade_rare.p; *bytes = c->mesh_nv.size() * sizeof(ShadeMeshRare); return FOVPT_OK; }
     if (strcmp(name, "scene_vertices") == 0 && c->up_vtx.p) { *ptr = c->up_vtx.p; *bytes = c->h_vtx.size() * 4; return FOVPT_OK; }
     StateSet& S = c->set[c->last_set];
     struct { const char* n; DevBuf* b; } tab[] = {
diff --git a/fovpathtracing_optixcodelatest_amd/csrc/fovpt_device.h b/fovpathtracing_optixcodelatest_amd/csrc/fovpt_device.h
--- a/fovpathtracing_optixcodelatest_amd/csrc/fovpt_device.h
+++ b/fovpathtracing_optixcodelatest_amd/csrc/fovpt_device.h
@@ -57,6 +57,23 @@
 };
 static_assert(sizeof(TriRec) == 48, "TriRec");
 
+struct alignas(32) TriShade {
+    float nx, ny, nz;
+    uint32_t prim;
+    uint32_t mesh;
+    uint32_t pad[3];
+};
+static_assert(sizeof(TriShade) == 32, "TriShade");
+__device__ inline TriShade fovpt_tri_shade(float e1x, float e1y, float e1z, float e2x, float e2y, float e2z, uint32_t prim, uint32_t mesh)
+{
+    const float cx = e1y * e2z - e1z * e2y, cy = e1z * e2x - e1x * e2z, cz = e1x * e2y - e1y * e2x;
+    const float invLen = 1.0f / sqrtf(cx * cx + cy * cy + cz * cz);
+    TriShade s;
+    s.nx = cx * invLen; s.ny = cy * invLen; s.nz = cz * invLen;
+    s.prim = prim; s.mesh = mesh; s.pad[0] = s.pad[1] = s.pad[2] = 0u;
+    return s;
+}
+
 struct alignas(16) BvhChild {
     float lox, loy, loz, hix;
     float hiy, hiz;
@@ -79,6 +96,27 @@
     int32_t has_texcoord;
     TexDev tex;
 };
+
+struct alignas(64) ShadeMesh {
+    float color[3];
+    float roughness;
+    float a;
+    float transmission, metallic, subsurface;
+    float specularTint, clearcoat;
+    float spec08;
+    float out_eta;
+    float cc_a2, cc_log;
+    float one_minus_metallic;
+    uint32_t bits;
+};
+static_assert(sizeof(ShadeMesh) == 64, "ShadeMesh");
+#define FOVPT_SHADE_CATCHER 1u
+#define FOVPT_SHADE_TEXTURED 2u
+struct alignas(32) ShadeMeshRare {
+    float emission[3], pad0;
+    float sqrt_color[3], pad1;
+};
+static_assert(sizeof(ShadeMeshRare) == 32, "ShadeMeshRare");
 
 struct SceneView {
     const BvhNode4* nodes;
@@ -86,6 +124,9 @@
     const float2* tri_tc;
     const MeshDev* meshes;
     const TexDev* textures;
+    const TriShade* tri_shade;
+    const ShadeMesh* shade_meshes;
+    const ShadeMeshRare* shade_rare;
     uint32_t num_tris;
     uint32_t any_catcher;
     uint32_t tri_off;
@@ -119,6 +160,7 @@
     const uint32_t* guide_y;
     const float4* probe_rec;
     int32_t probe_row_mul;
+    float probe_inv_w, probe_inv_h;
     fovpt_float4* accum;
     const fovpt_float4* accum_prev;
     uint32_t* frame;
@@ -183,6 +225,7 @@
 struct BvhBuildResult {
     BvhNode4* nodes;
     TriRec* tris;
+    TriShade* tri_shade;
     uint32_t num_nodes;
     uint32_t num_refs;
     uint32_t max_depth;
@@ -250,10 +293,11 @@
     uint32_t max_n;
 };
 void fovpt_launch_gather_vertices(hipStream_t st, const VertexGather& g, float* vtx);
-void fovpt_launch_refit(hipStream_t st, BvhNode4* nodes, TriRec* tris, const uint32_t* levels, uint32_t num_levels, const uint3* tri_vidx,
-                        const float* vtx);
+void fovpt_launch_refit(hipStream_t st, BvhNode4* nodes, TriRec* tris, TriShade* tri_shade, const uint32_t* levels, uint32_t num_levels,
+                        const uint3* tri_vidx, const float* vtx);
 void fovpt_launch_flatten(hipStream_t st, uint32_t n, const uint3* tri_vidx, const float* vtx, float* flat);
 void fovpt_launch_build_guide(hipStream_t st, const float* cdf, int n, int segments, uint32_t* guide);
 void fovpt_launch_probe_records(hipStream_t st, size_t n, const float* cdfX, const float* pdfX, const float4* data, float4* rec);
+void fovpt_launch_shade_meshes(hipStream_t st, int n, const MeshDev* meshes, ShadeMesh* out, ShadeMeshRare* rare);
 void fovpt_launch_build_cdf(hipStream_t st, int w, int h, const float4* data, float* pdfX, float* cdfX, float* pdfY, float* cdfY, float* row_total);
 void fovpt_launch_math(hipStream_t st, int op, const float* a, const float* b, float* out, size_t n);
diff --git a/fovpathtracing_optixcodelatest_amd/csrc/refit.hip b/fovpathtracing_optixcodelatest_amd/csrc/refit.hip
--- a/fovpathtracing_optixcodelatest_amd/csrc/refit.hip
+++ b/fovpathtracing_optixcodelatest_amd/csrc/refit.hip
@@ -26,7 +26,7 @@
 }
 
 __global__ void k_refit_level(uint32_t first, uint32_t count, BvhNode4* __restrict__ nodes, TriRec* __restrict__ tris,
-                              const uint3* __restrict__ tri_vidx, const float* __restrict__ vtx)
+                              TriShade* __restrict__ tri_shade, const uint3* __restrict__ tri_vidx, const float* __restrict__ vtx)
 {
     const uint32_t t = blockIdx.x * blockDim.x + threadIdx.x;
     if (t >= 4u * count) return;
@@ -48,6 +48,8 @@
             tr[0] = make_float4(p[0], p[1], p[2], p[3] - p[0]);
             tr[1] = make_float4(p[4] - p[1], p[5] - p[2], p[6] - p[0], p[7] - p[1]);
             tr[2] = make_float4(p[8] - p[2], w2.y, w2.z, w2.w);
+            tri_shade[t0 + j] = fovpt_tri_shade(p[3] - p[0], p[4] - p[1], p[5] - p[2], p[6] - p[0], p[7] - p[1], p[8] - p[2],
+                                                __float_as_uint(w2.y), __float_as_uint(w2.z));
             float blo[3], bhi[3];
             tri_box(p, blo, bhi);
             for (int a = 0; a < 3; a++) { lo[a] = fminf(lo[a], blo[a]); hi[a] = fmaxf(hi[a], bhi[a]); }
@@ -85,13 +87,13 @@
     hipLaunchKernelGGL(k_gather_vertices, dim3(gx, (uint32_t)g.count), dim3(FOVPT_BLOCK), 0, st, g, vtx);
 }
 
-void fovpt_launch_refit(hipStream_t st, BvhNode4* nodes, TriRec* tris, const uint32_t* levels, uint32_t num_levels, const uint3* tri_vidx,
-                        const float* vtx)
+void fovpt_launch_refit(hipStream_t st, BvhNode4* nodes, TriRec* tris, TriShade* tri_shade, const uint32_t* levels, uint32_t num_levels,
+                        const uint3* tri_vidx, const float* vtx)
 {
     for (uint32_t L = num_levels; L-- > 0;) {
         const uint32_t first = levels[L], count = levels[L + 1] - first;
         if (count) hipLaunchKernelGGL(k_refit_level, dim3((4u * count + FOVPT_BLOCK - 1) / FOVPT_BLOCK), dim3(FOVPT_BLOCK), 0, st, first, count,
-                                      nodes, tris, tri_vidx, vtx);
+                                      nodes, tris, tri_shade, tri_vidx, vtx);
     }
 }
 
diff --git a/fovpathtracing_optixcodelatest_amd/csrc/wavefront.hip b/fovpathtracing_optixcodelatest_amd/csrc/wavefront.hip
--- a/fovpathtracing_optixcodelatest_amd/csrc/wavefront.hip
+++ b/fovpathtracing_optixcodelatest_amd/csrc/wavefront.hip
@@ -73,9 +73,9 @@
     return lower;
 }
 template <int STRIDE>
-__device__ inline int lower_bound_guided(const float* __restrict__ a, const uint32_t* __restrict__ guide, int base, int n, float value)
-{
-    const float fn = (float)n, inv = 1.0f / fn;
+__device__ inline int lower_bound_guided(const float* __restrict__ a, const uint32_t* __restrict__ guide, int base, int n, float inv, float value)
+{
+    const float fn = (float)n;
     int k = (int)(value * fn);
     k = max(0, min(k, n - 1));
     if ((float)k * inv > value) k = max(k - 1, 0);
@@ -98,24 +98,28 @@
     }
     return lower;
 }
-__device__ inline void probe_sample(const fovpt_probe& pr, const uint32_t* __restrict__ guide_x, const uint32_t* __restrict__ guide_y, const float4* __restrict__ rec,
-                                    int row_mul, V3& dir, V3& color, float& pdf, Rng& rng)
-{
+template <bool OWN>
+__device__ inline void probe_sample(const FrameDev& fd, V3& dir, V3& color, float& pdf, Rng& rng)
+{
+    const fovpt_probe& pr = fd.probe;
+    const float4* __restrict__ rec = fd.probe_rec;
+    const int row_mul = fd.probe_row_mul;
     float r1 = rng.randf01();
     float r2 = rng.randf01();
     int row, col;
-    if (guide_x) {
-        row = lower_bound_guided<1>(pr.cdfValuesY, guide_y, 0, pr.height, r1);
+    if (OWN) {
+        row = lower_bound_guided<1>(pr.cdfValuesY, fd.guide_y, 0, pr.height, fd.probe_inv_h, r1);
         const int rx = row * row_mul;
-        if (rec) col = lower_bound_guided<8>((const float*)rec, guide_x + (size_t)rx * (pr.width + 2), rx * pr.width, pr.width, r2) - rx * pr.width;
-        else col = lower_bound_guided<1>(pr.cdfValuesX, guide_x + (size_t)rx * (pr.width + 2), rx * pr.width, pr.width, r2) - rx * pr.width;
+        const uint32_t* __restrict__ gx = fd.guide_x + (size_t)rx * (pr.width + 2);
+        if (rec) col = lower_bound_guided<8>((const float*)rec, gx, rx * pr.width, pr.width, fd.probe_inv_w, r2) - rx * pr.width;
+        else col = lower_bound_guided<1>(pr.cdfValuesX, gx, rx * pr.width, pr.width, fd.probe_inv_w, r2) - rx * pr.width;
     } else {
         row = lower_bound(pr.cdfValuesY, 0, pr.height, r1);
         const int rx = row * row_mul;
         col = lower_bound(pr.cdfValuesX, rx * pr.width, (rx + 1) * pr.width, r2) - rx * pr.width;
     }
     const int rowx = row * row_mul;
-    if (guide_x && rec) {
+    if (OWN && rec) {
         const float4 ra = rec[2 * (size_t)(rowx * pr.width + col)], rb = rec[2 * (size_t)(rowx * pr.width + col) + 1];
         color = v3(ra.z, ra.w, rb.x);
         pdf = ra.y * pr.pdfValuesY[row];
@@ -134,7 +138,7 @@
     dir = v3(-sinTheta * cosPhi, cosTheta, -sinTheta * sinPhi);
 }
 
-typedef fovpt_material Mat;
+typedef ShadeMesh Mat;
 
 __device__ inline float rcp_of_sqrt_as_the_reference(float x) { return (float)(1.0 / (double)sqrtf(x)); }
 __device__ inline void basis_from_vector(const V3& w, V3& u, V3& v)
@@ -193,11 +197,9 @@
     float etaI, etaO;
     float NDotV;
     float FrV;
-    float a;
     float GV_a, GV_q;
     float FV;
     V3 Cspec0;
-    float cc_a2, cc_log;
 };
 __device__ inline BsdfView bsdf_view(const Mat& mat, const V3& albedo, float etaI, float etaO, const V3& N, const V3& V)
 {
@@ -205,17 +207,13 @@
     w.etaI = etaI; w.etaO = etaO;
     w.NDotV = dot(N, V);
     w.FrV = fresnel(w.NDotV, etaI, etaO);
-    w.a = fmaxf(0.001f, mat.roughness);
-    w.GV_a = smith_ggx(w.NDotV, w.a);
+    w.GV_a = smith_ggx(w.NDotV, mat.a);
     w.GV_q = smith_ggx(w.NDotV, .25f);
     w.FV = schlick(w.NDotV);
     const V3 Cdlin = albedo;
     const float Cdlum = (float)(.3 * (double)Cdlin.x + .6 * (double)Cdlin.y + .1 * (double)Cdlin.z);
     const V3 Ctint = Cdlum > 0.0f ? div_vs(Cdlin, Cdlum) : v3(1.0f);
-    w.Cspec0 = lerp3((float)((double)mat.specular * .08) * lerp3(v3(1.0f), Ctint, mat.specularTint), Cdlin, mat.metallic);
-    const float cc_a = lerpf(.1f, .001f, mat.clearcoatGloss);
-    w.cc_a2 = cc_a >= 1 ? -1.0f : cc_a * cc_a;
-    w.cc_log = cc_a >= 1 ? 0.0f : fovpt_dm_logf(w.cc_a2);
+    w.Cspec0 = lerp3(mat.spec08 * lerp3(v3(1.0f), Ctint, mat.specularTint), Cdlin, mat.metallic);
     return w;
 }
 __device__ float bsdf_pdf(const Mat& mat, const BsdfView& w, const V3& n, const V3& V, const V3& L)
@@ -226,7 +224,7 @@
         return lerpf(brdfPdf, bsdfPdf, mat.transmission);
     }
     const float F = w.FrV;
-    const float a = w.a;
+    const float a = mat.a;
     const V3 half = safe_normalize(L + V);
     const float cosThetaHalf = fabsf(dot(half, n));
     const float pdfHalf = gtr2(cosThetaHalf, a) * cosThetaHalf;
@@ -274,7 +272,7 @@
     float sn, cs;
     fovpt_dm_sincos(angle, &sn, &cs);
     if (kind == SPECULAR) {
-        const float a = w.a;
+        const float a = mat.a;
         const float cosThetaHalf = sqrtf((1.0f - r2) / (1.0f + (sqr(a) - 1.0f) * r2));
         const float sinThetaHalf = sqrtf(fmaxf(0.0f, 1.0f - sqr(cosThetaHalf)));
         V3 half = U * (sinThetaHalf * cs) + V * (sinThetaHalf * sn) + N * cosThetaHalf;
@@ -292,7 +290,8 @@
     }
     return bsdf_pdf(mat, w, N, view, light);
 }
-__device__ V3 bsdf_eval(const Mat& mat, const V3& albedo, const BsdfView& w, const V3& N, const V3& V, const V3& L)
+__device__ V3 bsdf_eval(const Mat& mat, const V3& sqrt_color, const V3& albedo, const BsdfView& w, const V3& N, const V3& V,
+                        const V3& L)
 {
     float NDotL = dot(N, L);
     const float NDotV = w.NDotV;
@@ -305,13 +304,13 @@
     V3 brdf = v3(0.0f);
     float Ds = 0.0f, Gs = 0.0f;
     if (NDotL > 0) {
-        Ds = gtr2(NDotH, w.a);
-        Gs = w.GV_a * smith_ggx(NDotL, w.a);
+        Ds = gtr2(NDotH, mat.a);
+        Gs = w.GV_a * smith_ggx(NDotL, mat.a);
     }
     if (mat.transmission > 0.0f) {
         if (NDotL <= 0) {
             const float F = w.FrV;
-            bsdf = v3(mat.transmission * (1.0f - F) / fabsf(NDotL) * (1.0f - mat.metallic));
+            bsdf = v3(mat.transmission * (1.0f - F) / fabsf(NDotL) * mat.one_minus_metallic);
         } else {
             float FH = fresnel(LDotH, w.etaI, w.etaO);
             V3 Fs = lerp3(Cspec0, v3(1.0f), FH);
@@ -321,10 +320,10 @@
     if (mat.transmission < 1.0f) {
         if (NDotL <= 0) {
             if (mat.subsurface > 0.0f) {
-                V3 s = v3(sqrtf(mat.color.x), sqrtf(mat.color.y), sqrtf(mat.color.z));
+                const V3 s = sqrt_color;
                 float FL = schlick(fabsf(NDotL)), FV = w.FV;
                 float Fd = (1.0f - 0.5f * FL) * (1.0f - 0.5f * FV);
-                brdf = kInvPi * s * mat.subsurface * Fd * (1.0f - mat.metallic);
+                brdf = kInvPi * s * mat.subsurface * Fd * mat.one_minus_metallic;
             }
         } else {
             float FH = schlick(LDotH);
@@ -332,10 +331,10 @@
             float FL = schlick(NDotL), FV = w.FV;
             float Fd90 = half_plus_as_the_reference(2.0f * LDotH * LDotH * mat.roughness);
             float Fd = lerpf(1.0f, Fd90, FL) * lerpf(1.0f, Fd90, FV);
-            float Dr = gtr1_pre(NDotH, w.cc_a2, w.cc_log);
+            float Dr = gtr1_pre(NDotH, mat.cc_a2, mat.cc_log);
             float Fc = lerpf(.04f, 1.0f, FH);
             float Gr = smith_ggx(NDotL, .25f) * w.GV_q;
-            brdf = add_vs(kInvPi * Fd * Cdlin * (1.0f - mat.metallic) * (1.0f - mat.subsurface) + Gs * Fs * Ds,
+            brdf = add_vs(kInvPi * Fd * Cdlin * mat.one_minus_metallic * (1.0f - mat.subsurface) + Gs * Fs * Ds,
                           mat.clearcoat * Gr * Fc * Dr);
         }
     }
@@ -1130,6 +1129,25 @@
 #define FLAG_ALPHA_ONE 4u
 #define FLAG_ALPHA_SET 8u
 
+__device__ inline void shade_mesh_records(const MeshDev& M, ShadeMesh& r, ShadeMeshRare& q)
+{
+    const fovpt_material& mat = M.material;
+    r.color[0] = mat.color.x; r.color[1] = mat.color.y; r.color[2] = mat.color.z;
+    r.roughness = mat.roughness;
+    r.a = fmaxf(0.001f, mat.roughness);
+    r.transmission = mat.transmission; r.metallic = mat.metallic; r.subsurface = mat.subsurface;
+    r.specularTint = mat.specularTint; r.clearcoat = mat.clearcoat;
+    r.spec08 = (float)((double)mat.specular * .08);
+    r.out_eta = (mat.eta == 0.0f) ? 2.0f / (1.0f - sqrtf(0.08f * mat.specular)) - 1.0f : mat.eta;
+    const float cc_a = lerpf(.1f, .001f, mat.clearcoatGloss);
+    r.cc_a2 = cc_a >= 1 ? -1.0f : cc_a * cc_a;
+    r.cc_log = cc_a >= 1 ? 0.0f : fovpt_dm_logf(r.cc_a2);
+    r.one_minus_metallic = 1.0f - mat.metallic;
+    r.bits = ((mat.flags & FOVPT_MATERIAL_FLAG_SHADOW_CATCHER) ? FOVPT_SHADE_CATCHER : 0u)
+           | ((M.texture_id >= 0 && M.has_texcoord) ? FOVPT_SHADE_TEXTURED : 0u);
+    q.emission[0] = mat.emission.x; q.emission[1] = mat.emission.y; q.emission[2] = mat.emission.z; q.pad0 = 0.0f;
+    q.sqrt_color[0] = sqrtf(mat.color.x); q.sqrt_color[1] = sqrtf(mat.color.y); q.sqrt_color[2] = sqrtf(mat.color.z); q.pad1 = 0.0f;
+}
 #ifndef FOVPT_V_SHADEWAVES
 #define FOVPT_V_SHADEWAVES 1
 #endif
@@ -1183,17 +1201,21 @@
                 const V3 ray_o = v3(o4), ray_dir = v3(d4);
                 Rng rng_probe; rng_probe.s1 = rs.x; rng_probe.s2 = rs.y;
                 V3 wi, skyColor; float skyPdf;
-                probe_sample(fd.probe, fd.guide_x, fd.guide_y, fd.probe_rec, fd.probe_row_mul, wi, skyColor, skyPdf, rng_probe);
+                if (!EXTRA || fd.guide_x) probe_sample<true>(fd, wi, skyColor, skyPdf, rng_probe);
+                else probe_sample<false>(fd, wi, skyColor, skyPdf, rng_probe);
                 const float4 thr_in = ps.thr[slot];
-                const TriRec T = load_tri_off(sc.tris, tpos << 4);
-                const MeshDev M = sc.meshes[T.mesh];
-                const Mat& mat = M.material;
-                const V3 e1 = v3(T.e1x, T.e1y, T.e1z), e2 = v3(T.e2x, T.e2y, T.e2z);
-                const V3 N_0 = normalize(cross(e1, e2));
+                const float4* __restrict__ ts = (const float4*)(sc.tri_shade + tpos / 3u);
+                const float4 ts0 = ts[0];
+                const uint32_t mesh = __float_as_uint(ts[1].x), prim = __float_as_uint(ts0.w);
+                const Mat mat = sc.shade_meshes[mesh];
+                const ShadeMeshRare* __restrict__ rare = sc.shade_rare + mesh;
+                const V3 emission = (flags & FLAG_SECONDARY) == 0 ? v3(*(const float4*)rare->emission) : v3(0.f);
+                const V3 sqrt_color = mat.subsurface > 0.0f ? v3(*(const float4*)rare->sqrt_color) : v3(0.f);
+                const V3 N_0 = v3(ts0);
                 const V3 wo = neg(ray_dir);
                 const V3 N = N_0 * copysignf(1.0f, dot(wo, N_0));
                 const V3 P = ray_o + hit.x * ray_dir;
-                const bool catcher = (mat.flags & FOVPT_MATERIAL_FLAG_SHADOW_CATCHER) != 0;
+                const bool catcher = (mat.bits & FOVPT_SHADE_CATCHER) != 0;
                 if (catcher && (flags & FLAG_SECONDARY)) {
                     next_o = P; next_d = ray_dir; next_pdf = d4.w;
                     want_next = true;
@@ -1204,29 +1226,26 @@
                     V3 thr = v3(t4);
                     float rayEta = t4.w;
                     Rng rng = rng_probe;
-                    V3 albedo = v3(mat.color);
-                    if (M.texture_id >= 0 && M.has_texcoord) {
-                        const float2* tc = sc.tri_tc + (size_t)T.prim * 3;
+                    V3 albedo = v3(mat.color[0], mat.color[1], mat.color[2]);
+                    if (mat.bits & FOVPT_SHADE_TEXTURED) {
+                        const TexDev tex = sc.meshes[mesh].tex;
+                        const float2* tc = sc.tri_tc + (size_t)prim * 3;
                         const float2 t0 = tc[0], t1 = tc[1], t2 = tc[2];
                         const float w0 = 1.f - hit.y - hit.z;
                         const float tcx = (w0 * t0.x + hit.y * t1.x) + hit.z * t2.x;
                         const float tcy = (w0 * t0.y + hit.y * t1.y) + hit.z * t2.y;
-                        albedo = v3(tex2d(M.tex, tcx, tcy));
+                        albedo = v3(tex2d(tex, tcx, tcy));
                     }
                     if (ps.guide_n && depth == 0 && (flags & FLAG_SECONDARY) == 0) {
                         ps.guide_n[slot] = f4(N, 0.f);
                         ps.guide_a[slot] = f4(albedo, 0.f);
                     }
-                    float outEta;
-                    if (rayEta == 1.0f)
-                        outEta = (mat.eta == 0.0f) ? 2.0f / (1.0f - sqrtf(0.08f * mat.specular)) - 1.0f : mat.eta;
-                    else
-                        outEta = 1.0f;
+                    const float outEta = rayEta == 1.0f ? mat.out_eta : 1.0f;
                     const BsdfView view = bsdf_view(mat, albedo, rayEta, outEta, N, wo);
                     V3 sum_hit = v3(0.0f);
                     {
                         const float bsdfPdf = bsdf_pdf(mat, view, N, wo, wi);
-                        const V3 f = bsdf_eval(mat, albedo, view, N, wo, wi);
+                        const V3 f = bsdf_eval(mat, sqrt_color, albedo, view, N, wo, wi);
                         if (bsdfPdf > 0.0f) {
                             const float weight = 0.5f * skyPdf / (0.5f * bsdfPdf + 0.5f * skyPdf);
                             if (weight > 0.0f) {
@@ -1249,8 +1268,8 @@
                         alpha_occ = thr * sum_hit;
                     }
                     if ((flags & FLAG_SECONDARY) == 0) {
-                        rad_vis = rad_vis + v3(mat.emission);
-                        rad_occ = rad_occ + v3(mat.emission);
+                        rad_vis = rad_vis + emission;
+                        rad_occ = rad_occ + emission;
                     }
                     V3 bu, bv;
                     basis_from_vector(N, bu, bv);
@@ -1282,7 +1301,7 @@
                         flags |= FLAG_SECONDARY;
                         depth += 1;
                         if (depth < fd.max_depth || sc.any_catcher) {
-                            const V3 f = bsdf_eval(mat, albedo, view, N, wo, bsdfDir);
+                            const V3 f = bsdf_eval(mat, sqrt_color, albedo, view, N, wo, bsdfDir);
                             if (dot(bsdfDir, N) <= 0.0f) rayEta = outEta;
                             thr = thr * div_vs(f * fabsf(dot(N, bsdfDir)), bsdfPdf);
                             bool rr_kill = false;
@@ -1531,6 +1550,17 @@
     const float4 c = data[i];
     rec[2 * i] = make_float4(cdfX[i], pdfX[i], c.x, c.y);
     rec[2 * i + 1] = make_float4(c.z, 0.f, 0.f, 0.f);
+}
+
+__global__ void k_shade_meshes(int n, const MeshDev* __restrict__ meshes, ShadeMesh* __restrict__ out, ShadeMeshRare* __restrict__ rare)
+{
+    const int i = blockIdx.x * blockDim.x + threadIdx.x;
+    if (i >= n) return;
+    ShadeMesh r;
+    ShadeMeshRare q;
+    shade_mesh_records(meshes[i], r, q);
+    out[i] = r;
+    rare[i] = q;
 }
 
 #define CDF_ROWS 8
@@ -1667,7 +1697,7 @@
 void fovpt_launch_shade(hipStream_t st, const FrameDev& fd, SceneView sc, PathState ps, RayQueue queue_in, RayQueue queue_out,
                         ShadowQueue sq, uint32_t cap, Counters* cnt, int depth, int grid, hipEvent_t done, uint32_t sel)
 {
-    if (fd.options) {
+    if (fd.options || !fd.guide_x) {
         if (done) hipExtLaunchKernelGGL(k_shade<true>, dim3(grid), dim3(FOVPT_BLOCK), 0, st, nullptr, done, 0, fd, sc, ps, queue_in, queue_out, sq, cap, cnt, depth, sel);
         else hipLaunchKernelGGL(k_shade<true>, dim3(grid), dim3(FOVPT_BLOCK), 0, st, fd, sc, ps, queue_in, queue_out, sq, cap, cnt, depth, sel);
     } else {
@@ -1709,6 +1739,11 @@
 {
     hipLaunchKernelGGL(k_probe_records, dim3((unsigned)((n + 255) / 256)), dim3(256), 0, st, n, cdfX, pdfX, data, rec);
 }
+void fovpt_launch_shade_meshes(hipStream_t st, int n, const MeshDev* meshes, ShadeMesh* out, ShadeMeshRare* rare)
+{
+    hipLaunchKernelGGL(k_shade_meshes, dim3((n + 255) / 256), dim3(256), 0, st, n, meshes, out, rare);
+}
+
 void fovpt_launch_build_cdf(hipStream_t st, int w, int h, const float4* data, float* pdfX, float* cdfX, float* pdfY, float* cdfY, float* row_total)
 {
     hipLaunchKernelGGL(k_cdf_rows, dim3((h + CDF_ROWS - 1) / CDF_ROWS), dim3(CDF_COLS), 0, st, w, h, data, pdfX, cdfX, row_total);
```

Measured after the change: 4655 Mray/s (median of 6 runs). Within noise of the previous version (+0.9%).
